# yozhijk/capsaicin

Measured on AMD Instinct MI355X. Metric: Mrays/sec (primary+secondary), cornell_box 1080p 64spp, higher is better.
Workload: dtype f32; 1 GPU; cornell_box.obj 1920x1080 64spp depth=8 (reference shading: Lambert + directional light + sky), tile-sharded over 1 GPU(s); triangles=32, bvh_depth=8, parallelism=tiles1, exchange=none

## Files before the change

### capsaicin_amd/capi.py

```python
import ctypes as C
import os
import subprocess

import numpy as np

_PKG = os.path.dirname(os.path.abspath(__file__))
_ROOT = os.path.dirname(_PKG)
LIB_PATH = os.path.join(_PKG, "libcapsaicin_hip.so")
if os.environ.get("CAP_LIB_VARIANT"):
    LIB_PATH = os.path.join(_PKG, "variants", "libcapsaicin_hip_%s.so" % os.environ["CAP_LIB_VARIANT"])

RENDER_AOV = 1
RENDER_EXT_MATERIALS = 2
RENDER_STAGE_TIMERS = 4
RENDER_GBUFFER_FEEDBACK = 8
RENDER_LOWRES_INDIRECT = 16

BUF_GBUFFER_GEO, BUF_DIRECT, BUF_ALBEDO, BUF_NORMAL_DEPTH, BUF_INDIRECT, BUF_COMBINED, BUF_ACCUM_SUM, BUF_ACCUM_MEAN, BUF_INDIRECT_LOWRES = range(9)


class CapError(RuntimeError):
    pass


# ... 267 lines not shown
    "cap_obj_set_threads": (None, [C.c_int]),
    "cap_geometry_view": (_i, [_vp, C.POINTER(GeometryView)]),
    "cap_geometry_texture_name": (C.c_char_p, [_vp, _u32]),
    "cap_geometry_warning": (C.c_char_p, [_vp]),
    "cap_geometry_materials": (_i, [_vp, _vp]),
    "cap_scene_upload_geometry": (_i, [_vp, _vp]),
    "cap_comm_unique_id": (_i, [_vp]),
    "cap_comm_init_rank": (_i, [_vp, _vp, _u32, _u32]),
    "cap_comm_gather_frame": (_i, [_vp]),
    "cap_comm_init_all": (_i, [_vp, _u32]),
    "cap_comm_gather_frame_all": (_i, [_vp, _u32]),
    "cap_comm_image": (_i, [_vp, C.POINTER(C.c_void_p)]),
    "cap_comm_readback": (_i, [_vp, _vp]),
    "cap_comm_info": (_i, [_vp, C.POINTER(_u32), C.POINTER(_u32), C.POINTER(_u32)]),
    "cap_comm_destroy": (_i, [_vp]),
    "cap_comm_abort": (_i, [_vp]),
    "cap_image_decode": (_i, [_vp, C.c_size_t, C.c_char_p, C.POINTER(C.c_void_p), C.POINTER(_u32), C.POINTER(_u32)]),
    "cap_image_free": (None, [_vp]),
    "cap_host_sah_build": (_i, [_vp, _u32, _vp, _vp, C.POINTER(_u32)]),
    "cap_host_wide_build": (_i, [_vp, _u32, _vp, _vp, _vp, _u32, _vp, _vp]),
}

_LIB = None


def build_native(force=False):
    args = ["make", "-C", os.path.join(_PKG, "csrc"), "-j8"]
    if force:
        args.append("-B")
    subprocess.check_call(args, stdout=subprocess.DEVNULL)
    return LIB_PATH


def lib():
    global _LIB
    if _LIB is None:
        if not os.path.exists(LIB_PATH):
            raise CapError("native library %s is missing: run `python -c 'import __graft_entry__ as g; g.build()'` "
                           "(there is no CPU fallback)" % LIB_PATH)
        try:
            import torch
        except Exception:
            pass
        L = C.CDLL(LIB_PATH)
        for name, (res, args) in SYMBOLS.items():
            fn = getattr(L, name)
            fn.restype, fn.argtypes = res, args
        _LIB = L
    return _LIB


def _check(rc, what):
    if rc != 0:
        raise CapError("%s failed (status %d): %s" % (what, rc, lib().cap_last_error().decode()))


def _p(a):
    return a.ctypes.data_as(C.c_void_p)


def device_count():
    return int(lib().cap_device_count())


def load_bluenoise(path=None):
    path = path or os.path.join(_ROOT, "assets", "bluenoise256.rgba")
    return np.fromfile(path, np.uint8).reshape(256, 256, 4)


_SCENE_CONFIG = None


def scene_config():
    global _SCENE_CONFIG
    if _SCENE_CONFIG is None:
        import json
        cfg = json.load(open(os.path.join(os.path.dirname(_PKG), "assets", "scene_config.json")))
        cfg["cornell_ggx"] = {k: v for k, v in cfg["cornell_ggx"].items() if not k.startswith("_")}
        _SCENE_CONFIG = cfg
    return _SCENE_CONFIG


def camera_from_config(c, width, height):
    cam = CameraData()
    f = np.float64(c["forward"])
    f /= np.linalg.norm(f)
    right = np.float64(c["right"]) if "right" in c else -np.cross(f, (0.0, 1.0, 0.0))
    right /= np.linalg.norm(right)
    up = np.float64(c["up"]) if "up" in c else np.cross(f, right)
    cam.position[:] = c["position"]
    cam.forward[:] = f
    cam.right[:] = right
    cam.up[:] = up
    cam.focal_length = c["focal_length"]
    cam.sensor_size[0] = c["sensor_x"]
    cam.sensor_size[1] = np.float32(c["sensor_x"]) * (np.float32(height) / np.float32(width))
    return cam


def cornell_camera(width, height):
    return camera_from_config(scene_config()["cornell_camera"], width, height)


class Geometry:

    def __init__(self, obj_path, mtl_dir=None):
        self.h = C.c_void_p()
        _check(lib().cap_obj_load(obj_path.encode(), (mtl_dir or "").encode(), C.byref(self.h)), "cap_obj_load")
        v = GeometryView()
        _check(lib().cap_geometry_view(self.h, C.byref(v)), "cap_geometry_view")
        self.view = v
        nv, ni, nm = v.vertex_count, v.index_count, v.mesh_count
        self.positions = np.ctypeslib.as_array(v.positions, (3 * nv,)).copy() if nv else np.zeros(0, np.float32)
        self.normals = np.ctypeslib.as_array(v.normals, (3 * nv,)).copy() if nv else np.zeros(0, np.float32)
        self.texcoords = np.ctypeslib.as_array(v.texcoords, (2 * nv,)).copy() if nv else np.zeros(0, np.float32)
        self.indices = np.ctypeslib.as_array(v.indices, (ni,)).copy() if ni else np.zeros(0, np.uint32)
        self.meshes = np.ctypeslib.as_array(v.meshes, (nm * 8,)).copy().reshape(-1, 8) if nm else np.zeros((0, 8), np.uint32)
        self.texture_names = [lib().cap_geometry_texture_name(self.h, i).decode() for i in range(v.texture_count)]
        self.material_count = v.material_count
        self.warning = lib().cap_geometry_warning(self.h).decode()

    def materials(self):
        m = np.zeros((self.meshes.shape[0], 12), np.float32)
        _check(lib().cap_geometry_materials(self.h, _p(m)), "cap_geometry_materials")
        return m

    def __del__(self):
        if getattr(self, "h", None):
            lib().cap_geometry_free(self.h)
            self.h = None


def host_sah_build(tri_lo, tri_hi):
    lo, hi = np.asarray(tri_lo, np.float32), np.asarray(tri_hi, np.float32)
    n = len(lo)
    boxes = np.zeros((n, 8), np.float32)
    boxes[:, 0:3], boxes[:, 4:7] = lo, hi
    nodes = np.zeros((max(n - 1, 1), 16), np.float32)
    order = np.zeros(n, np.uint32)
    depth = C.c_uint32()
    _check(lib().cap_host_sah_build(_p(boxes), n, _p(nodes), _p(order), C.byref(depth)), "cap_host_sah_build")
    return nodes[:max(n - 1, 0)], order, int(depth.value)


def image_decode(data, name=None):
    buf = np.frombuffer(bytes(data), np.uint8)
    px, w, h = C.c_void_p(), _u32(), _u32()
    _check(lib().cap_image_decode(_p(buf), buf.size, name.encode() if name else None, C.byref(px), C.byref(w), C.byref(h)), "cap_image_decode")
    out = np.ctypeslib.as_array(C.cast(px, C.POINTER(C.c_uint8)), (h.value, w.value, 4)).copy()
    lib().cap_image_free(px)
    return out


def host_wide_build(nodes, n, scene_lo, scene_hi):
    nodes = np.ascontiguousarray(nodes, np.float32)
    lo, hi = np.ascontiguousarray(scene_lo, np.float32), np.ascontiguousarray(scene_hi, np.float32)
    wide = np.zeros((max(n, 1), 20), np.uint32)
    src = np.zeros(max(n, 1), np.uint32)
    info = np.zeros(3, np.uint32)
    _check(lib().cap_host_wide_build(_p(nodes) if n > 1 else None, n, _p(lo), _p(hi), _p(wide), wide.shape[0], _p(src), _p(info)),
           "cap_host_wide_build")
    return wide[:int(info[0])], src[:n], int(info[1]), int(info[2])


def comm_unique_id():
    buf = (C.c_uint8 * 128)()
    _check(lib().cap_comm_unique_id(C.cast(buf, C.c_void_p)), "cap_comm_unique_id")
    return bytes(buf)


def comm_init_all(renderers):
    arr = (C.c_void_p * len(renderers))(*[r.ctx for r in renderers])
    _check(lib().cap_comm_init_all(C.cast(arr, C.c_void_p), len(renderers)), "cap_comm_init_all")


def comm_gather_frame_all(renderers):
    arr = (C.c_void_p * len(renderers))(*[r.ctx for r in renderers])
    _check(lib().cap_comm_gather_frame_all(C.cast(arr, C.c_void_p), len(renderers)), "cap_comm_gather_frame_all")


class Renderer:

    def __init__(self, device=0, stream=None):
        self.ctx = C.c_void_p()
        _check(lib().cap_ctx_create(device, C.c_void_p(stream) if stream else None, C.byref(self.ctx)), "cap_ctx_create")
        self.width = self.height = 0
        self.device = device
        self._tri_end = np.zeros(0, np.int64)
        self._vertex_count = 0

    def close(self):
        if getattr(self, "ctx", None):
            lib().cap_ctx_destroy(self.ctx)
            self.ctx = None

    __del__ = close

    def upload_scene(self, positions, normals, texcoords, indices, meshes):
        a = [np.ascontiguousarray(positions, np.float32).ravel(), np.ascontiguousarray(normals, np.float32).ravel(),
             np.ascontiguousarray(texcoords, np.float32).ravel(), np.ascontiguousarray(indices, np.uint32).ravel(),
             np.ascontiguousarray(meshes, np.uint32).reshape(-1, 8)]
        _check(lib().cap_scene_upload(self.ctx, _p(a[0]), _p(a[1]), _p(a[2]), _p(a[3]), _p(a[4]), a[0].size // 3, a[3].size,
                                      a[4].shape[0]), "cap_scene_upload")
        self._set_mesh_table(a[4])
        self._vertex_count = a[0].size // 3

    def upload_geometry(self, geo):
        _check(lib().cap_scene_upload_geometry(self.ctx, geo.h), "cap_scene_upload_geometry")
        self._set_mesh_table(geo.meshes)
        self._vertex_count = int(geo.view.vertex_count)

    def _set_mesh_table(self, meshes):
        self._tri_end = np.cumsum(np.asarray(meshes, np.uint32).reshape(-1, 8)[:, 2].astype(np.int64) // 3)

    def upload_texture(self, index, rgba8):
        if rgba8 is None:
            _check(lib().cap_texture_upload(self.ctx, index, None, 0, 0), "cap_texture_upload")
            return
        t = np.ascontiguousarray(rgba8, np.uint8)
        _check(lib().cap_texture_upload(self.ctx, index, _p(t), t.shape[1], t.shape[0]), "cap_texture_upload")

    def upload_bluenoise(self, rgba8):
        t = np.ascontiguousarray(rgba8, np.uint8)
        assert t.size == 256 * 256 * 4
        _check(lib().cap_bluenoise_upload(self.ctx, _p(t)), "cap_bluenoise_upload")

    def upload_materials(self, materials):
        m = np.ascontiguousarray(materials, np.float32).reshape(-1, 12)
        _check(lib().cap_materials_upload(self.ctx, _p(m), m.shape[0]), "cap_materials_upload")

    BVH_BUILD_AUTO, BVH_BUILD_LBVH, BVH_BUILD_SAH, BVH_BUILD_PLOC, BVH_BUILD_SAH_DEVICE = 0, 1, 2, 3, 4

    def set_bvh_build(self, mode):
        _check(lib().cap_set_bvh_build(self.ctx, mode), "cap_set_bvh_build")

    def build_bvh(self):
        _check(lib().cap_bvh_build(self.ctx), "cap_bvh_build")
        return self.bvh_info()

    def update_vertices(self, positions=None, normals=None, texcoords=None):
        ptrs, flags, keep = vertex_update_args(self._vertex_count, positions, normals, texcoords)
        if flags:
            import torch
            dev = torch.device("cuda", self.device)
            for a in keep:
                if a.device != dev:
                    raise CapError("update_vertices: tensors must be on %s, got %s" % (dev, a.device))
            torch.cuda.current_stream(dev).synchronize()
        _check(lib().cap_scene_update_vertices(self.ctx, ptrs[0], ptrs[1], ptrs[2], flags), "cap_scene_update_vertices")

    def refit_bvh(self):
        info = RefitInfo()
        _check(lib().cap_bvh_refit(self.ctx, C.byref(info)), "cap_bvh_refit")
        return info

    def bvh_info(self):
        bi = BvhInfo()
        _check(lib().cap_bvh_info(self.ctx, C.byref(bi)), "cap_bvh_info")
        return bi

    def bvh_readback(self):
        bi = self.bvh_info()
        nodes = np.zeros((bi.node_count, 16), np.float32)
        leaves = np.zeros(bi.triangle_count, np.uint32)
        _check(lib().cap_bvh_readback(self.ctx, _p(nodes), _p(leaves)), "cap_bvh_readback")
        return nodes, leaves

    def bvh_wide_readback(self):
        info = np.zeros(3, np.uint32)
        _check(lib().cap_bvh_wide_readback(self.ctx, None, None, _p(info)), "cap_bvh_wide_readback")
        nodes = np.zeros((int(info[0]), 20), np.uint32)
        src = np.zeros(max(1, self.bvh_info().triangle_count), np.uint32)
        _check(lib().cap_bvh_wide_readback(self.ctx, _p(nodes), _p(src), _p(info)), "cap_bvh_wide_readback")
        return nodes, src[:self.bvh_info().triangle_count], int(info[1]), int(info[2])

    def bvh_wide_info(self):
        info = np.zeros(3, np.uint32)
        _check(lib().cap_bvh_wide_readback(self.ctx, None, None, _p(info)), "cap_bvh_wide_readback")
        return int(info[0]), int(info[1]), int(info[2])

    def set_camera(self, cam):
        _check(lib().cap_camera_set(self.ctx, C.byref(cam)), "cap_camera_set")

    def set_prev_camera(self, cam):
        _check(lib().cap_prev_camera_set(self.ctx, C.byref(cam)), "cap_prev_camera_set")

    def set_resolution(self, width, height):
        _check(lib().cap_set_resolution(self.ctx, width, height), "cap_set_resolution")
        self.width, self.height = width, height

    def set_shard(self, index, count):
        _check(lib().cap_set_shard(self.ctx, index, count), "cap_set_shard")

    def set_traversal(self, mode):
        _check(lib().cap_set_traversal(self.ctx, mode), "cap_set_traversal")

    DEBUG_QUEUE_CAPACITY_DIV, DEBUG_WIDE_DEPTH_LIMIT, DEBUG_WIDE_IN_USE, DEBUG_FAIL_LANE1, DEBUG_LANES_USED = 1, 2, 3, 4, 5
    DEBUG_QUEUE_CANARY_FILL, DEBUG_QUEUE_CANARY_BEHIND, DEBUG_QUEUE_CANARY_USED, DEBUG_SELFTEST_DIV, DEBUG_NEE_PAIRS = 6, 7, 8, 9, 10
    DEBUG_SELFTEST_SHADE_UNARY, DEBUG_SELFTEST_SHADE_DIV2, DEBUG_SHADE_TAME = 11, 12, 13
    DEBUG_CAMERA_CULL = 14
    DEBUG_MARK_FORM = 15
    DEBUG_SAMPLE_TABLE = 16
    DEBUG_SELFTEST_SAMPLE_TABLE = 17

    def debug_set(self, key, value):
        _check(lib().cap_debug_set(self.ctx, key, value), "cap_debug_set")

    DEBUG_SWITCH_BASE = 64

    def debug_switch(self, name, value):
        i = lib().cap_debug_switch_index(name.encode())
        if i < 0:
            raise CapError("unknown switch %s" % name)
        self.debug_set(self.DEBUG_SWITCH_BASE + i, 0xFFFFFFFFFFFFFFFF if value is None else int(value))

    def debug_get(self, key):
        v = _u64()
        _check(lib().cap_debug_get(self.ctx, key, C.byref(v)), "cap_debug_get")
        return int(v.value)

    def set_batch_paths(self, n):
        _check(lib().cap_set_batch_paths(self.ctx, n), "cap_set_batch_paths")

    def render(self, frame_begin, n_frames, num_bounces, flags=0):
        _check(lib().cap_render(self.ctx, frame_begin, n_frames, num_bounces, flags), "cap_render")

    def accum_reset(self):
        _check(lib().cap_accum_reset(self.ctx), "cap_accum_reset")

    def accum_import(self, sum_rgba, frames):
        a = np.ascontiguousarray(sum_rgba, np.float32)
        assert a.shape == (self.height, self.width, 4)
        _check(lib().cap_accum_import(self.ctx, _p(a), int(frames)), "cap_accum_import")

    def sync(self):
        _check(lib().cap_sync(self.ctx), "cap_sync")

    def readback(self, kind):
        if kind == BUF_INDIRECT_LOWRES:
            out = np.zeros((self.height // 2, self.width // 2, 4), np.float32)
        else:
            out = np.zeros((self.height, self.width, 4), np.float32)
        _check(lib().cap_readback(self.ctx, kind, _p(out)), "cap_readback")
        return out

    def stats(self):
        s = Stats()
        _check(lib().cap_stats_get(self.ctx, C.byref(s)), "cap_stats_get")
        return s

    def stats_reset(self):
        _check(lib().cap_stats_reset(self.ctx), "cap_stats_reset")

    RAY_FLAG_ACCEPT_FIRST_HIT, RAY_FLAG_CULL_BACK_FACING, RAY_FLAG_CULL_FRONT_FACING = 0x04, 0x10, 0x20

    def set_instance_masks(self, masks):
        if masks is None:
            _check(lib().cap_scene_set_instance_masks(self.ctx, None, len(self._tri_end)), "cap_scene_set_instance_masks")
            return
        m = np.ascontiguousarray(masks, np.uint8).reshape(-1)
        _check(lib().cap_scene_set_instance_masks(self.ctx, _p(m), m.size), "cap_scene_set_instance_masks")

    def trace_options(self, cull=None, mask=None, first_hit=False):
        if cull not in (None, "back", "front"):
            raise CapError('cull must be None, "back" or "front", got %r' % (cull,))
        if cull is None and mask is None and not first_hit:
            return None
        flags = {None: 0, "back": self.RAY_FLAG_CULL_BACK_FACING, "front": self.RAY_FLAG_CULL_FRONT_FACING}[cull]
        if first_hit:
            flags |= self.RAY_FLAG_ACCEPT_FIRST_HIT
        return TraceOptions(flags, 0 if mask is None else int(mask))

    MULTI_MAX_K, MULTI_CONTINUE = 16, 1

    def _stage_records(self, records, width, what):
        import torch
        dev = torch.device("cuda", self.device)
        if isinstance(records, np.ndarray):
            records = torch.from_numpy(np.ascontiguousarray(records, np.float32).reshape(-1, width)).to(dev)
        if records.dtype != torch.float32 or records.dim() != 2 or records.shape[1] != width or not records.is_contiguous() or records.device != dev:
            raise CapError("%s must be a contiguous (N, %d) float32 tensor on %s, got %s %s on %s"
                           % (what, width, dev, records.dtype, tuple(records.shape), records.device))
        return dev, records, records.shape[0]

    def _out(self, out, shape, dtype, dev):
        host_out = None
        if isinstance(out, np.ndarray):
            host_out, out = out, None
        if out is None:
            import torch
            out = torch.empty(shape, dtype=dtype, device=dev)
        elif out.dtype != dtype or out.shape != shape or not out.is_contiguous() or out.device != dev:
            raise CapError("out must be a contiguous %s %s tensor on %s, got %s %s on %s" % (shape, dtype, dev, out.dtype, tuple(out.shape), out.device))
        return out, host_out

    def _resume_page(self, page, shape, dtype, dev, what):
        if page is None or isinstance(page, np.ndarray):
            import torch
            if page is None:
                return torch.empty(shape, dtype=dtype, device=dev), None
            if page.size == int(np.prod(shape)):
                return torch.from_numpy(np.ascontiguousarray(page, np.float32 if dtype == torch.float32 else np.int32).reshape(shape)).to(dev), page
        elif page.dtype == dtype and page.shape == shape and page.is_contiguous() and page.device == dev:
            return page, None
        raise CapError("%s must be the %s %s page of the previous call, a contiguous tensor on %s or a numpy array of its size, got %s %s"
                       % (what, shape, dtype, dev, page.dtype, tuple(page.shape)))

    def _page_size(self, k, counts, resuming):
        k = int(k)
        if not 0 <= k <= self.MULTI_MAX_K:
            raise CapError("k must be in 0 .. %d (page with resume=), got %d" % (self.MULTI_MAX_K, k))
        if k == 0 and (not counts or resuming):
            raise CapError("k = 0 counts only: pass counts=True and no resume")
        return k

    def _run(self, name, args, dev, sync, host, outputs, host_outputs):
        if sync:
            import torch
            torch.cuda.current_stream(dev).synchronize()
        _check(getattr(lib(), name)(self.ctx, *[a if a is None or type(a) in (int, C.c_float) else C.byref(a) if type(a) is TraceOptions
                                                else C.c_void_p(a.data_ptr()) for a in args]), name)
        if sync or host:
            self.sync()
        if not host:
            return outputs
        res = []
        for out, mine in zip(outputs, host_outputs):
            h = out.cpu().numpy()
            if mine is not None:
                mine[...] = h.reshape(mine.shape)
                h = mine
            res.append(h)
        return res

    def _single(self, name, records, width, what, out, cols, dtype, sync, tail, second=()):
        host = isinstance(records, np.ndarray)
        dev, records, n = self._stage_records(records, width, what)
        out, host_out = self._out(out, (n, cols) if cols else (n,), dtype, dev)
        extra = [out.new_empty((n,), dtype=t) for t in second]
        res = self._run(name, (records, n, out, *extra, *tail), dev, sync or host, host or host_out is not None,
                        [out] + extra, [host_out] + [None] * len(extra))
        return tuple(res) if second else res[0]

    def _multi(self, name, records, width, what, cols, instanced, k, counts, resume, sync, tail):
        import torch
        if not instanced:
            given, names = [resume], ("resume",)
        elif resume is None or (isinstance(resume, (tuple, list)) and len(resume) == 2):
            given, names = [None, None] if resume is None else list(resume), ("resume[0]", "resume[1]")
        else:
            raise CapError("resume must be the (records, instances) pair of pages of the previous call")
        host = isinstance(records, np.ndarray)
        dev, records, n = self._stage_records(records, width, what)
        k = self._page_size(k, counts, resume is not None)
        pages, host_pages = [], []
        for page, page_name, (shape, dtype) in zip(given, names, (((n, k, cols), torch.float32), ((n, k), torch.int32))):
            page, mine = self._resume_page(page, shape, dtype, dev, page_name)
            pages.append(page)
            host_pages.append(mine)
            host = host or mine is not None
        cnt = [torch.empty((n,), dtype=torch.int32, device=dev)] if counts else []
        res = self._run(name, (records, n, k, *(pages if k else [None] * len(pages)), cnt[0] if counts else None,
                               self.MULTI_CONTINUE if resume is not None else 0, *tail),
                        dev, sync or host, host, pages + cnt, host_pages + [None])
        return tuple(res) if instanced or counts else res[0]

    @staticmethod
    def _plain_or_ex(name, options, plain_tail):
        return (name, plain_tail) if options is None else (name + "_ex", (options,))

    def trace_rays(self, rays, out=None, sync=True, cull=None, mask=None, first_hit=False):
        import torch
        name, tail = self._plain_or_ex("cap_trace_rays", self.trace_options(cull, mask, first_hit), (0,))
        return self._single(name, rays, 8, "rays", out, 4, torch.float32, sync, tail)

    def trace_occlusion(self, rays, out=None, sync=True, cull=None, mask=None):
        import torch
        name, tail = self._plain_or_ex("cap_trace_occlusion", self.trace_options(cull, mask), (0,))
        return self._single(name, rays, 8, "rays", out, 0, torch.int32, sync, tail)

    def _closest_single(self, name, points, out, sync, mask, second=()):
        import torch
        return self._single(name, points, 4, "points", out, 8, torch.float32, sync, (self.trace_options(None, mask),), second)

    def closest_points(self, points, out=None, sync=True, mask=None):
        return self._closest_single("cap_closest_points", points, out, sync, mask)

    def build_pseudonormals(self):
        info = PseudonormalsInfo()
        _check(lib().cap_pseudonormals_build(self.ctx, C.byref(info)), "cap_pseudonormals_build")
        return info

    def drop_pseudonormals(self):
        _check(lib().cap_pseudonormals_drop(self.ctx), "cap_pseudonormals_drop")

    def pseudonormals(self):
        table = np.zeros((int(self._tri_end[-1]) if len(self._tri_end) else 0, 7, 3), np.float32)
        _check(lib().cap_pseudonormals_readback(self.ctx, _p(table)), "cap_pseudonormals_readback")
        return table

    def signed_distance(self, points, out=None, sync=True, mask=None, sign="pseudonormal", beta=2.0):
        import torch
        if sign == "pseudonormal":
            return self._closest_single("cap_signed_distance", points, out, sync, mask, (torch.float32,))
        if sign != "winding":
            raise CapError('sign must be "pseudonormal" or "winding", got %r' % (sign,))
        if mask is not None:
            raise CapError('sign="winding" takes no mask=: the winding number covers every triangle')
        host = isinstance(points, np.ndarray)
        dev, pts, n = self._stage_records(points, 4, "points")
        rec, host_out = self._out(out, (n, 8), torch.float32, dev)
        rec, signed = self._closest_single("cap_signed_distance", pts, rec, sync or host, None, (torch.float32,))
        w = self.winding_numbers(pts, beta=beta, sync=sync or host)
        signed = torch.where(w >= 0.5, -signed.abs(), signed.abs())
        if not (host or host_out is not None):
            return rec, signed
        h = rec.cpu().numpy()
        if host_out is not None:
            host_out[...] = h.reshape(host_out.shape)
            h = host_out
        return h, signed.cpu().numpy()

    def build_winding(self):
        info = WindingInfo()
        _check(lib().cap_winding_build(self.ctx, C.byref(info)), "cap_winding_build")
        return info

    def drop_winding(self):
        _check(lib().cap_winding_drop(self.ctx), "cap_winding_drop")

    def winding_table(self):
        table = np.zeros((max(self.bvh_info().triangle_count, 1) - 1, 2, 8), np.float32)
        _check(lib().cap_winding_readback(self.ctx, _p(table)), "cap_winding_readback")
        return table

    def winding_numbers(self, points, beta=2.0, out=None, visits=False, sync=True):
        import torch
        host = isinstance(points, np.ndarray)
        dev, points, n = self._stage_records(points, 4, "points")
        out, host_out = self._out(out, (n,), torch.float32, dev)
        vis = [torch.empty((n, 2), dtype=torch.int32, device=dev)] if visits else []
        res = self._run("cap_winding_numbers", (points, n, C.c_float(beta), out, vis[0] if visits else None), dev, sync or host,
                        host or host_out is not None, [out] + vis, [host_out, None])
        return tuple(res) if visits else res[0]

    def closest_instances(self, points, out=None, sync=True, mask=None):
        import torch
        return self._closest_single("cap_closest_instances", points, out, sync, mask, (torch.int32,))

    def signed_distance_instances(self, points, out=None, sync=True, mask=None):
        import torch
        return self._closest_single("cap_signed_distance_instances", points, out, sync, mask, (torch.int32, torch.float32))

    def closest_points_multi(self, points, k, counts=False, resume=None, sync=True, mask=None):
        return self._multi("cap_closest_points_multi", points, 4, "points", 8, False, k, counts, resume, sync, (self.trace_options(None, mask),))

    def closest_instances_multi(self, points, k, counts=False, resume=None, sync=True, mask=None):
        return self._multi("cap_closest_instances_multi", points, 4, "points", 8, True, k, counts, resume, sync, (self.trace_options(None, mask),))


    def set_objects(self, ranges):
        info = ObjectsInfo()
        r = np.zeros((0, 2), np.uint32) if ranges is None else np.ascontiguousarray(ranges, np.uint32).reshape(-1, 2)
        _check(lib().cap_objects_set(self.ctx, _p(r) if len(r) else None, len(r), C.byref(info)), "cap_objects_set")
        self._instances_n = 0
        return info

    def objects_info(self):
        n = C.c_uint32(0)
        _check(lib().cap_objects_info(self.ctx, None, 0, C.byref(n)), "cap_objects_info")
        out = np.zeros(n.value, OBJECT_INFO_DTYPE)
        if n.value:
            _check(lib().cap_objects_info(self.ctx, _p(out), n.value, None), "cap_objects_info")
        return out

    def set_instances(self, transforms, masks=None, sync=True, objects=None):
        info = InstancesInfo()
        if transforms is None:
            _check(lib().cap_instances_set(self.ctx, None, 0, 0, C.byref(info)), "cap_instances_set")
            self._instances_n = 0
            return info
        if isinstance(transforms, np.ndarray) or not hasattr(transforms, "device"):
            t = np.ascontiguousarray(transforms, np.float32)
            if t.ndim < 2 or t.size != t.shape[0] * 12:
                raise CapError("transforms must be (N, 3, 4) or (N, 12), got %s" % (t.shape,))
            d = np.zeros(t.shape[0], INSTANCE_DESC_DTYPE)
            d["transform"] = t.reshape(-1, 12)
            d["mask"] = 0xFF if masks is None else np.asarray(masks).astype(np.uint32).reshape(-1)
            if objects is None:
                _check(lib().cap_instances_set(self.ctx, _p(d), d.shape[0], 0, C.byref(info)), "cap_instances_set")
            else:
                o = np.ascontiguousarray(np.asarray(objects).astype(np.uint32).reshape(-1))
                if o.size != d.shape[0]:
                    raise CapError("objects must hold one index per instance (%d), got %d" % (d.shape[0], o.size))
                _check(lib().cap_instances_set_ex(self.ctx, _p(d), _p(o), d.shape[0], 0, C.byref(info)), "cap_instances_set_ex")
            self._instances_n = d.shape[0]
            return info
        import torch
        dev = torch.device("cuda", self.device)
        if transforms.dtype != torch.float32 or transforms.device != dev or transforms.numel() != transforms.shape[0] * 12:
            raise CapError("transforms must be an (N, 3, 4) or (N, 12) float32 tensor on %s" % (dev,))
        n = transforms.shape[0]
        d = torch.zeros((n, 16), dtype=torch.float32, device=dev)
        d[:, :12] = transforms.reshape(n, 12)
        m = torch.full((n,), 0xFF, dtype=torch.int32, device=dev) if masks is None else torch.as_tensor(masks, device=dev).to(torch.int32).reshape(n)
        d[:, 12] = m.view(torch.float32)
# ... 128 lines not shown
```

### capsaicin_amd/csrc/cap_context.h

```cpp
#pragma once

#include <array>
#include <string>
#include <utility>
#include <vector>

#include "../../include/capsaicin_hip.h"

#include "cap_kernels.h"

namespace cap
{
int fail(int code, const char* fmt, ...);

#define HIP_TRY(expr)                                                                                         \
    do                                                                                                        \
    {                                                                                                         \
        hipError_t e_ = (expr);                                                                               \
        if (e_ != hipSuccess) return fail(CAP_ERR_HIP, "%s failed: %s (%s:%d)", #expr, hipGetErrorString(e_), \
                                          __FILE__, __LINE__);                                                \
    } while (0)

template <typename T>
struct DevBuf
{
    T*     p = nullptr;
    size_t n = 0;
    DevBuf() = default;
    DevBuf(const DevBuf&) = delete;
    DevBuf& operator=(const DevBuf&) = delete;
    DevBuf(DevBuf&& o) noexcept : p(o.p), n(o.n) { o.p = nullptr, o.n = 0; }
    DevBuf& operator=(DevBuf&& o) noexcept
    {
        if (this != &o)
        {
            release();
            p = o.p, n = o.n, o.p = nullptr, o.n = 0;
        }
        return *this;
    }
    ~DevBuf() { release(); }
    void release()
    {
        if (p) (void)hipFree(p);
        p = nullptr, n = 0;
    }
    hipError_t ensure(size_t count)
    {
        if (count <= n && p) return hipSuccess;
        release();
        if (count == 0) count = 1;
        hipError_t e = hipMalloc((void**)&p, count * sizeof(T));
        if (e == hipSuccess) n = count;
        return e;
    }
};

enum StageId
{
    ST_PRIMARY,
    ST_CLOSEST,
    ST_ANY,
    ST_SHADE,
    ST_RESOLVE,
    ST_POST,
    ST_COUNT,
    ST_DIRECT,
    ST_POST_PASS0,
    ST_NONE = -1
};

struct TimedSpan
{
    hipEvent_t a, b;
    int        stage;
    int        also = ST_NONE;
};
}

using namespace cap;

struct CapContext
{
    int         device = 0;
    hipStream_t stream = nullptr;
    bool        own_stream = false;
    int         cu_count = 256;

    DevBuf<float>    positions, normals, texcoords;
    DevBuf<uint32_t> indices;
    DevBuf<uint4>    tri_ids;
    DevBuf<uint4>    mesh_offsets;
    DevBuf<uint32_t> mesh_texture;
    uint32_t         vertex_count = 0, index_count = 0, mesh_count = 0, tri_count = 0;
    bool             scene_ready = false;

    std::vector<DevBuf<uint8_t>> texture_data;
    std::vector<TextureDev>      texture_host;
    DevBuf<TextureDev>           textures;
    bool                         textures_dirty = true;
    DevBuf<float2>               bluenoise;
    bool                         bluenoise_ready = false;
    std::vector<CapMaterial>     materials_host;
    DevBuf<CapMaterial>          materials;
    std::vector<float>           positions_host;
    std::vector<uint32_t>        indices_host;
    std::vector<CapMeshDesc>     meshes_host;
    DevBuf<uint32_t>             light_tris;
    DevBuf<float>                light_cdf;
    DevBuf<float2>               bluenoise_ba;
    uint32_t                     light_count = 0;
    float                        light_area  = 0.0f;
    bool                         materials_ready = false;

    DevBuf<float4>   shade_tris, tris_sorted, nodes, tri_raw, tri_box;
    DevBuf<float4>   nodes8, tris8;
    DevBuf<uint32_t> wide_src;
    DevBuf<uint32_t> wide_task, wide_alloc, wide_cnt;
    uint32_t         wide8_depth = 0, wide8_top = 0, wide8_nodes = 0;
    float            wide8_ms = 0.f;
    DevBuf<uint32_t> query_work, query_defer;
    DevBuf<uint8_t>  tri_mask;
    bool             tri_mask_on = false;
    DevBuf<float4>   inst_desc, inst_rec, inst_box, inst_tlas;
    DevBuf<uint32_t> inst_keys[2], inst_vals[2], inst_hist, inst_scan, inst_misc, inst_level_off;
    uint32_t         inst_count = 0, inst_top = 0, inst_nodes = 0;
    DevBuf<float2>   inst_near;
    DevBuf<uint32_t> inst_obj;
    bool             inst_obj_on = false;
    InstObject       scene_object_host{};
    DevBuf<InstObject> scene_object;
    std::vector<CapObjectInfo> obj_info;
    std::vector<uint32_t>      obj_node_base, obj_rec_base;
    uint32_t                   obj_count = 0, obj_max_depth = 0;
    DevBuf<float4>             forest_nodes, forest_tris;
    DevBuf<InstObject>         obj_table;
    DevBuf<float4>             obj_tri_raw, obj_tri_box;
    DevBuf<uint32_t>           obj_leaf_tri, obj_misc;
    DevBuf<float4>   fan_pairs, fan_singles;
    uint32_t         fan_pair_count = 0, fan_single_count = 0;
    DevBuf<float4>   fan_pairs_nee;
    uint32_t         fan_pair_nee_count = 0;
    std::vector<float>    fan_pairs_host;
    std::vector<uint32_t> light_tris_host;
    DevBuf<uint32_t> leaf_tri, keys0, keys1, vals0, vals1, hist, parent, flags, bvh_misc;
    DevBuf<float4>   ploc_boxes;
    DevBuf<uint32_t> ploc_ints;
    DevBuf<uint32_t> sahdev_words;
    CapBvhInfo       bvh_info{};
    bool             shade_tame = false;
    bool             bvh_ready = false;
    DevBuf<float>        pn_table;
    bool                 pn_ready = false;
    CapPseudonormalsInfo pn_info{};
    DevBuf<float4>       wn_table;
    bool                 wn_ready = false;
    CapWindingInfo       wn_info{};
    bool                  bvh_stale = false;
    bool                  positions_host_stale = false;
    bool                  visits_built_known = false;
    double                refit_visits_built = 0.0;
    std::vector<uint32_t> wide_levels;
    DevBuf<float>         wide_boxes;
    DevBuf<double>        refit_sums;

    CapCameraData camera{}, prev_camera{};
    bool          camera_ready = false, prev_camera_ready = false;
    ScreenDev     screen{};
    uint64_t      max_batch_paths = 0;
    SwitchTable   sw{};
    uint32_t      debug_capacity_div = 1;
    uint32_t      debug_wide_depth_limit = 0;
    bool          debug_fail_lane = false;
    uint64_t      lane1_failed_paths = 0;
    uint32_t      lane1_failed_bounces = 0, lane1_retry_tick = 0;
    uint32_t      lanes_last_render = 0;
    uint32_t      last_class_capacity = 0;
    uint32_t      tri_ids_dense = 0;
    uint32_t      last_mark_form = 0;
    uint32_t      last_sample_table = 0;
    struct LastTerms
    {
        const FrameConst* frames = nullptr;
        uint32_t          n_slots = 0, num_bounces = 0, lane = 0;
    } last_terms;
    uint32_t      last_cull_camera_pairs = 0;
    uint32_t      traversal_mode  = CAP_TRAVERSAL_AUTO;
    uint32_t      bvh_build_mode  = CAP_BVH_BUILD_AUTO;

    DevBuf<float4>     aov_geo, aov_nd, accum, image_tmp;
    DevBuf<uint64_t>   shaded_counter;
    struct Lane
    {
        hipStream_t      stream = nullptr;
        DevBuf<float4>   hits, q_org[2], q_dir[2], q_thr[2], s_org, s_dir, s_con, pl_color, pl_direct, pl_albedo;
        DevBuf<float4>   terms;
        DevBuf<uint32_t> counters;
        DevBuf<uint32_t> stack_spill;
    } lane[2];
    hipStream_t stream2 = nullptr;
    hipEvent_t  lane_ev[2] = {nullptr, nullptr}, fork_ev = nullptr, join_ev = nullptr;
    static constexpr int kFrameRing = 4;
    DevBuf<FrameConst> frames_ring[kFrameRing];
    FrameConst*        frames_pinned[kFrameRing] = {nullptr, nullptr, nullptr, nullptr};
    size_t             frames_pinned_n[kFrameRing] = {0, 0, 0, 0};
    hipEvent_t         frames_event[kFrameRing] = {nullptr, nullptr, nullptr, nullptr};
    uint32_t           frames_next = 0;
    uint32_t           last_slots = 0;
    bool               aov_valid = false;
    bool               aov_lowres = false;
    uint32_t           aov_frame  = 0;
    uint64_t           frames_accumulated = 0;

    DevBuf<float4> post_in[4];
    DevBuf<float4> post_ihist[2], post_mhist[2], post_chist[2], post_prev_nd, post_itemp, post_temp[2], post_normals;
    uint32_t       post_w = 0, post_h = 0;
    int            post_last_dst = -1;

    void*           comm = nullptr;
    uint32_t        comm_rank = 0, comm_size = 0;
    bool            comm_local = false;
    DevBuf<float>   comm_send, comm_gathered, comm_image;
    hipEvent_t      comm_event = nullptr;

    CapStats               stats{};
    std::vector<TimedSpan> spans;
    std::vector<std::array<hipEvent_t, 6>> post_marks;
    std::vector<hipEvent_t> event_pool;
    std::vector<uint32_t*> pinned_pool;
    std::vector<std::pair<uint32_t*, uint32_t>> pending;
    uint64_t*              pinned_shaded = nullptr;
};

namespace cap
{
struct AovPlanes
{
    const float4 *color, *direct, *albedo;
};

int        sync_and_collect(CapContext* c);
hipEvent_t get_event(CapContext* c);
CameraDev  camera_dev(const CapCameraData& cd);
BvhDev     bvh_dev(const CapContext* c, const CapContext::Lane& lane);
AovPlanes  aov_planes(const CapContext* c);
int        trace_launch(const CapContext* c, const char* fmt, ...);
void       launch_texture_footprints(hipStream_t stream, const uint32_t* src, uint4* dst, uint32_t width, uint32_t height);
bool pair_ids_dense(const float* pairs, uint32_t pair_count, uint32_t single_count, uint32_t tri_count);
int  upload_fan_records(CapContext* c);
int  update_nee_pairs(CapContext* c);
int  ensure_positions_host(CapContext* c);
int  upload_light_table(CapContext* c);
int query_state(CapContext* c, const char* what);
}
```

### capsaicin_amd/csrc/cap_kernels.h

```cpp
#pragma once

#include "cap_device.h"

#include <cstdio>
#include <vector>

namespace cap
{
enum CapSwitch : uint32_t
{
    SW_NO_WIDE8 = 0,
    SW_LANE1_PRIORITY,
    SW_PLOC_RADIUS,
    SW_SAHDEV_LEAF,
    SW_WIDE_HOST_COLLAPSE,
    SW_TRACE_LAUNCHES,
    SW_NO_TWO_LANES,
    SW_LANE_SPLIT_MIN,
    SW_BLOCKS_PER_CU,
    SW_NO_CAMERA_CULL,
    SW_NO_ALBEDO_IN_W,
    SW_NO_INLINE_NEE,
    SW_NO_INLINE_PROBE,
    SW_NO_WAVE_RING,
    SW_ANY_REFILL,
    SW_PRIMARY_WIDE,
    SW_NO_PACKET,
    SW_NO_ANY_PROBE,
    SW_ANY_PROBE,
    SW_ANY_BLOCKS,
    SW_NO_PRIMARY_FUSE,
    SW_W8_REFILL,
    SW_W8_GRID,
    SW_AUTO_SAH_TRIANGLES,
    SW_NO_NEE_PAIR_CULL,
    SW_RAYGEN_KERNEL,
    SW_NO_PLANE_CODE,
    SW_SAMPLE_TABLE,
    SW_COUNT
};
struct SwitchTable
{
    int64_t v[SW_COUNT];
    bool    on(CapSwitch k) const { return v[k] > 0; }
    int64_t get(CapSwitch k, int64_t dflt) const { return v[k] >= 0 ? v[k] : dflt; }
};

struct LaunchCfg
{
    hipStream_t stream;
    uint32_t    grid_blocks;
    uint32_t    stack_entries;
    uint32_t    cu_count = 0;
    uint32_t    any_no_probe = 0;
    const SwitchTable* sw = nullptr;
    bool    sw_on(CapSwitch k) const { return sw && sw->on(k); }
    int64_t sw_get(CapSwitch k, int64_t dflt) const { return sw ? sw->get(k, dflt) : dflt; }
};

template <auto K>
uint32_t resident_grid(const LaunchCfg& cfg, uint32_t want)
{
    static int per_cu = -1;
    if (per_cu < 0)
    {
        int n = 0;
        per_cu = (hipOccupancyMaxActiveBlocksPerMultiprocessor(&n, K, (int)kBlock, 0) == hipSuccess && n > 0) ? n : 0;
        if (cfg.sw_on(SW_TRACE_LAUNCHES)) fprintf(stderr, "[cap] resident workgroups per CU: %d\n", per_cu);
    }
    if (!cfg.cu_count || !per_cu) return want;
    const uint32_t cap = cfg.cu_count * (uint32_t)per_cu;
    return want < cap ? want : cap;
}
inline uint32_t queue_grid(const LaunchCfg& cfg, uint32_t max_count)
{
    uint32_t g = (max_count + kBlock - 1) / kBlock;
    if (g > cfg.grid_blocks) g = cfg.grid_blocks;
    return g ? g : 1;
}

void launch_trace_primary(const LaunchCfg& cfg, const BvhDev& bvh, const CameraDev& cam, const ScreenDev& screen,
                          const FrameConst* frames, uint32_t n_slots, float4* hits, uint32_t* work);
void launch_raygen_identity(const LaunchCfg& cfg, const CameraDev& cam, const ScreenDev& screen, const FrameConst* frames, uint32_t n_slots,
                            const RayQueue& q);
void launch_trace_closest(const LaunchCfg& cfg, const BvhDev& bvh, const RayQueue& q, uint32_t max_count, float4* hits);
void launch_trace_closest8(const LaunchCfg& cfg, const BvhDev& bvh, const RayQueue& q, uint32_t max_count, float4* hits, uint32_t* work);
void launch_trace_closest8_camera(const LaunchCfg& cfg, const BvhDev& bvh, const RayQueue& q, uint32_t max_count, float4* hits, uint32_t* work,
                                  const CameraDev& cam, const ScreenDev& screen, const FrameConst* frames, uint32_t n_slots);
void launch_trace_any(const LaunchCfg& cfg, const BvhDev& bvh, const ShadowQueue& q, uint32_t max_count, float4* target,
                      uint32_t pixels_padded, uint32_t n_slots, uint64_t* guard, uint32_t* work, bool mostly_unoccluded,
                      const FrameConst* frames, float4* code_plane = nullptr);

void launch_trace_any8_refill(const LaunchCfg& cfg, const BvhDev& bvh, const ShadowQueue& q, uint32_t max_count, float4* target, uint32_t pixels_padded,
                              uint32_t n_slots, uint64_t* guard, uint32_t* work, const FrameConst* frames);

struct QueryArgs
{
    const float4* rays;
    uint32_t      n;
    void*         out;
    uint32_t*     work;
    uint32_t*     defer;
    float         safe;
};
constexpr float kQuerySafeScale = 4.0f;
bool query8_stack_matches();
struct RayFilter;
void launch_query8(const LaunchCfg& cfg, const BvhDev& bvh, const QueryArgs& q, bool any, const RayFilter* f = nullptr, bool first_hit = false);
void launch_query_binary(const LaunchCfg& cfg, const BvhDev& bvh, const QueryArgs& q, bool any, bool deferred);
struct MultiArgs
{
    QueryArgs q;
    uint32_t  k;
    uint32_t* counts;
    uint32_t  resume;
};
constexpr uint32_t kMultiMaxK = 16;
uint32_t multi_bucket(uint32_t k);
void     launch_query8_multi(const LaunchCfg& cfg, const BvhDev& bvh, const MultiArgs& m, const RayFilter* f = nullptr);
void     launch_query_binary_multi(const LaunchCfg& cfg, const BvhDev& bvh, const MultiArgs& m, bool deferred, const RayFilter* f = nullptr);

struct RayFilter
{
    uint32_t       cull_and, cull_xor;
    uint32_t       mask;
    const uint8_t* tri_mask;
};
void launch_query_binary_filtered(const LaunchCfg& cfg, const BvhDev& bvh, const QueryArgs& q, const RayFilter& f, bool any, bool first_hit, bool deferred);

struct ClosestArgs
{
    const float4* points;
    uint32_t      n;
    float4*       out;
    float         slack;
};
constexpr float kClosestSlackScale = 1.0f / 262144.0f;
void launch_closest_points(const LaunchCfg& cfg, const BvhDev& bvh, const ClosestArgs& a, const RayFilter* f, uint32_t depth);
struct SignedArgs
{
    const float* normals;
    float*       signed_out;
};
void launch_signed_distance(const LaunchCfg& cfg, const BvhDev& bvh, const ClosestArgs& a, const SignedArgs& s, const RayFilter* f, uint32_t depth);
struct ClosestMultiArgs
{
    ClosestArgs a;
    uint32_t    k;
    uint32_t*   counts;
    uint32_t    resume;
};
void launch_closest_points_multi(const LaunchCfg& cfg, const BvhDev& bvh, const ClosestMultiArgs& m, const RayFilter* f, uint32_t depth);
struct TlasDev;
struct ClosestInstArgs
{
    ClosestArgs     a;
    uint32_t*       inst_out;
    const float4*   descs;
    const float2*   near;
    const uint32_t* xw_max;
};
void launch_closest_instances(const LaunchCfg& cfg, const BvhDev& bvh, const ClosestInstArgs& a, const TlasDev& tl, const RayFilter& f, uint32_t depth);
void launch_signed_distance_instances(const LaunchCfg& cfg, const BvhDev& bvh, const ClosestInstArgs& a, const SignedArgs& s, const TlasDev& tl,
                                      const RayFilter& f, uint32_t depth);
struct ClosestInstMultiArgs
{
    ClosestInstArgs ia;
    uint32_t        k;
    uint32_t*       counts;
    uint32_t        resume;
};
void launch_closest_instances_multi(const LaunchCfg& cfg, const BvhDev& bvh, const ClosestInstMultiArgs& m, const TlasDev& tl, const RayFilter& f,
                                    uint32_t depth);

struct InstObject
{
    double   blo[3], bhi[3];
    int32_t  root;
    uint32_t reserved;
};
struct InstanceBuildArgs
{
    const float*      descs;
    uint32_t          n;
    const InstObject* objects;
    uint32_t          n_objects;
    const uint32_t*   object_index;
    float4*      rec;
    float4*      box;
    float4*      tlas;
    float2*      near;
    uint32_t*    keys[2];
    uint32_t*    vals[2];
    uint32_t*    hist;
    uint32_t*    scan;
    uint32_t*    misc;
};
constexpr uint32_t kTlasMaxLevels = 25;
uint32_t tlas_layout(uint32_t n, uint32_t level_off[kTlasMaxLevels], uint32_t* total);
void     launch_instances_build(hipStream_t stream, const InstanceBuildArgs& a);
struct TlasDev
{
    const float4*   rec;
    const float4*   tlas;
    const uint32_t* level_off;
    uint32_t        top;
};
void launch_query_instances(const LaunchCfg& cfg, const BvhDev& bvh, const QueryArgs& q, const TlasDev& tl, const RayFilter& f, int mode, uint32_t* inst_out,
                            uint32_t depth);
void launch_query_instances_multi(const LaunchCfg& cfg, const BvhDev& bvh, const MultiArgs& m, const TlasDev& tl, const RayFilter& f, uint32_t* inst_out,
                                  uint32_t depth);
struct ForestRelocArgs
{
    float4*  nodes;
    float4*  tris;
    uint32_t n_tris, node_base, rec_base, first_triangle;
};
void launch_forest_relocate(hipStream_t stream, const ForestRelocArgs& a);

struct ShadeArgs
{
    SceneDev          scene;
    CameraDev         cam;
    ScreenDev         screen;
    const FrameConst* frames;
    union
    {
        const float4* hits;
        const float4* sample_terms;
    };
    RayQueue          in;
    RayQueue          out;
    ShadowQueue       shadow;
    Planes            planes;
    uint32_t          n_slots;
    uint32_t          bounce;
    uint32_t          num_bounces;
    uint32_t          max_count;
    uint32_t          aov_slot;
    uint64_t*         shaded_counter;
    uint32_t*         work;
    FeedbackDev       fb;
    uint32_t          albedo_in_w;
    uint32_t          inline_nee;
    uint32_t          inline_probe;
    uint32_t          wave_ring;
    uint32_t          cull_camera_pairs;
    uint32_t          code_in_color;
};
constexpr float kCodePadding = 0.f, kCodeSky = 1.f, kCodeKd = 2.f, kCodeBlack = 3.f;
constexpr float kCodeLit = 4.f;
constexpr float kCameraCullPad = 2.0f;
void launch_shade(const LaunchCfg& cfg, const ShadeArgs& args, bool ext, bool feedback = false);
bool launch_primary_shade(const LaunchCfg& cfg, const BvhDev& bvh, const ShadeArgs& args, float4* hits, bool ext);
uint32_t launch_trace_shade(const LaunchCfg& cfg, const BvhDev& bvh, const ShadeArgs& args, bool ext, bool feedback = false);
bool trace_shade_has_code_form(const BvhDev& bvh, const SceneDev& scene);
bool trace_shade_has_table_form(const BvhDev& bvh, const SceneDev& scene);
void launch_sample_terms(hipStream_t stream, const float2* bluenoise, const FrameConst* frames, uint32_t n_slots, uint32_t num_bounces, float4* table);
void launch_sample_terms_selftest(hipStream_t stream, const float2* bluenoise, const FrameConst* frames, uint32_t n_slots, uint32_t num_bounces,
                                  const float4* table, unsigned long long* out_device);

void launch_resolve(const LaunchCfg& cfg, const Planes& planes, uint32_t n_slots, uint32_t pixels_padded, float4* accum,
                    bool albedo_in_w = false, float kd_untextured = 0.0f, bool code_in_color = false);
void launch_untile(const LaunchCfg& cfg, const ScreenDev& screen, const float4* src, const float4* albedo, const float4* direct,
                   int plane_kind, float4* image);
void launch_tile(const LaunchCfg& cfg, const ScreenDev& screen, const float4* image, float4* dst);
void launch_untile4(const LaunchCfg& cfg, const ScreenDev& screen, const float4* s0, const float4* s1, const float4* s2, const float4* s3,
                    float4* d0, float4* d1, float4* d2, float4* d3);
void launch_tiles_mean(const LaunchCfg& cfg, const float4* accum, uint32_t pixels_padded, float4* dst);
void launch_assemble(const LaunchCfg& cfg, const ScreenDev& screen, const float4* gathered, uint32_t shard_count, float4* image,
                     size_t shard_stride = 0);
void launch_geo_aov(const LaunchCfg& cfg, const SceneDev& scene, const float4* hits_slot, uint32_t pixels_padded, float4* aov_geo);

struct BvhBuildArgs
{
    const float*    positions;
    const float*    normals;
    const float*    texcoords;
    const uint32_t* indices;
    const uint4*    tri_ids;
    const uint4*    mesh_offsets;
    uint32_t        tri_count;
    float4*         shade_tris;
    float4*         tris_sorted;
    float4*         nodes;
    uint32_t*       leaf_tri;
    float4*         tri_raw;
    float4*         tri_box;
    uint32_t*       keys[2];
    uint32_t*       vals[2];
    uint32_t*       hist;
    uint32_t*       parent;
    uint32_t*       flags;
    uint32_t*       bounds;
    uint32_t*       max_depth;
};
size_t bvh_radix_blocks(uint32_t n);
void   launch_bvh_build(hipStream_t stream, const BvhBuildArgs& a);
int    launch_bvh_sort(hipStream_t stream, const BvhBuildArgs& a);
size_t bvh_radix_scan_words(uint32_t n);
int    launch_radix_sort_pairs(hipStream_t stream, uint32_t* const keys[2], uint32_t* const vals[2], uint32_t n, uint32_t* hist, uint32_t* scan);
size_t bvh_scan_scratch_words(uint32_t total);
void   launch_exclusive_scan_u32(hipStream_t stream, uint32_t* v, uint32_t total, uint32_t* scratch);
struct PlocScratch
{
    float4*   boxes;
    uint32_t* ints;
};
int    launch_bvh_build_ploc(hipStream_t stream, const BvhBuildArgs& a, const PlocScratch& s, uint32_t radius);
size_t bvh_sah_device_scratch_words(uint32_t n);
int    launch_bvh_build_sah_device(hipStream_t stream, const BvhBuildArgs& a, const PlocScratch& s, uint32_t* scratch, uint32_t radius, uint32_t leaf);
void launch_bvh_setup(hipStream_t stream, const BvhBuildArgs& a);
void launch_bvh_finish_host(hipStream_t stream, const BvhBuildArgs& a);

void     launch_gather_wide(hipStream_t stream, const uint32_t* tri_src, const float4* tris_sorted, uint32_t n, float4* tris8);
struct WideCollapseArgs
{
    const float4*   bnodes;
    const uint32_t* count;
    uint32_t        n_tris, capacity;
    double          pad;
    uint32_t *      task, *alloc, *nodes8, *tri_src;
    uint32_t*       cnt;
    uint32_t        begin, end;
};
int      launch_wide_collapse(hipStream_t stream, WideCollapseArgs a, uint32_t* node_count, uint32_t* depth, uint32_t* top_nodes,
                          std::vector<uint32_t>* level_begin = nullptr);
struct PseudonormalArgs
{
    const float*    positions;
    const uint32_t* indices;
    const uint4*    tri_ids;
    const uint4*    mesh_offsets;
    uint32_t        tri_count;
    float*          table;
    uint32_t *      kx, *ky, *kz;
    uint32_t*       keys[2];
    uint32_t*       vals[2];
    uint32_t*       weld;
    uint32_t*       flag;
    uint32_t*       hist;
    uint32_t*       scan;
    double*         nf;
    double*         ang;
    uint32_t*       stats;
};
size_t pseudonormal_scan_words(uint32_t corners);
void   launch_pseudonormals_build(hipStream_t stream, const PseudonormalArgs& a);

struct WindingBuildArgs
{
    const float*    positions;
    const uint32_t* indices;
    const uint4*    tri_ids;
    const uint4*    mesh_offsets;
    uint32_t        tri_count;
    const float4*   nodes;
    const uint32_t* leaf_tri;
    float4*         table;
    double*         tri_sums;
    double*         sums;
    uint32_t*       parent;
    uint32_t*       flags;
    uint32_t*       stats;
    double*         root;
};
void launch_winding_build(hipStream_t stream, const WindingBuildArgs& a);
struct WindingArgs
{
    const float4* points;
    uint32_t      n;
    const float4* table;
    float         beta;
    float*        out;
    uint32_t*     visits;
};
void launch_winding_numbers(const LaunchCfg& cfg, const BvhDev& bvh, const WindingArgs& a, uint32_t depth);

void   launch_bvh_refit_climb(hipStream_t stream, const BvhBuildArgs& a);
void   launch_refit_binary(hipStream_t stream, const BvhBuildArgs& a);
size_t tree_visits_scratch();
void   launch_tree_visits(hipStream_t stream, const float4* nodes, uint32_t n_tris, double* scratch, double* out);
struct WideRefitArgs
{
    uint32_t*     nodes8;
    const float4* tris8;
    const float4* tri_box;
    float*        boxes;
    double        pad;
    uint32_t      one_triangle;
    uint32_t      begin, end;
};
void launch_refit_wide(hipStream_t stream, WideRefitArgs a, const std::vector<uint32_t>& level_begin);
uint32_t wide8_stack_pairs();

struct PostSettingsDev
{
    int   gather, denoise, eaw5;
    float eaw_normal_sigma, eaw_depth_sigma, eaw_luma_sigma;
    float gather_normal_sigma, gather_depth_sigma, gather_luma_sigma;
    float temporal_upscale_feedback, taa_feedback;
    int   lowres_indirect;
    int   use_variance;
    int   fast_weights;
    int   output;
};
struct PostChainArgs
{
    PostSettingsDev settings;
    uint32_t        width, height, frame_count;
    CameraDev       camera, prev_camera;
    const float4 *indirect, *direct, *albedo, *normal_depth;
    uint32_t      tiled;
    const float4 *tiled_indirect, *tiled_normal_depth;
    float4*       indirect_rowmajor;
    ScreenDev     screen;
    float4 *indirect_history[2], *moments_history[2], *combined_history[2], *prev_normal_depth;
    float4 *indirect_temp, *temp[2], *normals;
    void (*mark)(void* user, int pass);
    void* mark_user;
};
void launch_post_chain(hipStream_t stream, const PostChainArgs& a);
void launch_div_selftest(hipStream_t stream, unsigned long long* out_device);
void launch_shade_forms_selftest(hipStream_t stream, unsigned long long* out_device, uint32_t which);
void launch_decimate2x(hipStream_t stream, const float4* full, uint32_t width, uint32_t height, uint32_t ox, uint32_t oy, float4* out);
}
```

### capsaicin_amd/csrc/context.hip

```cpp
#include <algorithm>
#include <cmath>
#include <cstdarg>
#include <cstdio>
#include <cstdlib>
#include <cstring>
#include <memory>

#include "cap_context.h"
#include "cap_near.h"
#include "cap_wide.h"
#include "query_ranges.h"

namespace
{
thread_local std::string g_error;

constexpr double kPrimaryWideTrianglesPerPixel = 2.0;
constexpr uint64_t kAnyRefillTreeBytes = ~0ull;

constexpr size_t kGuardWords = 8;
}

namespace cap
{
int fail(int code, const char* fmt, ...)
{
    char    buf[512];
    va_list ap;
    va_start(ap, fmt);
    vsnprintf(buf, sizeof(buf), fmt, ap);
    va_end(ap);
    g_error = buf;
    return code;
}

int sync_and_collect(CapContext* c)
{
    HIP_TRY(hipStreamSynchronize(c->stream));
    for (auto& sp : c->spans)
    {
        float ms = 0.f;
        if (hipEventElapsedTime(&ms, sp.a, sp.b) == hipSuccess)
        {
            for (int stage : {sp.stage, sp.also})
                switch (stage)
                {
                case ST_PRIMARY: c->stats.ms_primary += ms; break;
                case ST_CLOSEST: c->stats.ms_trace_closest += ms; break;
                case ST_ANY: c->stats.ms_trace_any += ms; break;
                case ST_SHADE: c->stats.ms_shade += ms; break;
                case ST_RESOLVE: c->stats.ms_resolve += ms; break;
                case ST_POST: c->stats.ms_post += ms; break;
                case ST_COUNT: c->stats.ms_total += ms; break;
                case ST_DIRECT: c->stats.ms_direct += ms; break;
                default:
                    if (stage >= ST_POST_PASS0 && stage < ST_POST_PASS0 + 5) c->stats.ms_post_pass[stage - ST_POST_PASS0] += ms;
                }
        }
        c->event_pool.push_back(sp.a);
        c->event_pool.push_back(sp.b);
    }
    c->spans.clear();
    for (auto& m : c->post_marks)
    {
        for (int pass = 0; pass < 5; ++pass)
        {
            float ms = 0.f;
            if (hipEventElapsedTime(&ms, m[pass], m[pass + 1]) == hipSuccess) c->stats.ms_post_pass[pass] += ms, c->stats.ms_post += ms;
        }
        for (hipEvent_t e : m) c->event_pool.push_back(e);
    }
    c->post_marks.clear();
    for (auto& pc : c->pending)
    {
        const uint32_t D = pc.second & 0xffffu;
        const bool     queued = (pc.second >> 16) == 0u;
        const size_t per = (size_t)kQueueClasses * kCounterStride;
        for (uint32_t b = 0; b <= D; ++b)
            for (uint32_t k = 0; k < kQueueClasses; ++k)
            {
                c->stats.rays_extension += pc.first[b * per + k * kCounterStride];
                c->stats.rays_shadow += pc.first[b * per + k * kCounterStride + 1];
                if (queued) c->stats.shadow_entries += pc.first[b * per + k * kCounterStride + 1];
                if (b == 0)
                {
                    c->stats.rays_extension_bounce0 += pc.first[k * kCounterStride];
                    c->stats.rays_shadow_bounce0 += pc.first[k * kCounterStride + 1];
                    if (queued) c->stats.shadow_entries_bounce0 += pc.first[k * kCounterStride + 1];
                }
                c->stats.rays_shadow += pc.first[b * per + k * kCounterStride + 2];
                if (b == 0) c->stats.rays_shadow_bounce0 += pc.first[k * kCounterStride + 2];
                c->stats.shaded_vertices += pc.first[b * per + k * kCounterStride + 3];
            }
        c->pinned_pool.push_back(pc.first);
    }
    c->pending.clear();
    if (c->pinned_shaded && c->shaded_counter.p)
    {
        HIP_TRY(hipMemcpy(c->pinned_shaded, c->shaded_counter.p, kGuardWords * sizeof(uint64_t), hipMemcpyDeviceToHost));
        c->stats.guard_shade     = c->pinned_shaded[1];
        c->stats.guard_trace_any = c->pinned_shaded[2];
        c->stats.guard_last      = c->pinned_shaded[3];
        c->stats.guard_append    = c->pinned_shaded[4];
    }
    return CAP_OK;
}

hipEvent_t get_event(CapContext* c)
{
    if (!c->event_pool.empty())
    {
        hipEvent_t e = c->event_pool.back();
        c->event_pool.pop_back();
        return e;
    }
    hipEvent_t e = nullptr;
    (void)hipEventCreate(&e);
    return e;
}

CameraDev camera_dev(const CapCameraData& cd)
{
    CameraDev d{};
    for (int k = 0; k < 3; ++k) d.position[k] = cd.position[k], d.right[k] = cd.right[k], d.forward[k] = cd.forward[k], d.up[k] = cd.up[k];
    d.focal_length = cd.focal_length;
    d.sensor_x     = cd.sensor_size[0];
    d.sensor_y     = cd.sensor_size[1];
    return d;
}

BvhDev bvh_dev(const CapContext* c, const CapContext::Lane& lane)
{
    BvhDev b{};
    b.nodes     = c->nodes.p;
    b.tris      = c->tris_sorted.p;
    b.tris_by_id = c->tri_raw.p;
    b.stack_spill   = lane.stack_spill.p;
    b.spill_threads = (uint32_t)(lane.stack_spill.n / kSpillEntries);
    const bool no_wide8 = c->sw.on(SW_NO_WIDE8);
    b.nodes8 = c->nodes8.p, b.tris8 = c->tris8.p;
    b.wide8_ok  = !no_wide8 && lane.stack_spill.p && c->wide8_nodes != 0 && c->wide8_depth <= wide8_stack_pairs() + 1u &&
                 c->wide8_depth <= kWideLdsEntries / 2u + kSpillEntries / 2u + 1u &&
                 (c->debug_wide_depth_limit == 0u || c->wide8_depth <= c->debug_wide_depth_limit);
    b.wide8_top = c->wide8_top;
    b.fan_pairs = c->fan_pairs.p, b.fan_singles = c->fan_singles.p;
    b.fan_pair_count = c->fan_pair_count, b.fan_single_count = c->fan_single_count;
    b.tri_ids_dense = c->tri_ids_dense;
    b.fan_pairs_nee = c->fan_pairs_nee.p ? c->fan_pairs_nee.p : c->fan_pairs.p;
    b.fan_pair_nee_count = c->fan_pairs_nee.p ? c->fan_pair_nee_count : c->fan_pair_count;
    b.tri_count = c->tri_count;
    b.root      = c->tri_count >= 2 ? 0 : ~0;
    return b;
}

AovPlanes aov_planes(const CapContext* c)
{
    const size_t off = (size_t)(c->last_slots ? c->last_slots - 1 : 0) * c->screen.pixels_padded;
    return AovPlanes{c->lane[0].pl_color.p + off, c->lane[0].pl_direct.p + off, c->lane[0].pl_albedo.p + off};
}

int trace_launch(const CapContext* c, const char* fmt, ...)
{
    if (!c->sw.on(SW_TRACE_LAUNCHES)) return CAP_OK;
    va_list ap;
    va_start(ap, fmt);
    fputs("[cap] ", stderr);
    vfprintf(stderr, fmt, ap);
    va_end(ap);
    fputs(" ... ", stderr);
    fflush(stderr);
    hipError_t e = hipStreamSynchronize(c->stream);
    fprintf(stderr, "%s\n", hipGetErrorString(e));
    fflush(stderr);
    return e == hipSuccess ? CAP_OK : CAP_ERR_HIP;
}
}

namespace
{
struct StageTimer
{
    CapContext* c;
    TimedSpan   sp;
    bool        on;
    StageTimer(CapContext* ctx, int stage, bool enabled = true, int also = ST_NONE) : c(ctx), on(enabled)
    {
        if (!on) return;
        sp.stage = stage;
        sp.also  = also;
        sp.a     = get_event(c);
        sp.b     = get_event(c);
        (void)hipEventRecord(sp.a, c->stream);
    }
    ~StageTimer()
    {
        if (!on) return;
        (void)hipEventRecord(sp.b, c->stream);
        c->spans.push_back(sp);
    }
};

void update_screen(CapContext* c, uint32_t w, uint32_t h, uint32_t shard_index, uint32_t shard_count)
{
    ScreenDev& s  = c->screen;
    s.width       = w;
    s.height      = h;
    s.tiles_x     = (w + kTileDim - 1) / kTileDim;
    s.tiles_y     = (h + kTileDim - 1) / kTileDim;
    s.tile_count  = s.tiles_x * s.tiles_y;
    s.shard_index = shard_index;
    s.shard_count = shard_count ? shard_count : 1;
    const uint32_t max_local = (s.tile_count + s.shard_count - 1) / s.shard_count;
    s.local_tiles   = s.tile_count > s.shard_index ? (s.tile_count - s.shard_index + s.shard_count - 1) / s.shard_count : 0;
    s.pixels_padded = max_local * kTilePixels;
    tile_div_setup(s.tiles_x, s.tiles_x_mul, s.tiles_x_shift);
    c->frames_accumulated = 0;
    c->aov_valid = false;
}

FrameConst frame_const(uint32_t frame_count, bool lowres_indirect)
{
    FrameConst f{};
    halton23(frame_count, f.jitter_x, f.jitter_y);
    f.frame_count = frame_count;
    f.lowres_sel = lowres_indirect ? (4u | (((frame_count % 4u) / 2u) << 1) | ((frame_count % 4u) % 2u)) : 0u;
    const float t = 2.0f * 3.14f * (float)(frame_count % 4096) / 4096.0f;
    float       st, ct;
    sincos_c(t, st, ct);
    const v3 dir = normalize3(mk3(40.0f * st, 100.0f, 40.0f * ct));
    f.light_dir[0] = dir.x, f.light_dir[1] = dir.y, f.light_dir[2] = dir.z;
    f.light_intensity[0] = 1.0f * (2.0f * 14.0f + 0.0f);
    f.light_intensity[1] = 1.0f * (2.0f * 12.0f + 0.0f);
    f.light_intensity[2] = 1.0f * (2.0f * 10.0f + (2.0f + 2.0f * ct));
    return f;
}

SceneDev scene_dev(const CapContext* c)
{
    SceneDev s{};
    s.shade_tris    = c->shade_tris.p;
    s.tri_ids       = c->tri_ids.p;
    s.mesh_texture  = c->mesh_texture.p;
    s.textures      = c->textures.p;
    s.texture_count = (uint32_t)c->texture_host.size();
    s.bluenoise     = c->bluenoise.p;
    s.kd_untextured = pow22_c(0.75f);
    s.shade_tame    = c->shade_tame ? 1u : 0u;
    s.bluenoise_ba  = c->bluenoise_ba.p;
    s.materials     = reinterpret_cast<const MaterialDev*>(c->materials.p);
    s.material_count = c->materials_ready ? c->mesh_count : 0u;
    s.light_tris    = c->light_tris.p;
    s.light_cdf     = c->light_cdf.p;
    s.light_count   = c->light_count;
    s.light_area    = c->light_area;
    return s;
}

struct LaneSizes
{
    size_t planes, queues, rings, counters, terms;
};

LaneSizes lane_sizes(const CapContext* c, uint32_t slots, uint32_t bounces, bool sample_table)
{
    LaneSizes z;
    z.planes = (size_t)slots * c->screen.pixels_padded;
    z.queues = z.planes + (size_t)kQueueClasses * 64;
    z.rings = std::max(z.queues, (size_t)std::max(c->cu_count, 1) * 8 * (kBlock / 64) * 128);
    z.counters = (3 * (size_t)(bounces + 1) + 1) * kQueueClasses * kCounterStride;
    z.terms = sample_table ? (size_t)slots * bounces * 4096 : 0;
    return z;
}

bool lane_grows(const CapContext::Lane& L, const LaneSizes& z) { return L.pl_color.n < z.planes || L.counters.n < z.counters || L.terms.n < z.terms; }

int ensure_lane(CapContext* c, CapContext::Lane& L, uint32_t slots, uint32_t bounces, bool sample_table)
{
    const LaneSizes z = lane_sizes(c, slots, bounces, sample_table);
    for (DevBuf<float4>* b : {&L.hits, &L.q_org[0], &L.q_org[1], &L.q_dir[0], &L.q_dir[1], &L.q_thr[0], &L.q_thr[1], &L.s_dir})
        HIP_TRY(b->ensure(z.queues));
    for (DevBuf<float4>* b : {&L.s_org, &L.s_con}) HIP_TRY(b->ensure(z.rings));
    for (DevBuf<float4>* b : {&L.pl_color, &L.pl_direct, &L.pl_albedo}) HIP_TRY(b->ensure(z.planes));
    HIP_TRY(L.counters.ensure(z.counters));
    if (z.terms) HIP_TRY(L.terms.ensure(z.terms));
    if (c->lane[0].stack_spill.n) HIP_TRY(L.stack_spill.ensure(c->lane[0].stack_spill.n));
    return CAP_OK;
}

int ensure_frame_buffers(CapContext* c)
{
    HIP_TRY(c->aov_geo.ensure(c->screen.pixels_padded));
    HIP_TRY(c->aov_nd.ensure(c->screen.pixels_padded));
    if (!c->shaded_counter.p)
    {
        HIP_TRY(c->shaded_counter.ensure(kGuardWords));
        HIP_TRY(hipMemsetAsync(c->shaded_counter.p, 0, kGuardWords * sizeof(uint64_t), c->stream));
    }
    if (!c->accum.p || c->accum.n < c->screen.pixels_padded)
    {
        HIP_TRY(c->accum.ensure(c->screen.pixels_padded));
        HIP_TRY(hipMemsetAsync(c->accum.p, 0, sizeof(float4) * c->screen.pixels_padded, c->stream));
        c->frames_accumulated = 0;
    }
    return CAP_OK;
}

int ensure_lane_streams(CapContext* c)
{
    if (!c->stream2)
    {
        if (c->sw.v[SW_LANE1_PRIORITY] >= 0)
            HIP_TRY(hipStreamCreateWithPriority(&c->stream2, hipStreamNonBlocking, (int)c->sw.v[SW_LANE1_PRIORITY]));
        else
            HIP_TRY(hipStreamCreateWithFlags(&c->stream2, hipStreamNonBlocking));
    }
    c->lane[1].stream = c->stream2;
    for (hipEvent_t* e : {&c->lane_ev[0], &c->lane_ev[1], &c->fork_ev, &c->join_ev})
        if (!*e) HIP_TRY(hipEventCreateWithFlags(e, hipEventDisableTiming));
    return CAP_OK;
}

struct BatchPolicy
{
    uint32_t slots;
    bool     two_lanes;
    bool     lane1_failed_before;
};

BatchPolicy batch_policy(const CapContext* c, uint32_t n_frames, uint32_t num_bounces, uint32_t flags, bool tree_path)
{
    const uint32_t Ppad = c->screen.pixels_padded;
    uint64_t       budget = c->max_batch_paths ? c->max_batch_paths : (uint64_t)64 << 20;
    if (!c->max_batch_paths && (uint64_t)n_frames * Ppad > budget)
    {
        const uint64_t big       = (uint64_t)128 << 20;
        const uint64_t big_slots = std::max<uint64_t>(1, std::min<uint64_t>(big / std::max(1u, Ppad), kMaxFrameSlots));
        bool           room      = c->lane[0].pl_color.n >= big_slots * Ppad && (!tree_path || c->lane[1].pl_color.n >= big_slots * Ppad);
        if (!room)
        {
            size_t free_b = 0, total_b = 0;
            room = hipMemGetInfo(&free_b, &total_b) == hipSuccess && free_b > 3u * big_slots * Ppad * 256u;
        }
        if (room) budget = big;
    }
    uint32_t       slots  = (uint32_t)std::max<uint64_t>(1, std::min<uint64_t>(budget / std::max(1u, Ppad), kMaxFrameSlots));
    slots                 = std::min(slots, n_frames);
    const bool no_two_lanes = c->sw.on(SW_NO_TWO_LANES);
    bool two_lanes = !no_two_lanes && tree_path && c->bvh_info.stack_entries != 0 && !(flags & CAP_RENDER_GBUFFER_FEEDBACK) &&
                     !(flags & CAP_RENDER_LOWRES_INDIRECT) && n_frames >= 2;
    if (two_lanes && slots >= n_frames)
    {
        const uint64_t split_min = (uint64_t)c->sw.get(SW_LANE_SPLIT_MIN, (int64_t)4 << 20);
        if ((uint64_t)n_frames * Ppad >= split_min)
            slots = (n_frames + 1) / 2;
        else
            two_lanes = false;
    }
    if ((flags & CAP_RENDER_STAGE_TIMERS) || c->sw.on(SW_TRACE_LAUNCHES)) two_lanes = false;
    const bool failed_before =
        two_lanes && c->lane1_failed_paths && (uint64_t)slots * Ppad >= c->lane1_failed_paths && num_bounces >= c->lane1_failed_bounces;
    return BatchPolicy{slots, two_lanes, failed_before};
}
}

__global__ __launch_bounds__(256) void k_texture_footprints(const uint32_t* src, uint4* dst, uint32_t width, uint32_t height)
{
    const size_t i = (size_t)blockIdx.x * 256 + threadIdx.x;
    if (i >= (size_t)width * height) return;
    const uint32_t y = (uint32_t)(i / width), x = (uint32_t)(i - (size_t)y * width);
    const uint32_t x1 = x + 1 == width ? 0 : x + 1, y1 = y + 1 == height ? 0 : y + 1;
    dst[i] = make_uint4(src[(size_t)y * width + x], src[(size_t)y * width + x1], src[(size_t)y1 * width + x], src[(size_t)y1 * width + x1]);
}

void cap::launch_texture_footprints(hipStream_t stream, const uint32_t* src, uint4* dst, uint32_t width, uint32_t height)
{
    const size_t texels = (size_t)width * height;
    hipLaunchKernelGGL(k_texture_footprints, dim3((unsigned)((texels + 255) / 256)), dim3(256), 0, stream, src, dst, width, height);
}

extern "C" {

const char* cap_last_error(void) { return g_error.c_str(); }
void cap_set_error_(const char* msg) { g_error = msg ? msg : ""; }

int cap_device_count(void)
{
    int n = 0;
    if (hipGetDeviceCount(&n) != hipSuccess) return 0;
    return n;
}

static const char* const kSwitchNames[SW_COUNT] = {
    "CAP_NO_WIDE8", "CAP_LANE1_PRIORITY", "CAP_PLOC_RADIUS", "CAP_SAHDEV_LEAF", "CAP_WIDE_HOST_COLLAPSE", "CAP_TRACE_LAUNCHES", "CAP_NO_TWO_LANES",
    "CAP_LANE_SPLIT_MIN", "CAP_BLOCKS_PER_CU", "CAP_NO_CAMERA_CULL", "CAP_NO_ALBEDO_IN_W", "CAP_NO_INLINE_NEE", "CAP_NO_INLINE_PROBE", "CAP_NO_WAVE_RING",
    "CAP_ANY_REFILL", "CAP_PRIMARY_WIDE", "CAP_NO_PACKET", "CAP_NO_ANY_PROBE", "CAP_ANY_PROBE", "CAP_ANY_BLOCKS", "CAP_NO_PRIMARY_FUSE", "CAP_W8_REFILL",
    "CAP_W8_GRID", "CAP_AUTO_SAH_TRIANGLES", "CAP_NO_NEE_PAIR_CULL", "CAP_RAYGEN_KERNEL", "CAP_NO_PLANE_CODE", "CAP_SAMPLE_TABLE"};

static void switches_from_environment(SwitchTable& t)
{
    for (uint32_t k = 0; k < SW_COUNT; ++k)
    {
        const char* e = getenv(kSwitchNames[k]);
        t.v[k]        = -1;
        if (!e) continue;
        char*           end = nullptr;
        const long long v   = strtoll(e, &end, 10);
        t.v[k]              = (end != e && v >= 0) ? v : 1;
    }
    if (getenv("CAP_BVH_BINARY") && t.v[SW_NO_WIDE8] < 0) t.v[SW_NO_WIDE8] = 1;
}

int cap_debug_switch_index(const char* name)
{
    for (uint32_t k = 0; name && k < SW_COUNT; ++k)
        if (strcmp(name, kSwitchNames[k]) == 0) return (int)k;
    return -1;
}

extern "C" int cap_debug_tile_divmod(uint32_t tiles_x, const uint32_t* n, uint64_t count, uint32_t* quotient, uint32_t* remainder)
{
    if (!tiles_x || !n || !quotient || !remainder) return CAP_ERR_INVALID_ARG;
    uint32_t mul, shift;
    tile_div_setup(tiles_x, mul, shift);
    for (uint64_t k = 0; k < count; ++k)
    {
        quotient[k]  = tile_div(n[k], mul, shift);
        remainder[k] = n[k] - quotient[k] * tiles_x;
    }
    return CAP_OK;
}

int cap_debug_pair_ids_dense(const float* pair_records, uint32_t pair_count, uint32_t single_count, uint32_t tri_count)
{
    if (!pair_records && pair_count) return 0;
    return pair_ids_dense(pair_records, pair_count, single_count, tri_count) ? 1 : 0;
}

int cap_debug_query_ranges(uint64_t n, uint32_t count, const uint64_t* base, const uint64_t* stride, const uint32_t* align)
{
    static const char* const names[4] = {"range 0", "range 1", "range 2", "range 3"};
    if (count > 4 || (count && (!base || !stride || !align))) return fail(CAP_ERR_INVALID_ARG, "cap_debug_query_ranges: at most 4 ranges, no NULL array");
    QueryRange r[4];
    for (uint32_t i = 0; i < count; ++i)
    {
        if (!align[i] || (align[i] & (align[i] - 1u))) return fail(CAP_ERR_INVALID_ARG, "cap_debug_query_ranges: align[%u] is not a power of two", i);
        r[i] = QueryRange{names[i], (uintptr_t)base[i], stride[i], align[i], stride[i] != 0};
    }
    char msg[256];
    return query_ranges_ok("cap_debug_query_ranges", n, r, count, msg, sizeof(msg)) ? CAP_OK : fail(CAP_ERR_INVALID_ARG, "%s", msg);
}

int cap_debug_closest_instance_bound(const float* transform, const float* box_lo, const float* box_hi, const float* point, float best_dist2,
                                     float* world_to_object, float* g, float* xw, float* slack, uint32_t* skip)
{
    if (!transform || !box_lo || !box_hi || !point) return fail(CAP_ERR_INVALID_ARG, "cap_debug_closest_instance_bound: NULL input");
    double m[12], w[12], wd[12], A[12], nA, kappa, blo[3], bhi[3];
    float  wf[12];
    bool   live = true;
    for (int k = 0; k < 12; ++k) m[k] = (double)transform[k], live = live && finite_d(m[k]);
    for (int k = 0; k < 3; ++k) blo[k] = (double)box_lo[k], bhi[k] = (double)box_hi[k];
    live = instance_inverse(m, live, w, wf, wd, A, nA, kappa, (float)CAP_INSTANCE_MAX_CONDITION);
    const float gi = live ? near_sigma_min_bound(w) : 0.0f, xi = live ? near_world_extent(m, blo, bhi) : 0.0f;
    const float pmax = fmaxf(fabsf(point[0]), fmaxf(fabsf(point[1]), fabsf(point[2])));
    const float sl   = near_slack(pmax, xi);
    float       ox, oy, oz;
    near_to_object(wf, point[0], point[1], point[2], ox, oy, oz);
    const float bd2 = box_dist2(ox, oy, oz, box_lo[0], box_lo[1], box_lo[2], box_hi[0], box_hi[1], box_hi[2]);
    if (world_to_object)
        for (int k = 0; k < 12; ++k) world_to_object[k] = wf[k];
    if (g) *g = gi;
    if (xw) *xw = xi;
    if (slack) *slack = sl;
    if (skip) *skip = live && near_skip(bd2, near_bound2_object(sqrtf(best_dist2), sl, gi)) ? 1u : 0u;
    return CAP_OK;
}

int cap_ctx_create(int device_id, void* hip_stream, CapContext** out_ctx)
{
    if (!out_ctx) return fail(CAP_ERR_INVALID_ARG, "cap_ctx_create: out_ctx is NULL");
    *out_ctx = nullptr;
    int n    = 0;
    HIP_TRY(hipGetDeviceCount(&n));
    if (device_id < 0 || device_id >= n) return fail(CAP_ERR_HIP, "cap_ctx_create: device %d not present (%d HIP devices)", device_id, n);
    HIP_TRY(hipSetDevice(device_id));
    CapContext* c = new CapContext;
    c->device     = device_id;
    switches_from_environment(c->sw);
    hipDeviceProp_t prop;
    if (hipGetDeviceProperties(&prop, device_id) == hipSuccess) c->cu_count = prop.multiProcessorCount;
    if (hip_stream)
        c->stream = (hipStream_t)hip_stream;
    else
    {
        hipError_t e = hipStreamCreateWithFlags(&c->stream, hipStreamNonBlocking);
        if (e != hipSuccess)
        {
            delete c;
            return fail(CAP_ERR_HIP, "hipStreamCreate failed: %s", hipGetErrorString(e));
        }
        c->own_stream = true;
    }
    c->lane[0].stream = c->stream;
    (void)hipHostMalloc((void**)&c->pinned_shaded, kGuardWords * sizeof(uint64_t), hipHostMallocDefault);
    update_screen(c, 0, 0, 0, 1);
    *out_ctx = c;
    return CAP_OK;
}

void cap_ctx_destroy(CapContext* c)
{
    if (!c) return;
    (void)hipSetDevice(c->device);
    (void)hipStreamSynchronize(c->stream);
    for (auto& sp : c->spans)
    {
        (void)hipEventDestroy(sp.a);
        (void)hipEventDestroy(sp.b);
    }
    for (auto e : c->event_pool) (void)hipEventDestroy(e);
    for (auto& pc : c->pending) (void)hipHostFree(pc.first);
    for (auto p : c->pinned_pool) (void)hipHostFree(p);
    if (c->pinned_shaded) (void)hipHostFree(c->pinned_shaded);
    (void)cap_comm_destroy(c);
    for (int k = 0; k < CapContext::kFrameRing; ++k)
    {
        if (c->frames_pinned[k]) (void)hipHostFree(c->frames_pinned[k]);
        if (c->frames_event[k]) (void)hipEventDestroy(c->frames_event[k]);
    }
    if (c->stream2) (void)hipStreamSynchronize(c->stream2), (void)hipStreamDestroy(c->stream2);
    for (hipEvent_t e : {c->lane_ev[0], c->lane_ev[1], c->fork_ev, c->join_ev})
        if (e) (void)hipEventDestroy(e);
    if (c->own_stream) (void)hipStreamDestroy(c->stream);
    delete c;
}

int cap_camera_set(CapContext* c, const CapCameraData* camera)
{
    if (!c || !camera) return fail(CAP_ERR_INVALID_ARG, "cap_camera_set: NULL argument");
    c->camera       = *camera;
    c->camera_ready = true;
    return CAP_OK;
}

int cap_prev_camera_set(CapContext* c, const CapCameraData* camera)
{
    if (!c || !camera) return fail(CAP_ERR_INVALID_ARG, "cap_prev_camera_set: NULL argument");
    c->prev_camera       = *camera;
    c->prev_camera_ready = true;
    return CAP_OK;
}

int cap_set_resolution(CapContext* c, uint32_t width, uint32_t height)
{
    if (!c) return fail(CAP_ERR_INVALID_ARG, "cap_set_resolution: ctx is NULL");
    if (!width || !height || width > 32768 || height > 32768) return fail(CAP_ERR_INVALID_ARG, "cap_set_resolution: bad extent %ux%u", width, height);
    HIP_TRY(hipSetDevice(c->device));
    HIP_TRY(hipStreamSynchronize(c->stream));
    update_screen(c, width, height, c->screen.shard_index, c->screen.shard_count);
    if ((uint64_t)c->screen.pixels_padded > kPidMask) return fail(CAP_ERR_UNSUPPORTED, "too many pixels per shard");
    c->accum.release();
    c->lane1_failed_paths = 0;
    c->post_w = c->post_h = 0;
    c->post_last_dst = -1;
    return CAP_OK;
}

int cap_set_shard(CapContext* c, uint32_t shard_index, uint32_t shard_count)
{
    if (!c) return fail(CAP_ERR_INVALID_ARG, "cap_set_shard: ctx is NULL");
    if (!shard_count || shard_index >= shard_count) return fail(CAP_ERR_INVALID_ARG, "cap_set_shard: bad shard %u of %u", shard_index, shard_count);
    HIP_TRY(hipSetDevice(c->device));
    HIP_TRY(hipStreamSynchronize(c->stream));
    update_screen(c, c->screen.width, c->screen.height, shard_index, shard_count);
    c->accum.release();
    c->lane1_failed_paths = 0;
    return CAP_OK;
}

int cap_set_batch_paths(CapContext* c, uint64_t max_paths)
{
    if (!c) return fail(CAP_ERR_INVALID_ARG, "cap_set_batch_paths: ctx is NULL");
    c->max_batch_paths = max_paths;
    c->lane1_failed_paths = 0;
    return CAP_OK;
}

constexpr uint32_t kCanaryWord = 0x7fc0da7au;
__global__ __launch_bounds__(256) void k_canary_count(const uint4* p, size_t begin, size_t end, unsigned long long* out)
{
    unsigned long long n = 0;
    for (size_t i = begin + blockIdx.x * (size_t)256 + threadIdx.x; i < end; i += (size_t)gridDim.x * 256)
    {
        const uint4 v = p[i];
        n += (v.x != kCanaryWord || v.y != kCanaryWord || v.z != kCanaryWord || v.w != kCanaryWord) ? 1u : 0u;
    }
    for (int off = 32; off > 0; off >>= 1) n += __shfl_down(n, off);
    if ((threadIdx.x & 63u) == 0 && n) atomicAdd(out, n);
}
static int canary_count(CapContext* c, bool behind, uint64_t* value)
{
    CapContext::Lane& L = c->lane[0];
    if (!L.q_org[0].p || !c->last_class_capacity) return fail(CAP_ERR_STATE, "cap_debug_get: no render yet");
    HIP_TRY(hipSetDevice(c->device));
    DevBuf<unsigned long long> dbuf;
    HIP_TRY(dbuf.ensure(1));
    unsigned long long* d = dbuf.p;
    HIP_TRY(hipMemsetAsync(d, 0, sizeof(*d), c->stream));
    const size_t used = std::min((size_t)kQueueClasses * c->last_class_capacity, L.q_org[0].n);
    for (int k = 0; k < 2; ++k)
        for (DevBuf<float4>* b : {&L.q_org[k], &L.q_dir[k], &L.q_thr[k]})
        {
            const size_t lo = behind ? used : 0, hi = behind ? b->n : used;
            if (hi > lo) hipLaunchKernelGGL(k_canary_count, dim3(512), dim3(256), 0, c->stream, reinterpret_cast<const uint4*>(b->p), lo, hi, d);
        }
    HIP_TRY(hipGetLastError());
    unsigned long long h = 0;
    HIP_TRY(hipMemcpyAsync(&h, d, sizeof(h), hipMemcpyDeviceToHost, c->stream));
    HIP_TRY(hipStreamSynchronize(c->stream));
    *value = h;
    return CAP_OK;
}

int cap_debug_set(CapContext* c, uint32_t key, uint64_t value)
{
    if (!c) return fail(CAP_ERR_INVALID_ARG, "cap_debug_set: ctx is NULL");
    switch (key)
    {
    case CAP_DEBUG_QUEUE_CAPACITY_DIV:
        if (value < 1 || value > 1024) return fail(CAP_ERR_INVALID_ARG, "cap_debug_set: capacity divisor %llu not in 1..1024", (unsigned long long)value);
        c->debug_capacity_div = (uint32_t)value;
        return CAP_OK;
    case CAP_DEBUG_WIDE_DEPTH_LIMIT:
        c->debug_wide_depth_limit = (uint32_t)value;
        return CAP_OK;
    case CAP_DEBUG_QUEUE_CANARY_FILL:
        if (!c->lane[0].q_org[0].p) return fail(CAP_ERR_STATE, "cap_debug_set: the queues are allocated by the first cap_render");
        HIP_TRY(hipSetDevice(c->device));
        for (int k = 0; k < 2; ++k)
            for (DevBuf<float4>* b : {&c->lane[0].q_org[k], &c->lane[0].q_dir[k], &c->lane[0].q_thr[k]})
                HIP_TRY(hipMemsetD32Async((hipDeviceptr_t)b->p, (int)kCanaryWord, b->n * 4, c->stream));
        return CAP_OK;
    case CAP_DEBUG_FAIL_LANE1:
        c->debug_fail_lane = value != 0;
        if (!value) c->lane1_failed_paths = 0;
        return CAP_OK;
    default:
        if (key >= CAP_DEBUG_SWITCH_BASE && key < CAP_DEBUG_SWITCH_BASE + SW_COUNT)
        {
            c->sw.v[key - CAP_DEBUG_SWITCH_BASE] = value == ~0ull ? -1 : (int64_t)value;
            return CAP_OK;
        }
        return fail(CAP_ERR_INVALID_ARG, "cap_debug_set: unknown key %u", key);
    }
}

int cap_debug_get(CapContext* c, uint32_t key, uint64_t* value)
{
    if (!c || !value) return fail(CAP_ERR_INVALID_ARG, "cap_debug_get: NULL argument");
    switch (key)
    {
    case CAP_DEBUG_QUEUE_CAPACITY_DIV: *value = c->debug_capacity_div; return CAP_OK;
    case CAP_DEBUG_WIDE_DEPTH_LIMIT: *value = c->debug_wide_depth_limit; return CAP_OK;
    case CAP_DEBUG_FAIL_LANE1: *value = c->debug_fail_lane ? 1u : 0u; return CAP_OK;
    case CAP_DEBUG_LANES_USED: *value = c->lanes_last_render; return CAP_OK;
    case CAP_DEBUG_SELFTEST_DIV:
    {
        HIP_TRY(hipSetDevice(c->device));
        DevBuf<unsigned long long> d;
        unsigned long long         h[3] = {0, 0, 0};
        HIP_TRY(d.ensure(3));
        HIP_TRY(hipMemsetAsync(d.p, 0, sizeof(h), c->stream));
        launch_div_selftest(c->stream, d.p);
        HIP_TRY(hipGetLastError());
        HIP_TRY(hipMemcpyAsync(h, d.p, sizeof(h), hipMemcpyDeviceToHost, c->stream));
        HIP_TRY(hipStreamSynchronize(c->stream));
        const unsigned long long expected = (0x7f7fffffull - 0x00800000ull + 1ull) + (1ull << 30);
        if (h[2] != expected) return fail(CAP_ERR_HIP, "cap_debug_get: the division self-test compared %llu of %llu cases", h[2], expected);
        *value = h[0] + h[1];
        return CAP_OK;
    }
    case CAP_DEBUG_SELFTEST_SHADE_UNARY:
    case CAP_DEBUG_SELFTEST_SHADE_DIV2:
    {
        HIP_TRY(hipSetDevice(c->device));
        DevBuf<unsigned long long> d;
        unsigned long long         h[2] = {0, 0};
        HIP_TRY(d.ensure(2));
        HIP_TRY(hipMemsetAsync(d.p, 0, sizeof(h), c->stream));
        launch_shade_forms_selftest(c->stream, d.p, key == CAP_DEBUG_SELFTEST_SHADE_DIV2 ? 1u : 0u);
        HIP_TRY(hipGetLastError());
        HIP_TRY(hipMemcpyAsync(h, d.p, sizeof(h), hipMemcpyDeviceToHost, c->stream));
        HIP_TRY(hipStreamSynchronize(c->stream));
        const unsigned long long floats_sqrt = 0x7f7fffffull - ((127ull - 96ull) << 23) + 1ull;
        const unsigned long long least = key == CAP_DEBUG_SELFTEST_SHADE_DIV2 ? (1ull << 30) : 2ull * floats_sqrt + 3ull + (5ull << 23) + 1ull + 0x40000001ull + (8ull << 23);
        if (h[1] < least) return fail(CAP_ERR_HIP, "cap_debug_get: the shading self-test compared %llu of at least %llu cases", h[1], least);
        *value = h[0];
        return CAP_OK;
    }
    case CAP_DEBUG_SHADE_TAME:
        if (!c->bvh_ready || c->bvh_stale) return fail(CAP_ERR_STATE, "cap_debug_get: BVH not built or stale");
        *value = c->shade_tame ? 1u : 0u;
        return CAP_OK;
    case CAP_DEBUG_CAMERA_CULL: *value = c->last_cull_camera_pairs; return CAP_OK;
    case CAP_DEBUG_MARK_FORM:
        if (!c->bvh_ready) return fail(CAP_ERR_STATE, "cap_debug_get: BVH not built");
        *value = ((uint64_t)c->last_mark_form << 8) | c->tri_ids_dense;
        return CAP_OK;
    case CAP_DEBUG_SAMPLE_TABLE: *value = c->last_sample_table; return CAP_OK;
    case CAP_DEBUG_SELFTEST_SAMPLE_TABLE:
    {
        const CapContext::LastTerms& lt = c->last_terms;
        if (!c->last_sample_table || !lt.frames) return fail(CAP_ERR_STATE, "cap_debug_get: the last cap_render built no sample table");
        HIP_TRY(hipSetDevice(c->device));
        if (sync_and_collect(c) != CAP_OK) return CAP_ERR_HIP;
        DevBuf<unsigned long long> d;
        unsigned long long         h[2] = {0, 0};
        HIP_TRY(d.ensure(2));
        HIP_TRY(hipMemsetAsync(d.p, 0, sizeof(h), c->stream));
        launch_sample_terms_selftest(c->stream, c->bluenoise.p, lt.frames, lt.n_slots, lt.num_bounces, c->lane[lt.lane].terms.p, d.p);
        HIP_TRY(hipGetLastError());
        HIP_TRY(hipMemcpyAsync(h, d.p, sizeof(h), hipMemcpyDeviceToHost, c->stream));
        HIP_TRY(hipStreamSynchronize(c->stream));
        const unsigned long long expected = (unsigned long long)lt.n_slots * lt.num_bounces * 4096ull;
        if (h[1] != expected) return fail(CAP_ERR_HIP, "cap_debug_get: the sample table self-test compared %llu of %llu entries", h[1], expected);
        *value = (h[0] << 32) | (expected >> 12);
        return CAP_OK;
    }
    case CAP_DEBUG_NEE_PAIRS:
        if (!c->bvh_ready) return fail(CAP_ERR_STATE, "cap_debug_get: BVH not built");
        *value = ((uint64_t)(c->fan_pairs_nee.p ? c->fan_pair_nee_count : c->fan_pair_count) << 32) | c->fan_pair_count;
        return CAP_OK;
    case CAP_DEBUG_QUEUE_CANARY_BEHIND: return canary_count(c, true, value);
    case CAP_DEBUG_QUEUE_CANARY_USED: return canary_count(c, false, value);
    case CAP_DEBUG_WIDE_IN_USE:
        if (!c->bvh_ready) return fail(CAP_ERR_STATE, "cap_debug_get: BVH not built");
        *value = bvh_dev(c, c->lane[0]).wide8_ok;
        return CAP_OK;
    default:
        if (key >= CAP_DEBUG_SWITCH_BASE && key < CAP_DEBUG_SWITCH_BASE + SW_COUNT)
        {
            *value = (uint64_t)c->sw.v[key - CAP_DEBUG_SWITCH_BASE];
            return CAP_OK;
        }
        return fail(CAP_ERR_INVALID_ARG, "cap_debug_get: unknown key %u", key);
    }
}

int cap_set_bvh_build(CapContext* c, uint32_t mode)
{
    if (!c) return fail(CAP_ERR_INVALID_ARG, "cap_set_bvh_build: ctx is NULL");
    if (mode > CAP_BVH_BUILD_SAH_DEVICE) return fail(CAP_ERR_INVALID_ARG, "cap_set_bvh_build: unknown mode %u", mode);
    c->bvh_build_mode = mode;
    return CAP_OK;
}

int cap_set_traversal(CapContext* c, uint32_t mode)
{
    if (!c) return fail(CAP_ERR_INVALID_ARG, "cap_set_traversal: ctx is NULL");
    if (mode > CAP_TRAVERSAL_EXHAUSTIVE) return fail(CAP_ERR_INVALID_ARG, "cap_set_traversal: unknown mode %u", mode);
    c->traversal_mode = mode;
    return CAP_OK;
}

int cap_accum_reset(CapContext* c)
{
    if (!c) return fail(CAP_ERR_INVALID_ARG, "cap_accum_reset: ctx is NULL");
    HIP_TRY(hipSetDevice(c->device));
    if (c->accum.p) HIP_TRY(hipMemsetAsync(c->accum.p, 0, sizeof(float4) * c->accum.n, c->stream));
    c->frames_accumulated = 0;
    return CAP_OK;
}

int cap_accum_import(CapContext* c, const float* sum_rgba, uint64_t frames)
{
    if (!c || !sum_rgba) return fail(CAP_ERR_INVALID_ARG, "cap_accum_import: NULL argument");
    if (!c->screen.width) return fail(CAP_ERR_STATE, "cap_accum_import: resolution not set");
    HIP_TRY(hipSetDevice(c->device));
    if (sync_and_collect(c) != CAP_OK) return CAP_ERR_HIP;
    const size_t npix = (size_t)c->screen.width * c->screen.height;
    HIP_TRY(c->image_tmp.ensure(npix));
    HIP_TRY(c->accum.ensure(c->screen.pixels_padded));
    HIP_TRY(hipMemcpyAsync(c->image_tmp.p, sum_rgba, sizeof(float4) * npix, hipMemcpyHostToDevice, c->stream));
    LaunchCfg cfg{c->stream, (uint32_t)c->cu_count * 8u, 32};
    launch_tile(cfg, c->screen, c->image_tmp.p, c->accum.p);
    HIP_TRY(hipGetLastError());
    HIP_TRY(hipStreamSynchronize(c->stream));
    c->frames_accumulated = frames;
    return CAP_OK;
}

int cap_sync(CapContext* c)
{
    if (!c) return fail(CAP_ERR_INVALID_ARG, "cap_sync: ctx is NULL");
    HIP_TRY(hipSetDevice(c->device));
    return sync_and_collect(c);
}

int cap_render(CapContext* c, uint32_t frame_begin, uint32_t n_frames, uint32_t num_bounces, uint32_t flags)
{
    if (!c) return fail(CAP_ERR_INVALID_ARG, "cap_render: ctx is NULL");
    if (!c->bvh_ready) return fail(CAP_ERR_STATE, "cap_render: call cap_bvh_build first");
    if (c->bvh_stale) return fail(CAP_ERR_STATE, "cap_render: vertices changed; call cap_bvh_refit or cap_bvh_build");
    if (!c->camera_ready || !c->bluenoise_ready || !c->screen.width) return fail(CAP_ERR_STATE, "cap_render: camera, blue noise and resolution must be set");
    const bool ext = (flags & CAP_RENDER_EXT_MATERIALS) != 0;
    if (ext && !c->materials_ready) return fail(CAP_ERR_STATE, "cap_render: CAP_RENDER_EXT_MATERIALS needs cap_materials_upload (one material per mesh)");
    static_assert(sizeof(MaterialDev) == sizeof(CapMaterial), "material layouts must match");
    if (num_bounces > 255) return fail(CAP_ERR_INVALID_ARG, "cap_render: num_bounces %u exceeds 255", num_bounces);
    if (!n_frames) return CAP_OK;
    HIP_TRY(hipSetDevice(c->device));
    c->last_mark_form   = 0;
    c->last_sample_table = 0;
    c->last_terms        = CapContext::LastTerms{};
    const bool feedback = (flags & CAP_RENDER_GBUFFER_FEEDBACK) != 0;
    if (feedback)
    {
        if (ext) return fail(CAP_ERR_UNSUPPORTED, "cap_render: CAP_RENDER_GBUFFER_FEEDBACK is defined for the reference shading model only");
        if (n_frames != 1) return fail(CAP_ERR_INVALID_ARG, "cap_render: CAP_RENDER_GBUFFER_FEEDBACK renders one frame per call (n_frames is %u)", n_frames);
        if (!c->prev_camera_ready) return fail(CAP_ERR_STATE, "cap_render: CAP_RENDER_GBUFFER_FEEDBACK needs cap_prev_camera_set");
        if (c->post_w != c->screen.width || c->post_h != c->screen.height)
            if (int e = cap_post_reset(c)) return e;
    }

    const bool lowres = (flags & CAP_RENDER_LOWRES_INDIRECT) != 0;
    if (lowres)
    {
        if (ext) return fail(CAP_ERR_UNSUPPORTED, "cap_render: CAP_RENDER_LOWRES_INDIRECT is defined for the reference shading model only");
        if (n_frames != 1) return fail(CAP_ERR_INVALID_ARG, "cap_render: CAP_RENDER_LOWRES_INDIRECT renders one frame per call (n_frames is %u)", n_frames);
        if ((c->screen.width | c->screen.height) & 1u) return fail(CAP_ERR_INVALID_ARG, "cap_render: CAP_RENDER_LOWRES_INDIRECT needs even width and height (%ux%u)", c->screen.width, c->screen.height);
    }

    if (c->traversal_mode == CAP_TRAVERSAL_EXHAUSTIVE && c->tri_count > 4096)
        return fail(CAP_ERR_UNSUPPORTED, "cap_render: exhaustive traversal refused for %u triangles", c->tri_count);
    const bool     tree_path     = c->traversal_mode == CAP_TRAVERSAL_EXHAUSTIVE ? false
                                                                                 : !(c->traversal_mode == CAP_TRAVERSAL_AUTO && c->tri_count <= kExhaustiveMax);
    const uint32_t stack_entries = tree_path ? c->bvh_info.stack_entries : 0u;
    const bool     fused         = stack_entries == 0;

    const uint32_t    Ppad      = c->screen.pixels_padded;
    const BatchPolicy policy    = batch_policy(c, n_frames, num_bounces, flags, tree_path);
    const uint32_t    slots     = policy.slots;
    bool              two_lanes = policy.two_lanes;
    if (c->spans.size() > 2048 || c->pending.size() > 64 || c->post_marks.size() > 256)
        if (sync_and_collect(c) != CAP_OK) return CAP_ERR_HIP;
    const bool sample_table = fused && !ext && !feedback && num_bounces >= 1 && c->sw.get(SW_SAMPLE_TABLE, 1) != 0 &&
                              trace_shade_has_table_form(bvh_dev(c, c->lane[0]), scene_dev(c));
    c->last_sample_table = sample_table ? 1u : 0u;
    const LaneSizes need = lane_sizes(c, slots, num_bounces, sample_table);
    if (lane_grows(c->lane[0], need) || !c->accum.p || c->accum.n < Ppad) HIP_TRY(hipStreamSynchronize(c->stream));
    if (ensure_lane(c, c->lane[0], slots, num_bounces, sample_table) != CAP_OK || ensure_frame_buffers(c) != CAP_OK) return CAP_ERR_HIP;
    if (policy.lane1_failed_before)
    {
        size_t free_b = 0, total_b = 0;
        const bool room = hipMemGetInfo(&free_b, &total_b) == hipSuccess && free_b > (size_t)slots * Ppad * 256u;
        if (!room && (++c->lane1_retry_tick % 32u) != 0u)
        {
            two_lanes = false;
            ++c->stats.lane1_dropped;
        }
    }
    if (two_lanes)
    {
        if (lane_grows(c->lane[1], need))
        {
            HIP_TRY(hipStreamSynchronize(c->stream));
            if (c->stream2) HIP_TRY(hipStreamSynchronize(c->stream2));
        }
        if (c->debug_fail_lane || ensure_lane(c, c->lane[1], slots, num_bounces, sample_table) != CAP_OK || ensure_lane_streams(c) != CAP_OK)
        {
            (void)hipGetLastError();
            c->lane[1] = CapContext::Lane{};
            c->lane1_failed_paths = (uint64_t)slots * Ppad, c->lane1_failed_bounces = num_bounces;
            ++c->stats.lane1_dropped;
            two_lanes = false;
        }
    }
    c->lanes_last_render = two_lanes ? 2u : 1u;
    const uint32_t ring = c->frames_next;
    c->frames_next      = (c->frames_next + 1) % CapContext::kFrameRing;
    if (!c->frames_event[ring]) HIP_TRY(hipEventCreateWithFlags(&c->frames_event[ring], hipEventDisableTiming));
    HIP_TRY(hipEventSynchronize(c->frames_event[ring]));
    if (c->frames_ring[ring].n < n_frames)
    {
        HIP_TRY(c->frames_ring[ring].ensure(n_frames));
    }
    if (c->frames_pinned_n[ring] < n_frames)
    {
        if (c->frames_pinned[ring]) HIP_TRY(hipHostFree(c->frames_pinned[ring]));
        c->frames_pinned[ring] = nullptr;
        HIP_TRY(hipHostMalloc((void**)&c->frames_pinned[ring], sizeof(FrameConst) * n_frames, hipHostMallocDefault));
        c->frames_pinned_n[ring] = n_frames;
    }
    for (uint32_t f = 0; f < n_frames; ++f) c->frames_pinned[ring][f] = frame_const(frame_begin + f, lowres);
    HIP_TRY(hipMemcpyAsync(c->frames_ring[ring].p, c->frames_pinned[ring], sizeof(FrameConst) * n_frames, hipMemcpyHostToDevice, c->stream));
    const bool st = (flags & CAP_RENDER_STAGE_TIMERS) != 0;
    if (c->textures_dirty)
    {
        HIP_TRY(hipStreamSynchronize(c->stream));
        HIP_TRY(c->textures.ensure(std::max<size_t>(1, c->texture_host.size())));
        if (!c->texture_host.empty())
            HIP_TRY(hipMemcpy(c->textures.p, c->texture_host.data(), sizeof(TextureDev) * c->texture_host.size(), hipMemcpyHostToDevice));
        c->textures_dirty = false;
    }

    uint32_t blocks_per_cu = fused ? 6u : (stack_entries <= 32 ? 5u : 2u);
    if (c->sw.v[SW_BLOCKS_PER_CU] >= 0) blocks_per_cu = (uint32_t)std::max<int64_t>(1, c->sw.v[SW_BLOCKS_PER_CU]);
    const SceneDev  scene = scene_dev(c);
    const CameraDev cam   = camera_dev(c->camera);
    const uint32_t  D     = num_bounces;
    std::unique_ptr<StageTimer> total(new StageTimer(c, ST_COUNT));

    const uint32_t n_batches = (n_frames + slots - 1) / slots;
    struct LaneJoin
    {
        CapContext* c;
        bool        armed = false;
        ~LaneJoin()
        {
            if (!armed) return;
            if (hipEventRecord(c->join_ev, c->stream2) != hipSuccess || hipStreamWaitEvent(c->stream, c->join_ev, 0) != hipSuccess)
                (void)hipStreamSynchronize(c->stream2);
        }
    } lane_join{c};
    if (two_lanes)
    {
        HIP_TRY(hipEventRecord(c->fork_ev, c->stream));
        HIP_TRY(hipStreamWaitEvent(c->stream2, c->fork_ev, 0));
        lane_join.armed = true;
    }
    hipEvent_t last_resolve = nullptr;
    uint32_t   batch        = 0;

    for (uint32_t done = 0; done < n_frames; done += slots, ++batch)
    {
        const uint32_t    lane = two_lanes ? ((n_batches - 1u - batch) & 1u) : 0u;
        CapContext::Lane& L    = c->lane[lane];
        const BvhDev      bvh  = bvh_dev(c, L);
        LaunchCfg         cfg{L.stream, (uint32_t)c->cu_count * blocks_per_cu, stack_entries, (uint32_t)c->cu_count};
        cfg.sw = &c->sw;
        const uint32_t ns = std::min(slots, n_frames - done);
        const FrameConst* frames = c->frames_ring[ring].p + done;
        const size_t   per_queue     = (size_t)kQueueClasses * kCounterStride;
        const size_t   counter_words = (size_t)(D + 1) * per_queue;
        HIP_TRY(hipMemsetAsync(L.counters.p, 0, sizeof(uint32_t) * 3 * counter_words, L.stream));
        uint32_t*      ext_count = L.counters.p;
        uint32_t*      sh_count  = L.counters.p + 1;
        uint32_t*      work_shade = L.counters.p + counter_words;
        uint32_t*      work_any   = L.counters.p + 2 * counter_words;
        const uint32_t total_chunks   = ns * (Ppad >> 6);
        uint32_t       class_capacity = ((total_chunks + kQueueClasses - 1) / kQueueClasses) * 64u;
        if (c->debug_capacity_div > 1) class_capacity = std::max(64u, (class_capacity / c->debug_capacity_div) & ~63u);
        c->last_class_capacity = class_capacity;
        const bool     last_batch = done + ns >= n_frames;
        const uint32_t aov_slot   = ((flags & CAP_RENDER_AOV) && last_batch) ? ns - 1 : ~0u;
        const uint32_t max_count  = ns * Ppad;

        ShadeArgs sa{};
        sa.scene = scene, sa.cam = cam, sa.screen = c->screen, sa.frames = frames;
        if (!fused) sa.hits = L.hits.p;
        sa.planes = Planes{L.pl_color.p, L.pl_direct.p, L.pl_albedo.p, c->aov_geo.p, c->aov_nd.p};
        sa.n_slots = ns, sa.num_bounces = D, sa.max_count = max_count, sa.aov_slot = aov_slot, sa.shaded_counter = c->shaded_counter.p;
        {
            const bool no_cull = c->sw.on(SW_NO_CAMERA_CULL);
            auto dotf = [](const float* x, const float* y) { return x[0] * y[0] + x[1] * y[1] + x[2] * y[2]; };
            const CapCameraData& cd = c->camera;
            const float skew = std::max({std::fabs(dotf(cd.right, cd.up)), std::fabs(dotf(cd.right, cd.forward)), std::fabs(dotf(cd.up, cd.forward)),
                                         std::fabs(dotf(cd.right, cd.right) - 1.f), std::fabs(dotf(cd.up, cd.up) - 1.f),
                                         std::fabs(dotf(cd.forward, cd.forward) - 1.f)});
            const double f = cd.focal_length, sx = cd.sensor_size[0], sy = cd.sensor_size[1];
            const double shift_x = (double)skew * c->screen.width * (f / sx + 1.0 + sy / (2.0 * sx) + (sx + sy) / (4.0 * f));
            const double shift_y = (double)skew * c->screen.height * (f / sy + 1.0 + sx / (2.0 * sy) + (sx + sy) / (4.0 * f));
            const bool   ortho   = skew < 1e-4f && shift_x <= 0.125 * (double)kCameraCullPad && shift_y <= 0.125 * (double)kCameraCullPad;
            sa.cull_camera_pairs = (ortho && !no_cull) ? 1u : 0u;
            c->last_cull_camera_pairs = sa.cull_camera_pairs;
        }
        const bool no_albedo_w = c->sw.on(SW_NO_ALBEDO_IN_W);
        sa.albedo_in_w = (!no_albedo_w && !feedback && !lowres && !(flags & CAP_RENDER_AOV) && (ext || scene.texture_count == 0)) ? 1u : 0u;
        const bool no_plane_code = c->sw.on(SW_NO_PLANE_CODE);
        sa.code_in_color = (sa.albedo_in_w && fused && !ext && !no_plane_code && trace_shade_has_code_form(bvh, scene)) ? 1u : 0u;
        if (feedback)
            sa.fb = FeedbackDev{camera_dev(c->prev_camera), c->post_prev_nd.p, c->post_chist[(frame_begin + 1) % 2].p};
        const bool no_inline_nee = c->sw.on(SW_NO_INLINE_NEE);
        sa.inline_nee = (ext && fused && !no_inline_nee) ? 1u : 0u;
        const bool no_inline_probe = c->sw.on(SW_NO_INLINE_PROBE);
        sa.inline_probe = (!ext && !feedback && fused && !no_inline_probe && c->tri_count <= kExhaustiveMax && bvh.fan_pair_count >= 1 &&
                           bvh.fan_pair_count <= kExhaustiveMax / 2)
                              ? 1u
                              : 0u;
        const bool no_wave_ring = c->sw.on(SW_NO_WAVE_RING);
        sa.wave_ring = (sa.inline_probe && !no_wave_ring && (size_t)cfg.grid_blocks * (kBlock / 64) * 128 <= std::min(L.s_org.n, L.s_con.n)) ? 1u : 0u;
        LaunchCfg cfg_any    = cfg;
        cfg_any.any_no_probe = sa.inline_probe;
        bool primary_shaded = false;
        bool any_refill = false;
        if (!fused && !ext && bvh.wide8_ok && c->tri_count > kExhaustiveMax)
        {
            const int force = (int)c->sw.v[SW_ANY_REFILL];
            const uint64_t tree_bytes = (uint64_t)c->wide8_nodes * kWideNodeStride * 4u + (uint64_t)c->tri_count * 64u;
            any_refill = force >= 0 ? force != 0 : tree_bytes >= kAnyRefillTreeBytes;
        }
        bool primary_wide = false;
        if (!fused && bvh.wide8_ok && c->tri_count > kExhaustiveMax)
        {
            const int force = (int)c->sw.v[SW_PRIMARY_WIDE];
            bool inside = true;
            for (int k = 0; k < 3; ++k)
                inside = inside && c->camera.position[k] >= c->bvh_info.bounds_lo[k] && c->camera.position[k] <= c->bvh_info.bounds_hi[k];
            const double per_pixel = (double)c->tri_count / std::max(1.0, (double)c->screen.width * c->screen.height);
            primary_wide = inside && (force >= 0 ? force != 0 : per_pixel >= kPrimaryWideTrianglesPerPixel);
        }
        if (sample_table)
        {
            launch_sample_terms(L.stream, scene.bluenoise, frames, ns, D, L.terms.p);
            c->last_terms = CapContext::LastTerms{frames, ns, D, lane};
            if (trace_launch(c, "sample_terms batch %u", batch)) return fail(CAP_ERR_HIP, "sample_terms failed");
        }
        for (uint32_t b = 0; b <= D; ++b)
        {
            const int pi = (int)(b & 1u), po = pi ^ 1;
            sa.bounce    = b;
            if (fused) sa.sample_terms = sample_table ? L.terms.p + (size_t)(b < D ? b : 0u) * ns * 4096 : nullptr;
            sa.in        = RayQueue{L.q_org[pi].p, L.q_dir[pi].p, L.q_thr[pi].p, b ? ext_count + (b - 1) * per_queue : nullptr, class_capacity,
                                    pi ? L.s_dir.p : L.s_org.p};
            sa.out       = RayQueue{L.q_org[po].p, L.q_dir[po].p, L.q_thr[po].p, ext_count + b * per_queue, class_capacity,
                                    po ? L.s_dir.p : L.s_org.p};
            sa.shadow    = ShadowQueue{L.s_org.p, L.s_dir.p, L.s_con.p, sh_count + b * per_queue, class_capacity};
            sa.work      = work_shade + b * per_queue;
            if (fused)
            {
                StageTimer t(c, b == 0 ? ST_PRIMARY : ST_CLOSEST, st);
                const uint32_t form = launch_trace_shade(cfg, bvh, sa, ext, feedback);
                if (b) ++c->stats.launches_trace_closest, c->last_mark_form = form;
                if (trace_launch(c, "trace_shade bounce %u batch %u", b, batch)) return fail(CAP_ERR_HIP, "trace_shade failed");
            }
            else
            {
                if (b == 0)
                {
                    {
                        StageTimer t(c, ST_PRIMARY, st);
                        if (primary_wide)
                        {
                            const uint32_t id_cap = (((max_count + kQueueClasses - 1) / kQueueClasses) + 63u) & ~63u;
                            const RayQueue idq{L.q_org[0].p, L.q_dir[0].p, nullptr, L.counters.p + 3 * counter_words, id_cap, nullptr};
                            if (c->sw.on(SW_RAYGEN_KERNEL) || bvh.tri_count == 0)
                            {
                                launch_raygen_identity(cfg, cam, c->screen, frames, ns, idq);
                                launch_trace_closest8(cfg, bvh, idq, max_count, L.hits.p, sa.work);
                            }
                            else
                                launch_trace_closest8_camera(cfg, bvh, idq, max_count, L.hits.p, sa.work, cam, c->screen, frames, ns);
                        }
                        else
                        {
                            primary_shaded = launch_primary_shade(cfg, bvh, sa, L.hits.p, ext);
                            if (!primary_shaded) launch_trace_primary(cfg, bvh, cam, c->screen, frames, ns, L.hits.p, sa.work);
                        }
                    }
                    if (aov_slot != ~0u) launch_geo_aov(cfg, scene, L.hits.p + (size_t)aov_slot * Ppad, Ppad, c->aov_geo.p);
                }
                if (b != 0 || !primary_shaded)
                {
                    StageTimer t(c, ST_SHADE, st, b == 0 ? ST_DIRECT : ST_NONE);
                    launch_shade(cfg, sa, ext, feedback);
                    ++c->stats.launches_shade;
                }
            }
            if (!sa.inline_nee && !(fused && sa.wave_ring && b != 0))
            {
                StageTimer t(c, ST_ANY, st, b == 0 ? ST_DIRECT : ST_NONE);
                if (any_refill)
                    launch_trace_any8_refill(cfg_any, bvh, sa.shadow, max_count, b == 0 ? L.pl_direct.p : L.pl_color.p, Ppad, ns, c->shaded_counter.p,
                                             work_any + b * per_queue, frames);
                else
                    launch_trace_any(cfg_any, bvh, sa.shadow, max_count, b == 0 ? L.pl_direct.p : L.pl_color.p, Ppad, ns, c->shaded_counter.p,
                                     work_any + b * per_queue,  ext, frames,
                                     (b == 0 && sa.code_in_color) ? L.pl_color.p : nullptr);
                ++c->stats.launches_trace_any;
                if (trace_launch(c, "trace_any bounce %u batch %u", b, batch)) return fail(CAP_ERR_HIP, "trace_any failed");
            }
            if (!fused && b < D)
            {
                StageTimer t(c, ST_CLOSEST, st);
                if (bvh.wide8_ok)
                    launch_trace_closest8(cfg, bvh, sa.out, max_count, L.hits.p, work_shade + (b + 1) * per_queue);
                else
                    launch_trace_closest(cfg, bvh, sa.out, max_count, L.hits.p);
                ++c->stats.launches_trace_closest;
            }
        }
        if (!lowres)
        {
            StageTimer t(c, ST_RESOLVE, st);
            if (two_lanes && last_resolve) HIP_TRY(hipStreamWaitEvent(L.stream, last_resolve, 0));
            launch_resolve(cfg, sa.planes, ns, Ppad, c->accum.p, sa.albedo_in_w != 0u, scene.kd_untextured, sa.code_in_color != 0u);
            if (two_lanes)
            {
                HIP_TRY(hipEventRecord(c->lane_ev[lane], L.stream));
                last_resolve = c->lane_ev[lane];
            }
        }
        uint32_t* pinned = nullptr;
        if (!c->pinned_pool.empty())
        {
            pinned = c->pinned_pool.back();
            c->pinned_pool.pop_back();
        }
        else
            HIP_TRY(hipHostMalloc((void**)&pinned, sizeof(uint32_t) * 2 * 256 * kQueueClasses * kCounterStride, hipHostMallocDefault));
        HIP_TRY(hipMemcpyAsync(pinned, L.counters.p, sizeof(uint32_t) * counter_words, hipMemcpyDeviceToHost, L.stream));
        c->pending.push_back({pinned, D | (sa.inline_nee ? 1u << 16 : 0u)});
        HIP_TRY(hipGetLastError());

        uint64_t valid = 0;
        for (uint32_t lt = 0; lt < c->screen.local_tiles; ++lt)
        {
            const uint32_t gt = lt * c->screen.shard_count + c->screen.shard_index;
            const uint32_t ty = gt / c->screen.tiles_x, tx = gt % c->screen.tiles_x;
            const uint32_t w = std::min(kTileDim, c->screen.width - tx * kTileDim), h = std::min(kTileDim, c->screen.height - ty * kTileDim);
            valid += (uint64_t)w * h;
        }
        c->stats.rays_primary += valid * ns;
        c->stats.frames += ns;
        if (!lowres) c->frames_accumulated += ns;
        c->last_slots = ns;
        c->aov_valid  = aov_slot != ~0u;
        c->aov_lowres = lowres;
        c->aov_frame  = frame_begin + done + ns - 1;
        if (c->spans.size() > 4096)
        {
            total.reset();
            if (two_lanes) HIP_TRY(hipStreamSynchronize(c->stream2));
            if (sync_and_collect(c) != CAP_OK) return CAP_ERR_HIP;
            total.reset(new StageTimer(c, ST_COUNT));
        }
    }
    if (two_lanes)
    {
        HIP_TRY(hipEventRecord(c->join_ev, c->stream2));
        HIP_TRY(hipStreamWaitEvent(c->stream, c->join_ev, 0));
        lane_join.armed = false;
    }
    total.reset();
    HIP_TRY(hipEventRecord(c->frames_event[ring], c->stream));
    return CAP_OK;
}

int cap_readback(CapContext* c, CapBufferKind kind, float* dst)
{
    if (!c || !dst) return fail(CAP_ERR_INVALID_ARG, "cap_readback: NULL argument");
    if (!c->screen.width) return fail(CAP_ERR_STATE, "cap_readback: resolution not set");
    HIP_TRY(hipSetDevice(c->device));
    if (sync_and_collect(c) != CAP_OK) return CAP_ERR_HIP;
    const size_t npix = (size_t)c->screen.width * c->screen.height;
    HIP_TRY(c->image_tmp.ensure(npix));
    HIP_TRY(hipMemsetAsync(c->image_tmp.p, 0, sizeof(float4) * npix, c->stream));
    LaunchCfg cfg{c->stream, (uint32_t)c->cu_count * 8u, 32};
    const bool is_aov = kind <= CAP_BUF_COMBINED || kind == CAP_BUF_INDIRECT_LOWRES;
    if (is_aov && !c->aov_valid) return fail(CAP_ERR_STATE, "cap_readback: no frame rendered with CAP_RENDER_AOV");
    if (!is_aov && !c->accum.p) return fail(CAP_ERR_STATE, "cap_readback: nothing rendered");
    const AovPlanes aov = aov_planes(c);
    switch (kind)
    {
    case CAP_BUF_GBUFFER_GEO: launch_untile(cfg, c->screen, c->aov_geo.p, nullptr, nullptr, 0, c->image_tmp.p); break;
    case CAP_BUF_NORMAL_DEPTH: launch_untile(cfg, c->screen, c->aov_nd.p, nullptr, nullptr, 0, c->image_tmp.p); break;
    case CAP_BUF_DIRECT: launch_untile(cfg, c->screen, aov.direct, nullptr, nullptr, 0, c->image_tmp.p); break;
    case CAP_BUF_ALBEDO: launch_untile(cfg, c->screen, aov.albedo, nullptr, nullptr, 0, c->image_tmp.p); break;
    case CAP_BUF_INDIRECT: launch_untile(cfg, c->screen, aov.color, nullptr, nullptr, 0, c->image_tmp.p); break;
    case CAP_BUF_COMBINED:
        launch_untile(cfg, c->screen, aov.color, aov.albedo, aov.direct, 1, c->image_tmp.p);
        break;
    case CAP_BUF_ACCUM_SUM: launch_untile(cfg, c->screen, c->accum.p, nullptr, nullptr, 0, c->image_tmp.p); break;
    case CAP_BUF_ACCUM_MEAN: launch_untile(cfg, c->screen, c->accum.p, nullptr, nullptr, 2, c->image_tmp.p); break;
    case CAP_BUF_INDIRECT_LOWRES:
    {
        if (!c->aov_lowres) return fail(CAP_ERR_STATE, "cap_readback: the last CAP_RENDER_AOV frame was not rendered with CAP_RENDER_LOWRES_INDIRECT");
        launch_untile(cfg, c->screen, aov.color, nullptr, nullptr, 0, c->image_tmp.p);
        HIP_TRY(c->post_itemp.ensure(npix));
        launch_decimate2x(c->stream, c->image_tmp.p, c->screen.width, c->screen.height, (c->aov_frame % 4u) / 2u, (c->aov_frame % 4u) % 2u,
                          c->post_itemp.p);
        HIP_TRY(hipGetLastError());
        HIP_TRY(hipMemcpyAsync(dst, c->post_itemp.p, sizeof(float4) * (npix / 4), hipMemcpyDeviceToHost, c->stream));
        HIP_TRY(hipStreamSynchronize(c->stream));
        return CAP_OK;
    }
    default: return fail(CAP_ERR_INVALID_ARG, "cap_readback: unknown buffer kind %d", (int)kind);
    }
    HIP_TRY(hipGetLastError());
    HIP_TRY(hipMemcpyAsync(dst, c->image_tmp.p, sizeof(float4) * npix, hipMemcpyDeviceToHost, c->stream));
    HIP_TRY(hipStreamSynchronize(c->stream));
    return CAP_OK;
}

int cap_stats_get(CapContext* c, CapStats* out)
{
    if (!c || !out) return fail(CAP_ERR_INVALID_ARG, "cap_stats_get: NULL argument");
    HIP_TRY(hipSetDevice(c->device));
    if (sync_and_collect(c) != CAP_OK) return CAP_ERR_HIP;
    *out = c->stats;
    return CAP_OK;
}

int cap_stats_reset(CapContext* c)
{
    if (!c) return fail(CAP_ERR_INVALID_ARG, "cap_stats_reset: ctx is NULL");
    HIP_TRY(hipSetDevice(c->device));
    if (sync_and_collect(c) != CAP_OK) return CAP_ERR_HIP;
    c->stats = CapStats{};
    if (c->shaded_counter.p) HIP_TRY(hipMemsetAsync(c->shaded_counter.p, 0, kGuardWords * sizeof(uint64_t), c->stream));
    return CAP_OK;
}

int cap_tile_buffer_floats(CapContext* c, size_t* out_floats)
{
    if (!c || !out_floats) return fail(CAP_ERR_INVALID_ARG, "cap_tile_buffer_floats: NULL argument");
    if (!c->screen.width) return fail(CAP_ERR_STATE, "cap_tile_buffer_floats: resolution not set");
    *out_floats = (size_t)c->screen.pixels_padded * 4;
    return CAP_OK;
}

int cap_resolve_tiles(CapContext* c, float* device_dst)
{
    if (!c || !device_dst) return fail(CAP_ERR_INVALID_ARG, "cap_resolve_tiles: NULL argument");
    if (!c->accum.p) return fail(CAP_ERR_STATE, "cap_resolve_tiles: nothing rendered");
    HIP_TRY(hipSetDevice(c->device));
    LaunchCfg cfg{c->stream, (uint32_t)c->cu_count * 8u, 32};
    launch_tiles_mean(cfg, c->accum.p, c->screen.pixels_padded, reinterpret_cast<float4*>(device_dst));
    HIP_TRY(hipGetLastError());
    return CAP_OK;
}

int cap_assemble_tiles(CapContext* c, const float* device_src, uint32_t shard_count, float* device_image)
{
    if (!c || !device_src || !device_image) return fail(CAP_ERR_INVALID_ARG, "cap_assemble_tiles: NULL argument");
    if (shard_count != c->screen.shard_count) return fail(CAP_ERR_INVALID_ARG, "cap_assemble_tiles: shard_count %u != context's %u", shard_count, c->screen.shard_count);
    HIP_TRY(hipSetDevice(c->device));
    LaunchCfg cfg{c->stream, (uint32_t)c->cu_count * 8u, 32};
    launch_assemble(cfg, c->screen, reinterpret_cast<const float4*>(device_src), shard_count, reinterpret_cast<float4*>(device_image));
    HIP_TRY(hipGetLastError());
    return CAP_OK;
}
}
```

### capsaicin_amd/csrc/small_scene.hip

```cpp
#include "cap_shade.h"

#include <cassert>

namespace cap
{
#ifndef CAP_TS_FIRST
#define CAP_TS_FIRST 5
#endif
#ifndef CAP_TS_EXT
#define CAP_TS_EXT 6
#endif
#ifndef CAP_TS_NEXT
#define CAP_TS_NEXT 6
#endif
#ifdef CAP_STAMPS
__device__ unsigned long long g_wave_times[2 * 16384];
#endif
template <bool FIRST_, bool EXT_, bool FB_, bool LDS_, bool TAME_, bool CODE_ = false, bool TAB_ = false>
struct TraceShadeCfg
{
    static_assert(!TAME_ || (!EXT_ && !FB_ && LDS_), "TAME: reference model, scene in LDS");
    static_assert(!CODE_ || (FIRST_ && TAME_), "CODE: bounce 0 of the reference model, scene in LDS, tame records");
    static_assert(!TAB_ || (TAME_ && kChunkLean), "TAB: the lean kernels (reference model, scene in LDS, tame records)");
    static constexpr bool FIRST = FIRST_, EXT = EXT_, FB = FB_, LDS = LDS_, TAME = TAME_, CODE = CODE_, TAB = TAB_;
    static constexpr bool CARRY = !EXT && !TAB, SKY_RMW = false;
    static constexpr bool PROBE = !EXT && !FB && LDS;
    static constexpr bool LEAN = PROBE && TAME && kChunkLean;
    static constexpr bool ORG  = FIRST && LDS;
    static constexpr bool XT   = EXT && LDS;
    static constexpr int  kBlocksPerCu = FB ? 4 : (EXT ? (FIRST ? 5 : CAP_TS_EXT) : (FIRST ? CAP_TS_FIRST : CAP_TS_NEXT));
};

__device__ __forceinline__ void stage_scene_records(const BvhDev& bvh, const ShadeArgs& a, float4* lds_shade, float4* lds_rec)
{
    const uint32_t n = bvh.tri_count <= kExhaustiveMax ? bvh.tri_count : kExhaustiveMax;
    for (uint32_t k = threadIdx.x; k < kShadeRec * n; k += kBlock) lds_shade[k] = a.scene.shade_tris[k];
    for (uint32_t k = threadIdx.x; k < 4 * n; k += kBlock) lds_rec[k] = bvh.tris_by_id[k];
}
__device__ __forceinline__ void stage_ext_tables(const ShadeArgs& a, float* lds_mat, float* lds_lcdf, float4* lds_lrec)
{
    const float* ms = reinterpret_cast<const float*>(a.scene.materials);
    for (uint32_t k = threadIdx.x; k < 12u * a.scene.material_count; k += kBlock) lds_mat[k] = ms[k];
    for (uint32_t k = threadIdx.x; k < a.scene.light_count; k += kBlock)
    {
        lds_lcdf[k] = a.scene.light_cdf[k];
        const float4* lt = a.scene.shade_tris + kShadeRec * (size_t)a.scene.light_tris[k];
        const float4  l0 = lt[0], l1 = lt[1], l2 = lt[2];
        const v3      q0 = mk3(l0.x, l0.y, l0.z), q1 = mk3(l1.x, l1.y, l1.z), q2 = mk3(l2.x, l2.y, l2.z);
        const v3      nl = normalize3(cross3(q1 - q0, q2 - q0));
        const MaterialDev lm = a.scene.materials[f2u(lt[6].x)];
        lds_lrec[4 * k]     = make_float4(q0.x, q0.y, q0.z, lm.ke[0]);
        lds_lrec[4 * k + 1] = make_float4(q1.x, q1.y, q1.z, lm.ke[1]);
        lds_lrec[4 * k + 2] = make_float4(q2.x, q2.y, q2.z, lm.ke[2]);
        lds_lrec[4 * k + 3] = make_float4(nl.x, nl.y, nl.z, 0.f);
    }
}
__device__ __forceinline__ void stage_camera_pairs(const BvhDev& bvh, const ShadeArgs& a, float4* lds_org, float4* lds_bounds)
{
    const v3     o  = mk3(a.cam.position[0], a.cam.position[1], a.cam.position[2]);
    const float* fp = reinterpret_cast<const float*>(bvh.fan_pairs);
    for (uint32_t k = threadIdx.x; k < bvh.fan_pair_count && 2 * k + 1 < kExhaustiveMax; k += kBlock)
    {
        const float* rec  = fp + 20 * (size_t)k;
        const v3     tvec = o - mk3(rec[0], rec[1], rec[2]);
        lds_org[2 * k]     = make_float4(tvec.x, tvec.y, tvec.z, dot3(tvec, mk3(rec[12], rec[13], rec[14])));
        lds_org[2 * k + 1] = make_float4(dot3(tvec, mk3(rec[15], rec[16], rec[17])), 0.f, 0.f, 0.f);
        const v3 R = mk3(a.cam.right[0], a.cam.right[1], a.cam.right[2]), U = mk3(a.cam.up[0], a.cam.up[1], a.cam.up[2]),
                 F = mk3(a.cam.forward[0], a.cam.forward[1], a.cam.forward[2]);
        float x0 = 3.0e38f, y0 = 3.0e38f, x1 = -3.0e38f, y1 = -3.0e38f;
        bool  behind = false;
        for (int e = 0; e < 4; ++e)
        {
            const v3    d = e == 0 ? tvec * -1.0f : (mk3(rec[3 * e], rec[3 * e + 1], rec[3 * e + 2]) - tvec);
            const float z = dot3(d, F);
            behind |= !(z > 1e-4f);
            const float px = ((a.cam.focal_length * dot3(d, R) / z) / a.cam.sensor_x + 0.5f) * (float)a.screen.width;
            const float py = ((a.cam.focal_length * dot3(d, U) / z) / a.cam.sensor_y + 0.5f) * (float)a.screen.height;
            x0 = fminf(x0, px), x1 = fmaxf(x1, px), y0 = fminf(y0, py), y1 = fmaxf(y1, py);
        }
        const bool usable = a.cull_camera_pairs != 0u && !behind && x0 == x0 && y0 == y0 && x1 == x1 && y1 == y1;
        lds_bounds[k] = usable ? make_float4(x0 - kCameraCullPad, y0 - kCameraCullPad, x1 + kCameraCullPad, y1 + kCameraCullPad) : make_float4(-3.0e38f, -3.0e38f, 3.0e38f, 3.0e38f);
    }
}
__device__ __forceinline__ void stage_probe_rows(const BvhDev& bvh, const ShadeArgs& a, float* lds_pscore, uint32_t& probe_k, float4* lds_probe)
{
    const uint32_t np = bvh.fan_pair_count;
    const float*   fp = reinterpret_cast<const float*>(bvh.fan_pairs);
    if (threadIdx.x < np)
    {
        const float* rec = fp + 20 * (size_t)threadIdx.x;
        const v3     L   = mk3(a.frames[0].light_dir[0], a.frames[0].light_dir[1], a.frames[0].light_dir[2]);
        const v3     v0  = mk3(rec[0], rec[1], rec[2]);
        float        sc  = dot3(v0, L);
        for (int e = 0; e < 3; ++e) sc += dot3(v0 + mk3(rec[3 + 3 * e], rec[4 + 3 * e], rec[5 + 3 * e]), L);
        lds_pscore[threadIdx.x] = sc;
    }
    __syncthreads();
    if (threadIdx.x < np)
    {
        const float sc   = lds_pscore[threadIdx.x];
        uint32_t    rank = 0;
        for (uint32_t j = 0; j < np; ++j)
        {
            const float o = lds_pscore[j];
            rank += (o > sc || (o == sc && j < threadIdx.x)) ? 1u : 0u;
        }
        if (rank == 0) probe_k = threadIdx.x;
    }
    __syncthreads();
    const float* rec = fp + 20 * (size_t)probe_k;
    for (uint32_t sl = threadIdx.x; sl < a.n_slots && sl < kMaxFrameSlots; sl += kBlock)
    {
        const v3 d = mk3(a.frames[sl].light_dir[0], a.frames[sl].light_dir[1], a.frames[sl].light_dir[2]);
        lds_probe[2 * sl]     = tri_pre(d, mk3(rec[12], rec[13], rec[14]), kRayEps, kRayFar);
        lds_probe[2 * sl + 1] = tri_pre(d, mk3(rec[15], rec[16], rec[17]), kRayEps, kRayFar);
    }
}

template <bool FIRST, bool EXT, bool FB = false, bool LDS = false, bool TAME = false, bool CODE = false>
__global__ __launch_bounds__(kBlock, (TraceShadeCfg<FIRST, EXT, FB, LDS, TAME, CODE>::kBlocksPerCu)) void k_trace_shade(BvhDev bvh, ShadeArgs a)
{
    using C            = TraceShadeCfg<FIRST, EXT, FB, LDS, TAME, CODE>;
    constexpr bool TAB = false;
#include "small_scene_body.h"
}
template <bool FIRST, bool CODE>
__global__ __launch_bounds__(kBlock, (TraceShadeCfg<FIRST, false, false, true, true, CODE, kChunkLean>::kBlocksPerCu)) void k_trace_shade_tab(BvhDev bvh, ShadeArgs a)
{
    using C            = TraceShadeCfg<FIRST, false, false, true, true, CODE, kChunkLean>;
    constexpr bool EXT = false, FB = false, LDS = true, TAB = kChunkLean;
#include "small_scene_body.h"
}

#ifdef CAP_STAMPS
extern "C" int cap_debug_stamps(unsigned long long* out, int reset)
{
    if (reset == 2) return (int)hipMemcpyFromSymbol(out, HIP_SYMBOL(g_wave_times), 2 * 16384 * sizeof(unsigned long long));
    hipError_t e = hipMemcpyFromSymbol(out, HIP_SYMBOL(g_stamps), 8 * sizeof(unsigned long long));
    if (e == hipSuccess && reset)
    {
        unsigned long long z[16] = {};
        e = hipMemcpyToSymbol(HIP_SYMBOL(g_stamps), z, sizeof(z));
    }
    return (int)e;
}
#endif

__device__ __forceinline__ uint32_t selftest_hash32(uint32_t x)
{
    x ^= x >> 16, x *= 0x7feb352du, x ^= x >> 15, x *= 0x846ca68bu, x ^= x >> 16;
    return x;
}
__global__ __launch_bounds__(kBlock) void k_shade_forms_selftest(unsigned long long* out, uint32_t which)
{
    const uint32_t     tid = blockIdx.x * kBlock + threadIdx.x, total = gridDim.x * kBlock;
    unsigned long long bad = 0, n = 0;
    auto               differ = [](float x, float y) { return f2u(x) != f2u(y) ? 1u : 0u; };
    if (which == 0)
    {
        for (uint64_t b = ((127ull - 96ull) << 23) + tid; b <= 0x7f7fffffull; b += total)
        {
            const float x = u2f((uint32_t)b), s = sqrtf(x);
            bad += differ(sqrt_pos(x), s) + differ(sqrt_unscaled(x), s), n += 2;
        }
        if (tid < 3)
        {
            const float x = tid == 0 ? 0.0f : (tid == 1 ? -0.0f : __builtin_inff());
            bad += differ(sqrt_unscaled(x), sqrtf(x)), ++n;
        }
        for (uint64_t b = (uint64_t)f2u(kNormLo) + tid; b <= f2u(kNormHi); b += total)
        {
            const float x = u2f((uint32_t)b);
            bad += differ(div_unscaled(1.0f, sqrt_pos(x)), 1.0f / sqrtf(x)), ++n;
        }
        for (uint64_t b = tid; b <= f2u(2.0f); b += total)
        {
            const float x = u2f((uint32_t)b), pdf = x / kPi, fast = div_unscaled(x, kPi);
            if (b == 0 || b >= ((127ull - 80ull) << 23))
                bad += differ(fast, pdf);
            else
                bad += (fast < 1e-5f && fast > -1e-5f) ? 0u : 1u;
            ++n;
            if (!(pdf < 1e-5f)) bad += differ(div_unscaled(kInvPi * fmaxf(x, 0.0f), pdf), (kInvPi * fmaxf(x, 0.0f)) / pdf), ++n;
        }
    }
    else
    {
        for (uint64_t i = tid; i < (1ull << 31); i += total)
        {
            const uint32_t h0 = selftest_hash32((uint32_t)i), h1 = selftest_hash32((uint32_t)i ^ 0x9e3779b9u), h2 = selftest_hash32(h0 + h1);
            const uint32_t e1 = 82u + h2 % 90u, d = (h2 >> 8) % 96u, e0 = e1 > d ? e1 - d : 1u;
            float          p = u2f((e1 << 23) | (h0 & 0x007fffffu) | ((h2 << 3) & 0x80000000u));
            float          q = u2f((e0 << 23) | (h1 & 0x007fffffu) | ((h2 << 2) & 0x80000000u));
            if ((h2 >> 24 & 7u) == 0u) q = (h2 & 0x08000000u) ? 0.0f : -0.0f;
            const bool  sw = (h2 >> 27 & 1u) != 0u;
            const float a = sw ? q : p, b = sw ? p : q, g = fmaf(a, a, b * b);
            if (!ortho_in_range(a, b, g)) continue;
            const float k = sqrtf(g), kf = sqrt_pos(g);
            float       qa, qb;
            div2_unscaled(a, b, kf, qa, qb);
            bad += differ(kf, k) + differ(qa, a / k) + differ(qb, b / k), ++n;
        }
    }
    if (bad) atomicAdd(&out[0], bad);
    atomicAdd(&out[1], n);
}

void launch_shade_forms_selftest(hipStream_t stream, unsigned long long* out_device, uint32_t which)
{
    hipLaunchKernelGGL(k_shade_forms_selftest, dim3(4096), dim3(kBlock), 0, stream, out_device, which);
}

__global__ __launch_bounds__(kBlock) void k_sample_terms(const float2* bluenoise, const FrameConst* frames, uint32_t n_slots, uint32_t num_bounces, float4* table)
{
    const uint32_t tid = blockIdx.x * kBlock + threadIdx.x, row = tid >> 12, at = tid & 4095u;
    if (row >= n_slots * num_bounces) return;
    const uint32_t b = row / n_slots, sl = row - b * n_slots;
    const uint32_t count = frames[sl].frame_count * 25u + b;
    float          r1, r2;
    bluenoise_at(bluenoise, bluenoise_base(at & 63u, at >> 6), bluenoise_offset(count), bluenoise_shift(count), r1, r2);
    const HemiTerms h = hemisphere_terms(r1, r2);
    table[tid]        = make_float4(h.ca, h.cb, h.cos_theta, 0.0f);
}

void launch_sample_terms(hipStream_t stream, const float2* bluenoise, const FrameConst* frames, uint32_t n_slots, uint32_t num_bounces, float4* table)
{
    const uint32_t rows = n_slots * num_bounces;
    if (!rows) return;
    hipLaunchKernelGGL(k_sample_terms, dim3(rows * (4096u / kBlock)), dim3(kBlock), 0, stream, bluenoise, frames, n_slots, num_bounces, table);
}

__global__ __launch_bounds__(kBlock) void k_sample_terms_selftest(const float2* bluenoise, const FrameConst* frames, uint32_t n_slots, uint32_t num_bounces,
                                                                  const float4* table, unsigned long long* out)
{
    const uint32_t tid = blockIdx.x * kBlock + threadIdx.x, row = tid >> 12, at = tid & 4095u;
    if (row >= n_slots * num_bounces) return;
    const uint32_t b = row / n_slots, sl = row - b * n_slots;
    float          r1, r2;
    bluenoise4x4(bluenoise, at & 63u, at >> 6, frames[sl].frame_count * 25u + b, r1, r2);
    const HemiTerms h = hemisphere_terms(r1, r2);
    const float4    q = table[tid];
    const bool      bad = f2u(q.x) != f2u(h.ca) || f2u(q.y) != f2u(h.cb) || f2u(q.z) != f2u(h.cos_theta) || f2u(q.w) != 0u;
    const unsigned long long mb = __ballot(bad), mn = __ballot(true);
    if ((threadIdx.x & 63u) == 0u)
    {
        if (mb) atomicAdd(&out[0], (unsigned long long)__popcll(mb));
        atomicAdd(&out[1], (unsigned long long)__popcll(mn));
    }
}

void launch_sample_terms_selftest(hipStream_t stream, const float2* bluenoise, const FrameConst* frames, uint32_t n_slots, uint32_t num_bounces,
                                  const float4* table, unsigned long long* out_device)
{
    const uint32_t rows = n_slots * num_bounces;
    if (!rows) return;
    hipLaunchKernelGGL(k_sample_terms_selftest, dim3(rows * (4096u / kBlock)), dim3(kBlock), 0, stream, bluenoise, frames, n_slots, num_bounces, table, out_device);
}

enum : uint32_t { TS_FIRST = 1, TS_EXT = 2, TS_FB = 4, TS_LDS = 8, TS_TAME = 16, TS_CODE = 32, TS_TAB = 64 };
struct TraceShadeKernel
{
    uint32_t is;
    void (*kernel)(BvhDev, ShadeArgs);
};
template <uint32_t IS>
constexpr TraceShadeKernel trace_shade_kernel()
{
    if constexpr ((IS & TS_TAB) != 0)
    {
        static_assert((IS & ~(TS_FIRST | TS_CODE)) == (TS_LDS | TS_TAME | TS_TAB), "TAB: the lean kernels");
        return {IS, k_trace_shade_tab<(IS & TS_FIRST) != 0, (IS & TS_CODE) != 0>};
    }
    else
        return {IS, k_trace_shade<(IS & TS_FIRST) != 0, (IS & TS_EXT) != 0, (IS & TS_FB) != 0, (IS & TS_LDS) != 0, (IS & TS_TAME) != 0, (IS & TS_CODE) != 0>};
}
constexpr TraceShadeKernel kTraceShadeKernels[16] = {
    trace_shade_kernel<TS_FIRST | TS_LDS | TS_TAME | TS_CODE>(),
    trace_shade_kernel<TS_FIRST | TS_EXT | TS_LDS>(), trace_shade_kernel<TS_FIRST | TS_EXT>(),
    trace_shade_kernel<TS_FIRST | TS_LDS | TS_TAME>(), trace_shade_kernel<TS_FIRST | TS_LDS>(), trace_shade_kernel<TS_FIRST>(),
    trace_shade_kernel<TS_EXT | TS_LDS>(), trace_shade_kernel<TS_EXT>(),
    trace_shade_kernel<TS_FB | TS_LDS>(), trace_shade_kernel<TS_FB>(),
    trace_shade_kernel<TS_LDS | TS_TAME>(), trace_shade_kernel<TS_LDS>(), trace_shade_kernel<0>(),
    trace_shade_kernel<TS_FIRST | TS_LDS | TS_TAME | TS_CODE | TS_TAB>(), trace_shade_kernel<TS_FIRST | TS_LDS | TS_TAME | TS_TAB>(), trace_shade_kernel<TS_LDS | TS_TAME | TS_TAB>(),
};

static bool tame_kernels(const BvhDev& bvh, const SceneDev& scene)
{
#if defined(CAP_SHADE_IEEE)
    return false;
#else
    return bvh.tri_count <= kExhaustiveMax && scene.shade_tame != 0;
#endif
}
bool trace_shade_has_code_form(const BvhDev& bvh, const SceneDev& scene) { return tame_kernels(bvh, scene); }
bool trace_shade_has_table_form(const BvhDev& bvh, const SceneDev& scene) { return kChunkLean && tame_kernels(bvh, scene); }

uint32_t launch_trace_shade(const LaunchCfg& cfg, const BvhDev& bvh, const ShadeArgs& args, bool ext, bool feedback)
{
    const bool first = args.bounce == 0;
    const bool fb    = feedback && !ext && !first;
    const bool lds   = bvh.tri_count <= kExhaustiveMax;
    const bool tame  = !ext && !fb && tame_kernels(bvh, args.scene);
    const bool code  = first && args.code_in_color != 0u;
    assert(!code || tame);
    const bool tab = args.sample_terms != nullptr;
    assert(!tab || (tame && kChunkLean));
    const uint32_t is = (first ? TS_FIRST : 0u) | (ext ? TS_EXT : 0u) | (fb ? TS_FB : 0u) | (lds ? TS_LDS : 0u) | (tame ? TS_TAME : 0u) | (code ? TS_CODE : 0u) | (tab ? TS_TAB : 0u);
    const uint32_t gx = queue_grid(cfg, first ? args.screen.pixels_padded * args.n_slots : args.max_count);
    const TraceShadeKernel* k = kTraceShadeKernels;
    while (k->is != is && k + 1 < kTraceShadeKernels + 16) ++k;
    assert(k->is == is);
    hipLaunchKernelGGL(k->kernel, dim3(gx), dim3(kBlock), 0, cfg.stream, bvh, args);
#if defined(CAP_CLOSEST_V1)
    return 0u;
#else
    if (!lds || first) return 0u;
    return (kMarkCarry && bvh.tri_ids_dense) ? (bvh.tri_count > 32u ? 3u : 2u) : 1u;
#endif
}
}
```

### capsaicin_amd/csrc/small_scene_body.h

```cpp
    const uint32_t Ppad     = a.screen.pixels_padded;
    const uint32_t cps      = Ppad >> 6;
    const uint32_t chunks   = FIRST ? cps * a.n_slots : (a.in.class_capacity >> 6) * kQueueClasses;
    uint32_t       n_shaded = 0, n_probed = 0;
    __shared__ FrameConst lds_frames[kMaxFrameSlots];
    __shared__ float4     lds_shade[LDS ? kShadeRec * kExhaustiveMax : 1];
    __shared__ float4     lds_rec[LDS ? 4 * kExhaustiveMax : 1];
    __shared__ float4     lds_probe[C::PROBE ? 2 * kMaxFrameSlots : 1];
    __shared__ float      lds_pscore[C::PROBE ? kExhaustiveMax / 2 : 1];
    __shared__ SlotSample lds_first[(C::LEAN && FIRST && !TAB) ? kMaxFrameSlots : 1];
    __shared__ uint32_t   lds_probe_k;
    __shared__ float4     lds_ring[(C::PROBE && !FIRST) ? (kBlock / 64) * kWaveRing : 1];
    __shared__ float4     lds_org[C::ORG ? kExhaustiveMax : 1];
    __shared__ float4     lds_bounds[C::ORG ? kExhaustiveMax / 2 : 1];
    __shared__ float      lds_mat[C::XT ? 12 * kExhaustiveMax : 1];
    __shared__ float      lds_lcdf[C::XT ? kExtLightsMax : 1];
    __shared__ float4     lds_lrec[C::XT ? 4 * kExtLightsMax : 1];
    const bool            ext_tabs = C::XT && a.scene.material_count <= kExhaustiveMax && a.scene.light_count <= kExtLightsMax;
    if (LDS)
    {
        stage_scene_records(bvh, a, lds_shade, lds_rec);
        if (C::XT && ext_tabs) stage_ext_tables(a, lds_mat, lds_lcdf, lds_lrec);
        if (C::ORG) stage_camera_pairs(bvh, a, lds_org, lds_bounds);
    }
    if (C::PROBE && a.inline_probe) stage_probe_rows(bvh, a, lds_pscore, lds_probe_k, lds_probe);
    if constexpr (C::LEAN)
        stage_frames_samples<FIRST, TAB>(a, lds_frames, lds_first);
    else
        stage_frames(a, lds_frames);
    ProbeArgs probe;
    if (C::PROBE && a.inline_probe) probe.rows = lds_probe, probe.pairs = bvh.fan_pairs, probe.k = lds_probe_k;
    uint32_t ring_head = 0, ring_n = 0;
    if (C::PROBE && !FIRST && a.inline_probe && a.wave_ring)
    {
        probe.ring_org = lds_ring + (threadIdx.x >> 6) * kWaveRing;
        probe.ring_con = a.shadow.contrib_pid + (size_t)wave_global_id() * kWaveRing;
    }
    auto trace_ring = [&](uint32_t count) {
        wave_handoff();
        const uint32_t lane_ = threadIdx.x & 63u;
        const bool     on    = lane_ < count;
        const uint32_t pos   = (ring_head + lane_) & (kWaveRing - 1u);
        float4         o     = make_float4(0.f, 0.f, 0.f, 0.f);
        if (on) o = probe.ring_org[pos];
        const uint32_t spid = f2u(o.w);
        const bool     good = on && (spid >> kPidShift) < a.n_slots && (spid & kPidMask) < Ppad;
        const FrameConst& fc = lds_frames[good ? (spid >> kPidShift) : 0u];
        const Ray  sr = make_ray(mk3(o.x, o.y, o.z), mk3(fc.light_dir[0], fc.light_dir[1], fc.light_dir[2]), kRayEps, good ? kRayFar : kRayEps);
        float4* const target = a.bounce == 0 ? a.planes.direct : a.planes.color;
        const size_t  idx    = good ? (size_t)(spid >> kPidShift) * Ppad + (spid & kPidMask) : 0;
        float4        c = make_float4(0.f, 0.f, 0.f, 0.f), cur = c;
        if (good) c = probe.ring_con[pos], cur = target[idx];
        const bool occluded = exhaustive_any<false>(bvh, sr);
        if (good && !occluded) target[idx] = make_float4(cur.x + c.x, cur.y + c.y, cur.z + c.z, cur.w);
        ring_head = (ring_head + count) & (kWaveRing - 1u);
        ring_n -= count;
    };
    const float4* shade_tab = LDS ? lds_shade : a.scene.shade_tris;
    const float4* rec_tab   = LDS ? lds_rec : bvh.tris_by_id;
    ExtTables     xtabs;
    if (C::XT && ext_tabs) xtabs.materials = reinterpret_cast<const MaterialDev*>(lds_mat), xtabs.light_cdf = lds_lcdf, xtabs.light_rec = lds_lrec;
    Stamps st;
    st.start();
    const uint32_t my_class = wave_global_id() % kQueueClasses;
    const uint32_t lane     = threadIdx.x & 63u;
    uint32_t       n_class  = 0;
    if (!FIRST)
    {
        n_class = a.in.count[my_class * kCounterStride];
        n_class = n_class < a.in.class_capacity ? n_class : a.in.class_capacity;
    }
    uint32_t grab = grab_issue(a.work, my_class);
    while (true)
    {
        const uint32_t j = grab_value(grab);
        uint32_t       i, pid = 0, slot = 0;
        const uint32_t klass = my_class;
        bool           active;
        v3             thr = mk3(1.0f, 1.0f, 1.0f);
        Ray            r   = make_ray(mk3(0.f, 0.f, 0.f), mk3(0.f, 0.f, 1.f), 0.0f, 0.0f);
        float          carried_r1 = 0.f, carried_r2 = 0.f;
        if (FIRST)
        {
            const uint32_t chunk = class_chunk(j, my_class);
            if (chunk >= chunks) break;
            grab   = grab_issue(a.work, my_class);
            slot   = chunk / cps;
            i      = (chunk - slot * cps) * 64 + lane;
            active = true;
            pid    = (slot << kPidShift) | i;
            uint32_t x, y;
            if (local_pixel_to_xy(a.screen, i, x, y))
                r = make_ray(mk3(a.cam.position[0], a.cam.position[1], a.cam.position[2]),
                             primary_dir(a.cam, a.screen, lds_frames[slot], x, y), 0.0f, kPrimaryFar);
        }
        else
        {
            if (j * 64u >= n_class) break;
            active = j * 64u + lane < n_class;
            if constexpr (C::LEAN)
            {
                const uint32_t local = j * 64u + lane;
                i                    = my_class * a.in.class_capacity + (local < n_class ? local : n_class - 1u);
                const float4 o = a.in.org_tmin[i], d = a.in.dir_tmax[i], tp = a.in.thr_pid[i];
                grab = grab_issue(a.work, my_class);
                r    = make_ray(mk3(o.x, o.y, o.z), mk3(d.x, d.y, d.z), kRayEps, kRayFar);
                thr  = mk3(tp.x, tp.y, tp.z), pid = f2u(tp.w);
                if (!TAB) carried_r1 = o.w, carried_r2 = d.w;
            }
            else
            {
                i      = my_class * a.in.class_capacity + j * 64u + lane;
                float4 o = make_float4(0.f, 0.f, 0.f, 0.f), d = make_float4(0.f, 0.f, 1.f, 0.f), tp = make_float4(1.f, 1.f, 1.f, 0.f);
                if (active) o = a.in.org_tmin[i], d = a.in.dir_tmax[i], tp = a.in.thr_pid[i];
                grab = grab_issue(a.work, my_class);
                if (active)
                {
                    r   = make_ray(mk3(o.x, o.y, o.z), mk3(d.x, d.y, d.z), kRayEps, kRayFar);
                    thr = mk3(tp.x, tp.y, tp.z), pid = f2u(tp.w);
                    carried_r1 = o.w, carried_r2 = d.w;
                }
            }
        }
        float    t, u, v;
        uint32_t gid;
        STAMP(st, 0, true);
        uint32_t pair_mask = ~0u;
        if (C::ORG)
        {
            uint32_t tx = 0, ty = 0;
            (void)local_pixel_to_xy(a.screen, i & ~63u, tx, ty);
            const float4 b    = lds_bounds[lane < kExhaustiveMax / 2 ? lane : 0u];
            const bool   over = lane < bvh.fan_pair_count && b.x < (float)(tx + 8u) && b.z >= (float)tx && b.y < (float)(ty + 8u) && b.w >= (float)ty;
            pair_mask         = (uint32_t)__ballot(over);
        }
        __builtin_amdgcn_s_setprio(0);
#if !defined(CAP_CLOSEST_V1)
        if constexpr (LDS && !C::ORG)
        {
            if (bvh.tri_count > 32u)
                exhaustive_closest_marked<true>(bvh, rec_tab, r, active, t, u, v, gid);
            else
                exhaustive_closest_marked<false>(bvh, rec_tab, r, active, t, u, v, gid);
        }
        else
#endif
            exhaustive_closest<C::ORG, !LDS>(bvh, rec_tab, r, t, u, v, gid, lds_org, pair_mask);
        __builtin_amdgcn_s_setprio(3);
        STAMP(st, 1, true);
        const ShadePre pre = shade_prefetch<C>(a, lds_frames, active, pid, carried_r1, carried_r2, lds_first);
        if (FIRST && slot == a.aov_slot)
        {
            float4 g = make_float4(0.f, 0.f, u2f(kInvalidId), u2f(kInvalidId));
            if (gid != kInvalidId)
            {
                const uint4 id = a.scene.tri_ids[gid];
                g              = make_float4(u, v, u2f(id.x), u2f(id.y));
            }
            a.planes.aov_geo[i] = g;
        }
        if constexpr (EXT)
        {
            if (a.inline_nee)
            {
                v3 acc = mk3(0.f, 0.f, 0.f);
                if (!FIRST && active)
                {
                    const float4 q = a.in.acc[i];
                    acc            = mk3(q.x, q.y, q.z);
                }
                shade_vertex_ext<FIRST, true>(a, shade_tab, pre, klass, pid, make_float4(u, v, u2f(gid), t), thr, r.d, n_shaded, &bvh, acc, xtabs);
            }
            else
                shade_vertex_ext<FIRST>(a, shade_tab, pre, klass, pid, make_float4(u, v, u2f(gid), t), thr, r.d, n_shaded, nullptr, mk3(0.f, 0.f, 0.f), xtabs);
        }
        else
        {
            shade_vertex<C>(a, shade_tab, pre, klass, pid, make_float4(u, v, u2f(gid), t), thr, n_shaded, st, probe, &n_probed, ring_head, &ring_n);
            if (C::PROBE && ring_n >= 64u) trace_ring(64u);
        }
        STAMP(st, 4, false);
    }
    if (!FIRST && !EXT && !FB) st.flush();
#ifdef CAP_STAMPS
    if (!FIRST && !EXT && !FB && (threadIdx.x & 63u) == 0 && wave_global_id() < 16384)
    {
        g_wave_times[2 * wave_global_id() + 0] = st.t_begin;
        g_wave_times[2 * wave_global_id() + 1] = __builtin_amdgcn_s_memrealtime();
    }
#endif
    if (C::PROBE && ring_n != 0u) trace_ring(ring_n);
    flush_stats(a.out.count + (size_t)my_class * kCounterStride, n_shaded, n_probed);
```

### include/capsaicin_hip.h

```cpp
#ifndef CAPSAICIN_HIP_H
#define CAPSAICIN_HIP_H

#include <stddef.h>
#include <stdint.h>

#ifdef __cplusplus
extern "C" {
#endif

typedef struct CapContext CapContext;

typedef enum CapStatus
{
    CAP_OK                = 0,
    CAP_ERR_INVALID_ARG   = 1,
    CAP_ERR_HIP           = 2,
    CAP_ERR_STATE         = 3,
    CAP_ERR_UNSUPPORTED   = 4,
    CAP_ERR_IO            = 5
} CapStatus;

typedef struct CapCameraData
{
    float position[3];
    float focal_length;
    float right[3];
    float znear;
    float forward[3];
    float focus_distance;
    float up[3];
    float aperture;
    float sensor_size[2];
} CapCameraData;

typedef struct CapMeshDesc
{
    uint32_t vertex_count;
    uint32_t first_vertex_offset;
    uint32_t index_count;
    uint32_t first_index_offset;
    uint32_t index;
    uint32_t texture_index;
    uint32_t padding[2];
} CapMeshDesc;

typedef struct CapMaterial
{
    float kd[3];
    float roughness;
    float ks[3];
    float pad0;
    float ke[3];
    float pad1;
} CapMaterial;

enum
{
    CAP_RENDER_AOV           = 1u << 0,
    CAP_RENDER_EXT_MATERIALS = 1u << 1,
    CAP_RENDER_STAGE_TIMERS  = 1u << 2,
    CAP_RENDER_GBUFFER_FEEDBACK = 1u << 3,
    CAP_RENDER_LOWRES_INDIRECT = 1u << 4
};

typedef enum CapBufferKind
{
    CAP_BUF_GBUFFER_GEO  = 0,
    CAP_BUF_DIRECT       = 1,
    CAP_BUF_ALBEDO       = 2,
    CAP_BUF_NORMAL_DEPTH = 3,
    CAP_BUF_INDIRECT     = 4,
    CAP_BUF_COMBINED     = 5,
    CAP_BUF_ACCUM_SUM    = 6,
    CAP_BUF_ACCUM_MEAN   = 7,
    CAP_BUF_INDIRECT_LOWRES = 8
} CapBufferKind;

typedef struct CapStats
{
    uint64_t rays_primary;
    uint64_t rays_extension;
    uint64_t rays_shadow;
    uint64_t shaded_vertices;
    uint64_t frames;
    double   ms_total;
    double   ms_primary;
    double   ms_trace_closest;
    double   ms_trace_any;
    double   ms_shade;
    double   ms_resolve;
    uint64_t launches_trace_closest;
    uint64_t launches_trace_any;
    uint64_t launches_shade;
    uint64_t rays_extension_bounce0;
    uint64_t rays_shadow_bounce0;
    uint64_t guard_shade;
    uint64_t guard_trace_any;
    uint64_t guard_last;
    double   ms_post;
    uint64_t post_frames;
    double   ms_direct;
    double   ms_post_pass[5];
    uint64_t shadow_entries;
    uint64_t shadow_entries_bounce0;
    uint64_t guard_append;
    uint64_t lane1_dropped;
} CapStats;

typedef struct CapBvhInfo
{
    uint32_t triangle_count;
    uint32_t node_count;
    uint32_t max_depth;
    uint32_t stack_entries;
    float    bounds_lo[3];
    float    bounds_hi[3];
    double   build_ms;
} CapBvhInfo;

const char* cap_last_error(void);
int cap_device_count(void);

int  cap_ctx_create(int device_id, void* hip_stream, CapContext** out_ctx);
void cap_ctx_destroy(CapContext* ctx);

int cap_scene_upload(CapContext* ctx, const float* positions, const float* normals, const float* texcoords,
                     const uint32_t* indices, const CapMeshDesc* meshes, uint32_t vertex_count, uint32_t index_count,
                     uint32_t mesh_count);
int cap_texture_upload(CapContext* ctx, uint32_t index, const uint8_t* rgba8, uint32_t width, uint32_t height);
int cap_bluenoise_upload(CapContext* ctx, const uint8_t* rgba8_256x256);
int cap_materials_upload(CapContext* ctx, const CapMaterial* materials, uint32_t mesh_count);

int cap_bvh_build(CapContext* ctx);
typedef enum CapBvhBuild
{
    CAP_BVH_BUILD_AUTO = 0,
    CAP_BVH_BUILD_LBVH = 1,
    CAP_BVH_BUILD_SAH  = 2,
    CAP_BVH_BUILD_PLOC = 3,
    CAP_BVH_BUILD_SAH_DEVICE = 4
} CapBvhBuild;
int cap_set_bvh_build(CapContext* ctx, uint32_t mode);
int cap_bvh_info(CapContext* ctx, CapBvhInfo* out);
int cap_bvh_readback(CapContext* ctx, float* nodes, uint32_t* leaf_triangles);
int cap_bvh_wide_readback(CapContext* ctx, uint32_t* nodes, uint32_t* tri_src, uint32_t* info);

enum
{
    CAP_VERTICES_DEVICE = 1u << 0
};
int cap_scene_update_vertices(CapContext* ctx, const float* positions, const float* normals, const float* texcoords, uint32_t flags);
typedef struct CapRefitInfo
{
    double ms;
    double expected_node_visits;
    double expected_node_visits_built;
} CapRefitInfo;
int cap_bvh_refit(CapContext* ctx, CapRefitInfo* out);

int cap_camera_set(CapContext* ctx, const CapCameraData* camera);
int cap_prev_camera_set(CapContext* ctx, const CapCameraData* camera);
int cap_set_resolution(CapContext* ctx, uint32_t width, uint32_t height);
int cap_set_shard(CapContext* ctx, uint32_t shard_index, uint32_t shard_count);
int cap_set_batch_paths(CapContext* ctx, uint64_t max_paths);
enum
{
    CAP_DEBUG_QUEUE_CAPACITY_DIV = 1,
    CAP_DEBUG_WIDE_DEPTH_LIMIT   = 2,
    CAP_DEBUG_WIDE_IN_USE        = 3,
    CAP_DEBUG_FAIL_LANE1         = 4,
    CAP_DEBUG_LANES_USED         = 5,
    CAP_DEBUG_QUEUE_CANARY_FILL   = 6,
    CAP_DEBUG_QUEUE_CANARY_BEHIND = 7,
    CAP_DEBUG_QUEUE_CANARY_USED   = 8,
    CAP_DEBUG_SELFTEST_DIV        = 9,
    CAP_DEBUG_NEE_PAIRS           = 10,
    CAP_DEBUG_SELFTEST_SHADE_UNARY = 11,
    CAP_DEBUG_SELFTEST_SHADE_DIV2  = 12,
    CAP_DEBUG_SHADE_TAME           = 13,
    CAP_DEBUG_CAMERA_CULL          = 14,
    CAP_DEBUG_MARK_FORM            = 15,
    CAP_DEBUG_SAMPLE_TABLE          = 16,
    CAP_DEBUG_SELFTEST_SAMPLE_TABLE = 17,
    CAP_DEBUG_SWITCH_BASE         = 64
};
int cap_debug_set(CapContext* ctx, uint32_t key, uint64_t value);
int cap_debug_get(CapContext* ctx, uint32_t key, uint64_t* value);
int cap_debug_switch_index(const char* name);
int cap_debug_pair_ids_dense(const float* pair_records, uint32_t pair_count, uint32_t single_count, uint32_t tri_count);
int cap_debug_query_ranges(uint64_t n, uint32_t count, const uint64_t* base, const uint64_t* stride, const uint32_t* align);
int cap_debug_closest_instance_bound(const float* transform, const float* box_lo, const float* box_hi, const float* point, float best_dist2,
                                     float* world_to_object, float* g, float* xw, float* slack, uint32_t* skip);
typedef enum CapTraversal
{
    CAP_TRAVERSAL_AUTO       = 0,
    CAP_TRAVERSAL_STACK      = 1,
    CAP_TRAVERSAL_EXHAUSTIVE = 2
} CapTraversal;
int cap_set_traversal(CapContext* ctx, uint32_t mode);

int cap_render(CapContext* ctx, uint32_t frame_begin, uint32_t n_frames, uint32_t num_bounces, uint32_t flags);
int cap_accum_reset(CapContext* ctx);
int cap_accum_import(CapContext* ctx, const float* sum_rgba, uint64_t frames);
int cap_sync(CapContext* ctx);

int cap_readback(CapContext* ctx, CapBufferKind kind, float* dst);

int cap_stats_get(CapContext* ctx, CapStats* out);
int cap_stats_reset(CapContext* ctx);

typedef struct CapRayDesc
{
    float origin[3];
    float tmin;
    float direction[3];
    float tmax;
} CapRayDesc;
typedef struct CapHit
{
    float    t;
    float    u;
    float    v;
    uint32_t triangle;
} CapHit;
int cap_trace_rays(CapContext* ctx, const CapRayDesc* device_rays, uint64_t n, CapHit* device_hits, uint32_t flags);
int cap_trace_occlusion(CapContext* ctx, const CapRayDesc* device_rays, uint64_t n, uint32_t* device_occluded, uint32_t flags);

#define CAP_MULTI_MAX_K 16
enum
{
    CAP_MULTI_CONTINUE = 1u << 0
};
int cap_trace_rays_multi(CapContext* ctx, const CapRayDesc* device_rays, uint64_t n, uint32_t k, CapHit* device_hits, uint32_t* device_counts,
                         uint32_t flags);

enum
{
    CAP_RAY_FLAG_ACCEPT_FIRST_HIT  = 0x04,
    CAP_RAY_FLAG_CULL_BACK_FACING  = 0x10,
    CAP_RAY_FLAG_CULL_FRONT_FACING = 0x20
};
typedef struct CapTraceOptions
{
    uint32_t ray_flags;
    uint32_t instance_mask;
    uint32_t reserved[2];
} CapTraceOptions;
int cap_scene_set_instance_masks(CapContext* ctx, const uint8_t* masks, uint32_t mesh_count);
int cap_trace_rays_ex(CapContext* ctx, const CapRayDesc* device_rays, uint64_t n, CapHit* device_hits, const CapTraceOptions* options);
int cap_trace_occlusion_ex(CapContext* ctx, const CapRayDesc* device_rays, uint64_t n, uint32_t* device_occluded,
                           const CapTraceOptions* options);
int cap_trace_rays_multi_ex(CapContext* ctx, const CapRayDesc* device_rays, uint64_t n, uint32_t k, CapHit* device_hits,
                            uint32_t* device_counts, uint32_t multi_flags, const CapTraceOptions* options);

typedef struct CapPointDesc
{
    float point[3];
    float radius;
} CapPointDesc;
typedef struct CapClosest
{
    float    point[3];
    float    dist2;
    float    u, v;
    uint32_t triangle;
    uint32_t feature;
} CapClosest;
enum
{
    CAP_FEATURE_FACE = 0,
    CAP_FEATURE_EDGE_V0V1 = 1,
    CAP_FEATURE_EDGE_V1V2 = 2,
    CAP_FEATURE_EDGE_V2V0 = 3,
    CAP_FEATURE_V0 = 4,
    CAP_FEATURE_V1 = 5,
    CAP_FEATURE_V2 = 6
};
int cap_closest_points(CapContext* ctx, const CapPointDesc* device_points, uint64_t n, CapClosest* device_out,
                       const CapTraceOptions* options );

int cap_closest_points_multi(CapContext* ctx, const CapPointDesc* device_points, uint64_t n, uint32_t k, CapClosest* device_out,
                             uint32_t* device_counts, uint32_t multi_flags, const CapTraceOptions* options );

#define CAP_INSTANCE_MAX_CONDITION 4096.0
#define CAP_INSTANCE_MAX_COUNT (1u << 24)
typedef struct CapInstanceDesc
{
    float    transform[12];
    uint32_t mask;
    uint32_t reserved[3];
} CapInstanceDesc;
enum
{
    CAP_INSTANCES_DEVICE = 1u << 0
};
typedef struct CapInstancesInfo
{
    uint32_t count, inert, tlas_nodes, tlas_depth;
    double   ms;
} CapInstancesInfo;
int cap_instances_set(CapContext* ctx, const CapInstanceDesc* descs, uint32_t count, uint32_t flags, CapInstancesInfo* out );
int cap_instances_set_ex(CapContext* ctx, const CapInstanceDesc* descs, const uint32_t* object_index , uint32_t count,
                         uint32_t flags, CapInstancesInfo* out );
int cap_instances_readback(CapContext* ctx, float* world_to_object, float* world_boxes);
int cap_trace_instances(CapContext* ctx, const CapRayDesc* device_rays, uint64_t n, CapHit* device_hits, uint32_t* device_instances,
                        const CapTraceOptions* options );
int cap_trace_instances_occlusion(CapContext* ctx, const CapRayDesc* device_rays, uint64_t n, uint32_t* device_occluded,
                                  const CapTraceOptions* options );
int cap_trace_instances_multi(CapContext* ctx, const CapRayDesc* device_rays, uint64_t n, uint32_t k, CapHit* device_hits,
                              uint32_t* device_instances, uint32_t* device_counts, uint32_t multi_flags,
                              const CapTraceOptions* options );

int cap_closest_instances(CapContext* ctx, const CapPointDesc* device_points, uint64_t n, CapClosest* device_out,
                          uint32_t* device_instances , const CapTraceOptions* options );

int cap_closest_instances_multi(CapContext* ctx, const CapPointDesc* device_points, uint64_t n, uint32_t k, CapClosest* device_out,
                                uint32_t* device_instances, uint32_t* device_counts, uint32_t multi_flags,
                                const CapTraceOptions* options );

typedef struct CapPseudonormalsInfo
{
    uint32_t vertices;
    uint32_t edges;
    uint32_t boundary_edges;
    uint32_t nonmanifold_edges;
    uint32_t inconsistent_edges;
    uint32_t degenerate_triangles;
    uint32_t closed;
    uint32_t reserved;
    double   ms;
} CapPseudonormalsInfo;
int cap_pseudonormals_build(CapContext* ctx, CapPseudonormalsInfo* out );
int cap_pseudonormals_drop(CapContext* ctx);
int cap_pseudonormals_readback(CapContext* ctx, float* host_normals );
int cap_signed_distance(CapContext* ctx, const CapPointDesc* device_points, uint64_t n, CapClosest* device_out, float* device_signed,
                        const CapTraceOptions* options );

int cap_signed_distance_instances(CapContext* ctx, const CapPointDesc* device_points, uint64_t n, CapClosest* device_out,
                                  uint32_t* device_instances , float* device_signed,
                                  const CapTraceOptions* options );

typedef struct CapWindingInfo
{
    uint32_t inner_nodes;
    uint32_t degenerate_triangles;
    double   total_area;
    float    root_n[3];
    float    root_p[3];
    double   ms;
} CapWindingInfo;
int cap_winding_build(CapContext* ctx, CapWindingInfo* out );
int cap_winding_drop(CapContext* ctx);
int cap_winding_readback(CapContext* ctx, float* host_table );
int cap_winding_numbers(CapContext* ctx, const CapPointDesc* device_points, uint64_t n, float beta, float* device_winding,
                        uint32_t* device_visits );

#define CAP_OBJECT_MAX_COUNT 4096u
typedef struct CapObjectRange
{
    uint32_t first_mesh, mesh_count;
} CapObjectRange;
typedef struct CapObjectInfo
{
    uint32_t first_triangle, triangle_count, node_count, max_depth;
    float    bounds_lo[3], bounds_hi[3];
    uint32_t builder;
    uint32_t reserved;
} CapObjectInfo;
typedef struct CapObjectsInfo
{
    uint32_t count, triangles, nodes, max_depth;
    double   ms;
} CapObjectsInfo;
int cap_objects_set(CapContext* ctx, const CapObjectRange* ranges , uint32_t count, CapObjectsInfo* out );
int cap_objects_info(CapContext* ctx, CapObjectInfo* out, uint32_t capacity, uint32_t* count_out);

int cap_tile_buffer_floats(CapContext* ctx, size_t* out_floats);
int cap_resolve_tiles(CapContext* ctx, float* device_dst);
int cap_assemble_tiles(CapContext* ctx, const float* device_src, uint32_t shard_count, float* device_image);

#define CAP_COMM_ID_BYTES 128
int cap_comm_unique_id(uint8_t* id_128_bytes);
int cap_comm_init_rank(CapContext* ctx, const uint8_t* id_128_bytes, uint32_t rank, uint32_t nranks);
int cap_comm_gather_frame(CapContext* ctx);
int cap_comm_init_all(CapContext* const* ctxs, uint32_t n);
int cap_comm_gather_frame_all(CapContext* const* ctxs, uint32_t n);
int cap_comm_image(CapContext* ctx, float** device_image);
int cap_comm_readback(CapContext* ctx, float* dst);
int cap_comm_info(CapContext* ctx, uint32_t* rank, uint32_t* size, uint32_t* uses_rccl);
int cap_comm_destroy(CapContext* ctx);
int cap_comm_abort(CapContext* ctx);

typedef struct CapPostSettings
{
    int32_t gather;
    int32_t denoise;
    int32_t eaw5;
    float   eaw_normal_sigma;
    float   eaw_depth_sigma;
    float   eaw_luma_sigma;
    float   gather_normal_sigma;
    float   gather_depth_sigma;
    float   gather_luma_sigma;
    float   temporal_upscale_feedback;
    float   taa_feedback;
    int32_t lowres_indirect;
    int32_t disable_variance;
    int32_t fast_weights;
    int32_t output;
} CapPostSettings;
enum
{
    CAP_OUTPUT_COMBINED = 0,
    CAP_OUTPUT_DIRECT   = 1,
    CAP_OUTPUT_INDIRECT = 2,
    CAP_OUTPUT_VARIANCE = 3
};
void cap_post_settings_default(CapPostSettings* out);
int cap_post_frame(CapContext* ctx, const CapPostSettings* settings, uint32_t frame_count, const CapCameraData* prev_camera);
int cap_aov_tile_buffer_floats(CapContext* ctx, size_t* out_floats);
int cap_resolve_aov_tiles(CapContext* ctx, float* device_dst);
int cap_post_frame_gathered(CapContext* ctx, const CapPostSettings* settings, uint32_t frame_count, const CapCameraData* prev_camera,
                            const float* device_gathered, uint32_t shard_count);
int cap_feedback_buffer_floats(CapContext* ctx, size_t* out_floats);
int cap_feedback_export(CapContext* ctx, float* device_dst);
int cap_feedback_import(CapContext* ctx, const float* device_src, uint32_t frame_count);
int cap_post_reset(CapContext* ctx);
int cap_post_readback(CapContext* ctx, float* dst);

#ifdef __cplusplus
}
#endif
#endif
```

Before: 57900 Mrays/s.

## Precompute camera vertices per jitter group and shade bounce zero from a table

Groups frames in a batch by identical Halton jitter on the host and stores each group's index in spare frame-constant fields. A new kernel computes primary hit position, normal and material code once per group into a per-lane table. A new head variant of the lean trace-shade kernel then performs bounce-zero direct lighting, shadow probing and the first extension ray from that table, replacing the fused primary kernel. This aims to avoid redundant primary traversal and shorten the bounce-zero kernel, at the cost of extra table memory, an extra launch and a more complex shading path.

```diff
diff --git a/capsaicin_amd/capi.py b/capsaicin_amd/capi.py
--- a/capsaicin_amd/capi.py
+++ b/capsaicin_amd/capi.py
@@ -593,6 +593,8 @@
     DEBUG_MARK_FORM = 15
     DEBUG_SAMPLE_TABLE = 16
     DEBUG_SELFTEST_SAMPLE_TABLE = 17
+    DEBUG_CAMERA_TABLE = 18
+    DEBUG_SELFTEST_CAMERA_TABLE = 19
 
     def debug_set(self, key, value):
         _check(lib().cap_debug_set(self.ctx, key, value), "cap_debug_set")
diff --git a/capsaicin_amd/csrc/cap_context.h b/capsaicin_amd/csrc/cap_context.h
--- a/capsaicin_amd/csrc/cap_context.h
+++ b/capsaicin_amd/csrc/cap_context.h
@@ -184,6 +184,12 @@
         const FrameConst* frames = nullptr;
         uint32_t          n_slots = 0, num_bounces = 0, lane = 0;
     } last_terms;
+    uint32_t      last_camera_table = 0;
+    struct LastCamera
+    {
+        const FrameConst* frames = nullptr;
+        uint32_t          n_slots = 0, n_groups = 0, lane = 0;
+    } last_camera;
     uint32_t      last_cull_camera_pairs = 0;
     uint32_t      traversal_mode  = CAP_TRAVERSAL_AUTO;
     uint32_t      bvh_build_mode  = CAP_BVH_BUILD_AUTO;
@@ -194,6 +200,7 @@
     {
         hipStream_t      stream = nullptr;
         DevBuf<float4>   hits, q_org[2], q_dir[2], q_thr[2], s_org, s_dir, s_con, pl_color, pl_direct, pl_albedo;
+        DevBuf<float4>   camera;
         DevBuf<float4>   terms;
         DevBuf<uint32_t> counters;
         DevBuf<uint32_t> stack_spill;
diff --git a/capsaicin_amd/csrc/cap_kernels.h b/capsaicin_amd/csrc/cap_kernels.h
--- a/capsaicin_amd/csrc/cap_kernels.h
+++ b/capsaicin_amd/csrc/cap_kernels.h
@@ -37,6 +37,7 @@
     SW_RAYGEN_KERNEL,
     SW_NO_PLANE_CODE,
     SW_SAMPLE_TABLE,
+    SW_NO_CAMERA_TABLE,
     SW_COUNT
 };
 struct SwitchTable
@@ -253,12 +254,15 @@
 constexpr float kCameraCullPad = 2.0f;
 void launch_shade(const LaunchCfg& cfg, const ShadeArgs& args, bool ext, bool feedback = false);
 bool launch_primary_shade(const LaunchCfg& cfg, const BvhDev& bvh, const ShadeArgs& args, float4* hits, bool ext);
-uint32_t launch_trace_shade(const LaunchCfg& cfg, const BvhDev& bvh, const ShadeArgs& args, bool ext, bool feedback = false);
+uint32_t launch_trace_shade(const LaunchCfg& cfg, const BvhDev& bvh, const ShadeArgs& args, bool ext, bool feedback = false, bool camera_head = false);
 bool trace_shade_has_code_form(const BvhDev& bvh, const SceneDev& scene);
 bool trace_shade_has_table_form(const BvhDev& bvh, const SceneDev& scene);
 void launch_sample_terms(hipStream_t stream, const float2* bluenoise, const FrameConst* frames, uint32_t n_slots, uint32_t num_bounces, float4* table);
 void launch_sample_terms_selftest(hipStream_t stream, const float2* bluenoise, const FrameConst* frames, uint32_t n_slots, uint32_t num_bounces,
                                   const float4* table, unsigned long long* out_device);
+
+void launch_camera_vertices(const LaunchCfg& cfg, const BvhDev& bvh, const ShadeArgs& args, uint32_t rows, float4* tab_p, float4* tab_n,
+                            unsigned long long* selftest_out = nullptr);
 
 void launch_resolve(const LaunchCfg& cfg, const Planes& planes, uint32_t n_slots, uint32_t pixels_padded, float4* accum,
                     bool albedo_in_w = false, float kd_untextured = 0.0f, bool code_in_color = false);
diff --git a/capsaicin_amd/csrc/context.hip b/capsaicin_amd/csrc/context.hip
--- a/capsaicin_amd/csrc/context.hip
+++ b/capsaicin_amd/csrc/context.hip
@@ -258,10 +258,10 @@
 
 struct LaneSizes
 {
-    size_t planes, queues, rings, counters, terms;
+    size_t planes, queues, rings, counters, terms, camera;
 };
 
-LaneSizes lane_sizes(const CapContext* c, uint32_t slots, uint32_t bounces, bool sample_table)
+LaneSizes lane_sizes(const CapContext* c, uint32_t slots, uint32_t bounces, bool sample_table, uint32_t camera_groups)
 {
     LaneSizes z;
     z.planes = (size_t)slots * c->screen.pixels_padded;
@@ -269,20 +269,22 @@
     z.rings = std::max(z.queues, (size_t)std::max(c->cu_count, 1) * 8 * (kBlock / 64) * 128);
     z.counters = (3 * (size_t)(bounces + 1) + 1) * kQueueClasses * kCounterStride;
     z.terms = sample_table ? (size_t)slots * bounces * 4096 : 0;
+    z.camera = 2 * (size_t)camera_groups * c->screen.pixels_padded;
     return z;
 }
 
-bool lane_grows(const CapContext::Lane& L, const LaneSizes& z) { return L.pl_color.n < z.planes || L.counters.n < z.counters || L.terms.n < z.terms; }
-
-int ensure_lane(CapContext* c, CapContext::Lane& L, uint32_t slots, uint32_t bounces, bool sample_table)
-{
-    const LaneSizes z = lane_sizes(c, slots, bounces, sample_table);
+bool lane_grows(const CapContext::Lane& L, const LaneSizes& z) { return L.pl_color.n < z.planes || L.counters.n < z.counters || L.terms.n < z.terms || L.camera.n < z.camera; }
+
+int ensure_lane(CapContext* c, CapContext::Lane& L, uint32_t slots, uint32_t bounces, bool sample_table, uint32_t camera_groups)
+{
+    const LaneSizes z = lane_sizes(c, slots, bounces, sample_table, camera_groups);
     for (DevBuf<float4>* b : {&L.hits, &L.q_org[0], &L.q_org[1], &L.q_dir[0], &L.q_dir[1], &L.q_thr[0], &L.q_thr[1], &L.s_dir})
         HIP_TRY(b->ensure(z.queues));
     for (DevBuf<float4>* b : {&L.s_org, &L.s_con}) HIP_TRY(b->ensure(z.rings));
     for (DevBuf<float4>* b : {&L.pl_color, &L.pl_direct, &L.pl_albedo}) HIP_TRY(b->ensure(z.planes));
     HIP_TRY(L.counters.ensure(z.counters));
     if (z.terms) HIP_TRY(L.terms.ensure(z.terms));
+    if (z.camera) HIP_TRY(L.camera.ensure(z.camera));
     if (c->lane[0].stack_spill.n) HIP_TRY(L.stack_spill.ensure(c->lane[0].stack_spill.n));
     return CAP_OK;
 }
@@ -394,7 +396,7 @@
     "CAP_NO_WIDE8", "CAP_LANE1_PRIORITY", "CAP_PLOC_RADIUS", "CAP_SAHDEV_LEAF", "CAP_WIDE_HOST_COLLAPSE", "CAP_TRACE_LAUNCHES", "CAP_NO_TWO_LANES",
     "CAP_LANE_SPLIT_MIN", "CAP_BLOCKS_PER_CU", "CAP_NO_CAMERA_CULL", "CAP_NO_ALBEDO_IN_W", "CAP_NO_INLINE_NEE", "CAP_NO_INLINE_PROBE", "CAP_NO_WAVE_RING",
     "CAP_ANY_REFILL", "CAP_PRIMARY_WIDE", "CAP_NO_PACKET", "CAP_NO_ANY_PROBE", "CAP_ANY_PROBE", "CAP_ANY_BLOCKS", "CAP_NO_PRIMARY_FUSE", "CAP_W8_REFILL",
-    "CAP_W8_GRID", "CAP_AUTO_SAH_TRIANGLES", "CAP_NO_NEE_PAIR_CULL", "CAP_RAYGEN_KERNEL", "CAP_NO_PLANE_CODE", "CAP_SAMPLE_TABLE"};
+    "CAP_W8_GRID", "CAP_AUTO_SAH_TRIANGLES", "CAP_NO_NEE_PAIR_CULL", "CAP_RAYGEN_KERNEL", "CAP_NO_PLANE_CODE", "CAP_SAMPLE_TABLE", "CAP_NO_CAMERA_TABLE"};
 
 static void switches_from_environment(SwitchTable& t)
 {
@@ -726,6 +728,31 @@
         *value = (h[0] << 32) | (expected >> 12);
         return CAP_OK;
     }
+    case CAP_DEBUG_CAMERA_TABLE: *value = c->last_camera_table; return CAP_OK;
+    case CAP_DEBUG_SELFTEST_CAMERA_TABLE:
+    {
+        const CapContext::LastCamera& lc = c->last_camera;
+        if (!c->last_camera_table || !lc.frames) return fail(CAP_ERR_STATE, "cap_debug_get: the last cap_render built no camera table");
+        HIP_TRY(hipSetDevice(c->device));
+        if (sync_and_collect(c) != CAP_OK) return CAP_ERR_HIP;
+        DevBuf<unsigned long long> d;
+        unsigned long long         h[2] = {0, 0};
+        HIP_TRY(d.ensure(2));
+        HIP_TRY(hipMemsetAsync(d.p, 0, sizeof(h), c->stream));
+        ShadeArgs sa{};
+        sa.scene = scene_dev(c), sa.cam = camera_dev(c->camera), sa.screen = c->screen, sa.frames = lc.frames, sa.n_slots = lc.n_slots;
+        sa.cull_camera_pairs = c->last_cull_camera_pairs;
+        LaunchCfg     cfg{c->stream, (uint32_t)c->cu_count * 6u, 0u, (uint32_t)c->cu_count};
+        float4* const tab = c->lane[lc.lane].camera.p;
+        launch_camera_vertices(cfg, bvh_dev(c, c->lane[lc.lane]), sa, lc.n_slots, tab, tab + (size_t)lc.n_groups * c->screen.pixels_padded, d.p);
+        HIP_TRY(hipGetLastError());
+        HIP_TRY(hipMemcpyAsync(h, d.p, sizeof(h), hipMemcpyDeviceToHost, c->stream));
+        HIP_TRY(hipStreamSynchronize(c->stream));
+        const unsigned long long expected = (unsigned long long)lc.n_slots * c->screen.pixels_padded;
+        if (h[1] != expected) return fail(CAP_ERR_HIP, "cap_debug_get: the camera table self-test compared %llu of %llu entries", h[1], expected);
+        *value = (h[0] << 32) | ((uint64_t)lc.n_groups << 16) | lc.n_slots;
+        return CAP_OK;
+    }
     case CAP_DEBUG_NEE_PAIRS:
         if (!c->bvh_ready) return fail(CAP_ERR_STATE, "cap_debug_get: BVH not built");
         *value = ((uint64_t)(c->fan_pairs_nee.p ? c->fan_pair_nee_count : c->fan_pair_count) << 32) | c->fan_pair_count;
@@ -845,9 +872,40 @@
     const bool sample_table = fused && !ext && !feedback && num_bounces >= 1 && c->sw.get(SW_SAMPLE_TABLE, 1) != 0 &&
                               trace_shade_has_table_form(bvh_dev(c, c->lane[0]), scene_dev(c));
     c->last_sample_table = sample_table ? 1u : 0u;
-    const LaneSizes need = lane_sizes(c, slots, num_bounces, sample_table);
+    const bool camera_table = sample_table && !lowres && !(flags & CAP_RENDER_AOV) && !c->sw.on(SW_NO_CAMERA_TABLE) && !c->sw.on(SW_NO_ALBEDO_IN_W) &&
+                              !c->sw.on(SW_NO_PLANE_CODE) && !c->sw.on(SW_NO_INLINE_PROBE) && !c->sw.on(SW_NO_WAVE_RING) && c->debug_capacity_div <= 1 &&
+                              c->texture_host.empty() && trace_shade_has_code_form(bvh_dev(c, c->lane[0]), scene_dev(c));
+    c->last_camera_table = 0;
+    c->last_camera       = CapContext::LastCamera{};
+    std::vector<uint32_t> slot_group, group_first, batch_groups;
+    uint32_t              camera_groups = 0;
+    if (camera_table)
+    {
+        slot_group.resize(n_frames), group_first.assign(n_frames, 0u);
+        for (uint32_t done = 0; done < n_frames; done += slots)
+        {
+            const uint32_t ns = std::min(slots, n_frames - done);
+            uint32_t       ng = 0;
+            for (uint32_t s = 0; s < ns; ++s)
+            {
+                float sx, sy, gx, gy;
+                halton23(frame_begin + done + s, sx, sy);
+                uint32_t g = 0;
+                for (; g < ng; ++g)
+                {
+                    halton23(frame_begin + done + group_first[done + g], gx, gy);
+                    if (memcmp(&gx, &sx, sizeof(float)) == 0 && memcmp(&gy, &sy, sizeof(float)) == 0) break;
+                }
+                if (g == ng) group_first[done + ng++] = s;
+                slot_group[done + s] = g;
+            }
+            batch_groups.push_back(ng);
+            camera_groups = std::max(camera_groups, ng);
+        }
+    }
+    const LaneSizes need = lane_sizes(c, slots, num_bounces, sample_table, camera_groups);
     if (lane_grows(c->lane[0], need) || !c->accum.p || c->accum.n < Ppad) HIP_TRY(hipStreamSynchronize(c->stream));
-    if (ensure_lane(c, c->lane[0], slots, num_bounces, sample_table) != CAP_OK || ensure_frame_buffers(c) != CAP_OK) return CAP_ERR_HIP;
+    if (ensure_lane(c, c->lane[0], slots, num_bounces, sample_table, camera_groups) != CAP_OK || ensure_frame_buffers(c) != CAP_OK) return CAP_ERR_HIP;
     if (policy.lane1_failed_before)
     {
         size_t free_b = 0, total_b = 0;
@@ -865,7 +923,7 @@
             HIP_TRY(hipStreamSynchronize(c->stream));
             if (c->stream2) HIP_TRY(hipStreamSynchronize(c->stream2));
         }
-        if (c->debug_fail_lane || ensure_lane(c, c->lane[1], slots, num_bounces, sample_table) != CAP_OK || ensure_lane_streams(c) != CAP_OK)
+        if (c->debug_fail_lane || ensure_lane(c, c->lane[1], slots, num_bounces, sample_table, camera_groups) != CAP_OK || ensure_lane_streams(c) != CAP_OK)
         {
             (void)hipGetLastError();
             c->lane[1] = CapContext::Lane{};
@@ -890,7 +948,11 @@
         HIP_TRY(hipHostMalloc((void**)&c->frames_pinned[ring], sizeof(FrameConst) * n_frames, hipHostMallocDefault));
         c->frames_pinned_n[ring] = n_frames;
     }
-    for (uint32_t f = 0; f < n_frames; ++f) c->frames_pinned[ring][f] = frame_const(frame_begin + f, lowres);
+    for (uint32_t f = 0; f < n_frames; ++f)
+    {
+        FrameConst& fc = c->frames_pinned[ring][f] = frame_const(frame_begin + f, lowres);
+        if (camera_table) memcpy(&fc.pad1, &slot_group[f], 4), memcpy(&fc.pad2, &group_first[f], 4);
+    }
     HIP_TRY(hipMemcpyAsync(c->frames_ring[ring].p, c->frames_pinned[ring], sizeof(FrameConst) * n_frames, hipMemcpyHostToDevice, c->stream));
     const bool st = (flags & CAP_RENDER_STAGE_TIMERS) != 0;
     if (c->textures_dirty)
@@ -1014,7 +1076,19 @@
             c->last_terms = CapContext::LastTerms{frames, ns, D, lane};
             if (trace_launch(c, "sample_terms batch %u", batch)) return fail(CAP_ERR_HIP, "sample_terms failed");
         }
-        for (uint32_t b = 0; b <= D; ++b)
+        const bool     camera_head = camera_table && sa.code_in_color && sa.wave_ring;
+        const uint32_t n_groups    = camera_head ? batch_groups[batch] : 0u;
+        float4* const  tab_p = L.camera.p, *const tab_n = L.camera.p + (size_t)n_groups * Ppad;
+        if (camera_head)
+        {
+            StageTimer t(c, ST_PRIMARY, st);
+            launch_camera_vertices(cfg, bvh, sa, n_groups, tab_p, tab_n);
+            c->last_camera = CapContext::LastCamera{frames, ns, n_groups, lane};
+            ++c->stats.launches_trace_any;
+            if (trace_launch(c, "camera_vertices batch %u", batch)) return fail(CAP_ERR_HIP, "camera_vertices failed");
+        }
+        c->last_camera_table = camera_head ? 1u : 0u;
+        for (uint32_t b = camera_head ? 1u : 0u; b <= D; ++b)
         {
             const int pi = (int)(b & 1u), po = pi ^ 1;
             sa.bounce    = b;
@@ -1025,10 +1099,12 @@
                                     po ? L.s_dir.p : L.s_org.p};
             sa.shadow    = ShadowQueue{L.s_org.p, L.s_dir.p, L.s_con.p, sh_count + b * per_queue, class_capacity};
             sa.work      = work_shade + b * per_queue;
+            const bool head = camera_head && b == 1;
+            if (head) sa.in = RayQueue{tab_p, tab_n, L.terms.p, ext_count, class_capacity, nullptr};
             if (fused)
             {
                 StageTimer t(c, b == 0 ? ST_PRIMARY : ST_CLOSEST, st);
-                const uint32_t form = launch_trace_shade(cfg, bvh, sa, ext, feedback);
+                const uint32_t form = launch_trace_shade(cfg, bvh, sa, ext, feedback, head);
                 if (b) ++c->stats.launches_trace_closest, c->last_mark_form = form;
                 if (trace_launch(c, "trace_shade bounce %u batch %u", b, batch)) return fail(CAP_ERR_HIP, "trace_shade failed");
             }
diff --git a/capsaicin_amd/csrc/small_scene.hip b/capsaicin_amd/csrc/small_scene.hip
--- a/capsaicin_amd/csrc/small_scene.hip
+++ b/capsaicin_amd/csrc/small_scene.hip
@@ -1,5 +1,6 @@
 #include "cap_shade.h"
 
+#include <algorithm>
 #include <cassert>
 
 namespace cap
@@ -16,13 +17,14 @@
 #ifdef CAP_STAMPS
 __device__ unsigned long long g_wave_times[2 * 16384];
 #endif
-template <bool FIRST_, bool EXT_, bool FB_, bool LDS_, bool TAME_, bool CODE_ = false, bool TAB_ = false>
+template <bool FIRST_, bool EXT_, bool FB_, bool LDS_, bool TAME_, bool CODE_ = false, bool TAB_ = false, bool HEAD_ = false>
 struct TraceShadeCfg
 {
     static_assert(!TAME_ || (!EXT_ && !FB_ && LDS_), "TAME: reference model, scene in LDS");
     static_assert(!CODE_ || (FIRST_ && TAME_), "CODE: bounce 0 of the reference model, scene in LDS, tame records");
     static_assert(!TAB_ || (TAME_ && kChunkLean), "TAB: the lean kernels (reference model, scene in LDS, tame records)");
-    static constexpr bool FIRST = FIRST_, EXT = EXT_, FB = FB_, LDS = LDS_, TAME = TAME_, CODE = CODE_, TAB = TAB_;
+    static_assert(!HEAD_ || (TAB_ && !FIRST_), "HEAD: the lean bounce >= 1 kernel with the sample table");
+    static constexpr bool FIRST = FIRST_, EXT = EXT_, FB = FB_, LDS = LDS_, TAME = TAME_, CODE = CODE_, TAB = TAB_, HEAD = HEAD_;
     static constexpr bool CARRY = !EXT && !TAB, SKY_RMW = false;
     static constexpr bool PROBE = !EXT && !FB && LDS;
     static constexpr bool LEAN = PROBE && TAME && kChunkLean;
@@ -129,6 +131,13 @@
 {
     using C            = TraceShadeCfg<FIRST, false, false, true, true, CODE, kChunkLean>;
     constexpr bool EXT = false, FB = false, LDS = true, TAB = kChunkLean;
+#include "small_scene_body.h"
+}
+
+__global__ __launch_bounds__(kBlock, (TraceShadeCfg<false, false, false, true, true, false, kChunkLean, kChunkLean>::kBlocksPerCu)) void k_trace_shade_head(BvhDev bvh, ShadeArgs a)
+{
+    using C              = TraceShadeCfg<false, false, false, true, true, false, kChunkLean, kChunkLean>;
+    constexpr bool FIRST = false, EXT = false, FB = false, LDS = true, TAB = kChunkLean;
 #include "small_scene_body.h"
 }
 
@@ -257,7 +266,89 @@
     hipLaunchKernelGGL(k_sample_terms_selftest, dim3(rows * (4096u / kBlock)), dim3(kBlock), 0, stream, bluenoise, frames, n_slots, num_bounces, table, out_device);
 }
 
-enum : uint32_t { TS_FIRST = 1, TS_EXT = 2, TS_FB = 4, TS_LDS = 8, TS_TAME = 16, TS_CODE = 32, TS_TAB = 64 };
+__device__ __forceinline__ void camera_vertex(const BvhDev& bvh, const ShadeArgs& a, const FrameConst& fc, uint32_t i, const float4* lds_shade,
+                                              const float4* lds_rec, const float4* lds_org, const float4* lds_bounds, float4& cp, float4& cn)
+{
+    const uint32_t lane = threadIdx.x & 63u;
+    Ray            r    = make_ray(mk3(0.f, 0.f, 0.f), mk3(0.f, 0.f, 1.f), 0.0f, 0.0f);
+    uint32_t       x, y;
+    const bool     valid = local_pixel_to_xy(a.screen, i, x, y);
+    if (valid) r = make_ray(mk3(a.cam.position[0], a.cam.position[1], a.cam.position[2]), primary_dir(a.cam, a.screen, fc, x, y), 0.0f, kPrimaryFar);
+    uint32_t tx = 0, ty = 0;
+    (void)local_pixel_to_xy(a.screen, i & ~63u, tx, ty);
+    const float4   b    = lds_bounds[lane < kExhaustiveMax / 2 ? lane : 0u];
+    const bool     over = lane < bvh.fan_pair_count && b.x < (float)(tx + 8u) && b.z >= (float)tx && b.y < (float)(ty + 8u) && b.w >= (float)ty;
+    const uint32_t pair_mask = (uint32_t)__ballot(over);
+    float          t, u, v;
+    uint32_t       gid;
+    exhaustive_closest<true, false>(bvh, lds_rec, r, t, u, v, gid, lds_org, pair_mask);
+    cp = make_float4(0.f, 0.f, 0.f, kCodePadding), cn = make_float4(0.f, 0.f, 0.f, 0.f);
+    if (valid && gid == kInvalidId)
+        cp.w = kCodeSky;
+    else if (valid)
+    {
+        const float4* tab = lds_shade + kShadeRec * (size_t)gid;
+        const float4  s0 = tab[0], s1 = tab[1], s2 = tab[2], s3 = tab[3], s4 = tab[4], s5 = tab[5];
+        const float   w = (1.0f - u) - v;
+        auto          mix = [&](float c0, float c1, float c2) { return fmaf(c2, v, fmaf(c1, u, c0 * w)); };
+        const v3      nm = mk3(mix(s3.x, s4.x, s5.x), mix(s3.y, s4.y, s5.y), mix(s3.z, s4.z, s5.z));
+        const v3      n  = normalize3_tame(nm);
+        const v3      p  = mk3(mix(s0.x, s1.x, s2.x), mix(s0.y, s1.y, s2.y), mix(s0.z, s1.z, s2.z));
+        const float   kd = a.scene.kd_untextured;
+        cp = make_float4(p.x, p.y, p.z, kd < 1e-5f ? kCodeBlack : kCodeKd);
+        cn = make_float4(n.x, n.y, n.z, 0.0f);
+    }
+}
+template <bool SELFTEST>
+__global__ __launch_bounds__(kBlock) void k_camera_vertices(BvhDev bvh, ShadeArgs a, uint32_t rows, float4* tab_p, float4* tab_n, unsigned long long* out)
+{
+    __shared__ float4 lds_shade[kShadeRec * kExhaustiveMax];
+    __shared__ float4 lds_rec[4 * kExhaustiveMax];
+    __shared__ float4 lds_org[kExhaustiveMax];
+    __shared__ float4 lds_bounds[kExhaustiveMax / 2];
+    stage_scene_records(bvh, a, lds_shade, lds_rec);
+    stage_camera_pairs(bvh, a, lds_org, lds_bounds);
+    __syncthreads();
+    const uint32_t Ppad = a.screen.pixels_padded, cps = Ppad >> 6, chunks = cps * rows, lane = threadIdx.x & 63u;
+    unsigned long long bad = 0, n = 0;
+    for (uint32_t chunk = wave_global_id(); chunk < chunks; chunk += gridDim.x * (kBlock / 64))
+    {
+        const uint32_t   row = chunk / cps, i = (chunk - row * cps) * 64 + lane;
+        const FrameConst fc  = a.frames[SELFTEST ? row : f2u(a.frames[row].pad2)];
+        float4           cp, cn;
+        camera_vertex(bvh, a, fc, i, lds_shade, lds_rec, lds_org, lds_bounds, cp, cn);
+        const size_t at = (size_t)(SELFTEST ? f2u(fc.pad1) : row) * Ppad + i;
+        if (!SELFTEST)
+            tab_p[at] = cp, tab_n[at] = cn;
+        else
+        {
+            const float4 qp = tab_p[at], qn = tab_n[at];
+            const bool   differ = f2u(qp.x) != f2u(cp.x) || f2u(qp.y) != f2u(cp.y) || f2u(qp.z) != f2u(cp.z) || f2u(qp.w) != f2u(cp.w) ||
+                                f2u(qn.x) != f2u(cn.x) || f2u(qn.y) != f2u(cn.y) || f2u(qn.z) != f2u(cn.z) || f2u(qn.w) != f2u(cn.w);
+            bad += (unsigned long long)__popcll(__ballot(differ)), n += 64ull;
+        }
+    }
+    if (SELFTEST && lane == 0u)
+    {
+        if (bad) atomicAdd(&out[0], bad);
+        if (n) atomicAdd(&out[1], n);
+    }
+}
+
+void launch_camera_vertices(const LaunchCfg& cfg, const BvhDev& bvh, const ShadeArgs& args, uint32_t rows, float4* tab_p, float4* tab_n,
+                            unsigned long long* selftest_out)
+{
+    assert(bvh.tri_count <= kExhaustiveMax && args.scene.shade_tame != 0 && args.scene.texture_count == 0);
+    const uint32_t chunks = (args.screen.pixels_padded >> 6) * rows;
+    if (!chunks) return;
+    const uint32_t gx = std::max(1u, std::min(cfg.grid_blocks, (chunks + kBlock / 64 - 1) / (kBlock / 64)));
+    if (selftest_out)
+        hipLaunchKernelGGL(k_camera_vertices<true>, dim3(gx), dim3(kBlock), 0, cfg.stream, bvh, args, rows, tab_p, tab_n, selftest_out);
+    else
+        hipLaunchKernelGGL(k_camera_vertices<false>, dim3(gx), dim3(kBlock), 0, cfg.stream, bvh, args, rows, tab_p, tab_n, selftest_out);
+}
+
+enum : uint32_t { TS_FIRST = 1, TS_EXT = 2, TS_FB = 4, TS_LDS = 8, TS_TAME = 16, TS_CODE = 32, TS_TAB = 64, TS_HEAD = 128 };
 struct TraceShadeKernel
 {
     uint32_t is;
@@ -266,7 +357,12 @@
 template <uint32_t IS>
 constexpr TraceShadeKernel trace_shade_kernel()
 {
-    if constexpr ((IS & TS_TAB) != 0)
+    if constexpr ((IS & TS_HEAD) != 0)
+    {
+        static_assert(IS == (TS_LDS | TS_TAME | TS_TAB | TS_HEAD), "HEAD: the lean bounce >= 1 kernel");
+        return {IS, k_trace_shade_head};
+    }
+    else if constexpr ((IS & TS_TAB) != 0)
     {
         static_assert((IS & ~(TS_FIRST | TS_CODE)) == (TS_LDS | TS_TAME | TS_TAB), "TAB: the lean kernels");
         return {IS, k_trace_shade_tab<(IS & TS_FIRST) != 0, (IS & TS_CODE) != 0>};
@@ -274,7 +370,7 @@
     else
         return {IS, k_trace_shade<(IS & TS_FIRST) != 0, (IS & TS_EXT) != 0, (IS & TS_FB) != 0, (IS & TS_LDS) != 0, (IS & TS_TAME) != 0, (IS & TS_CODE) != 0>};
 }
-constexpr TraceShadeKernel kTraceShadeKernels[16] = {
+constexpr TraceShadeKernel kTraceShadeKernels[17] = {
     trace_shade_kernel<TS_FIRST | TS_LDS | TS_TAME | TS_CODE>(),
     trace_shade_kernel<TS_FIRST | TS_EXT | TS_LDS>(), trace_shade_kernel<TS_FIRST | TS_EXT>(),
     trace_shade_kernel<TS_FIRST | TS_LDS | TS_TAME>(), trace_shade_kernel<TS_FIRST | TS_LDS>(), trace_shade_kernel<TS_FIRST>(),
@@ -282,6 +378,7 @@
     trace_shade_kernel<TS_FB | TS_LDS>(), trace_shade_kernel<TS_FB>(),
     trace_shade_kernel<TS_LDS | TS_TAME>(), trace_shade_kernel<TS_LDS>(), trace_shade_kernel<0>(),
     trace_shade_kernel<TS_FIRST | TS_LDS | TS_TAME | TS_CODE | TS_TAB>(), trace_shade_kernel<TS_FIRST | TS_LDS | TS_TAME | TS_TAB>(), trace_shade_kernel<TS_LDS | TS_TAME | TS_TAB>(),
+    trace_shade_kernel<TS_LDS | TS_TAME | TS_TAB | TS_HEAD>(),
 };
 
 static bool tame_kernels(const BvhDev& bvh, const SceneDev& scene)
@@ -295,7 +392,7 @@
 bool trace_shade_has_code_form(const BvhDev& bvh, const SceneDev& scene) { return tame_kernels(bvh, scene); }
 bool trace_shade_has_table_form(const BvhDev& bvh, const SceneDev& scene) { return kChunkLean && tame_kernels(bvh, scene); }
 
-uint32_t launch_trace_shade(const LaunchCfg& cfg, const BvhDev& bvh, const ShadeArgs& args, bool ext, bool feedback)
+uint32_t launch_trace_shade(const LaunchCfg& cfg, const BvhDev& bvh, const ShadeArgs& args, bool ext, bool feedback, bool camera_head)
 {
     const bool first = args.bounce == 0;
     const bool fb    = feedback && !ext && !first;
@@ -305,10 +402,12 @@
     assert(!code || tame);
     const bool tab = args.sample_terms != nullptr;
     assert(!tab || (tame && kChunkLean));
-    const uint32_t is = (first ? TS_FIRST : 0u) | (ext ? TS_EXT : 0u) | (fb ? TS_FB : 0u) | (lds ? TS_LDS : 0u) | (tame ? TS_TAME : 0u) | (code ? TS_CODE : 0u) | (tab ? TS_TAB : 0u);
-    const uint32_t gx = queue_grid(cfg, first ? args.screen.pixels_padded * args.n_slots : args.max_count);
+    assert(!camera_head || (args.bounce == 1 && tab && args.inline_probe && args.wave_ring && args.in.org_tmin && args.in.dir_tmax && args.in.thr_pid));
+    const uint32_t is = (first ? TS_FIRST : 0u) | (ext ? TS_EXT : 0u) | (fb ? TS_FB : 0u) | (lds ? TS_LDS : 0u) | (tame ? TS_TAME : 0u) | (code ? TS_CODE : 0u) | (tab ? TS_TAB : 0u) |
+                        (camera_head ? TS_HEAD : 0u);
+    const uint32_t gx = queue_grid(cfg, (first || camera_head) ? args.screen.pixels_padded * args.n_slots : args.max_count);
     const TraceShadeKernel* k = kTraceShadeKernels;
-    while (k->is != is && k + 1 < kTraceShadeKernels + 16) ++k;
+    while (k->is != is && k + 1 < kTraceShadeKernels + 17) ++k;
     assert(k->is == is);
     hipLaunchKernelGGL(k->kernel, dim3(gx), dim3(kBlock), 0, cfg.stream, bvh, args);
 #if defined(CAP_CLOSEST_V1)
diff --git a/capsaicin_amd/csrc/small_scene_body.h b/capsaicin_amd/csrc/small_scene_body.h
--- a/capsaicin_amd/csrc/small_scene_body.h
+++ b/capsaicin_amd/csrc/small_scene_body.h
@@ -1,7 +1,8 @@
     const uint32_t Ppad     = a.screen.pixels_padded;
     const uint32_t cps      = Ppad >> 6;
-    const uint32_t chunks   = FIRST ? cps * a.n_slots : (a.in.class_capacity >> 6) * kQueueClasses;
+    const uint32_t chunks   = (FIRST || C::HEAD) ? cps * a.n_slots : (a.in.class_capacity >> 6) * kQueueClasses;
     uint32_t       n_shaded = 0, n_probed = 0;
+    uint32_t       head_ext = 0, head_shadow = 0, head_probed = 0, head_shaded = 0;
     __shared__ FrameConst lds_frames[kMaxFrameSlots];
     __shared__ float4     lds_shade[LDS ? kShadeRec * kExhaustiveMax : 1];
     __shared__ float4     lds_rec[LDS ? 4 * kExhaustiveMax : 1];
@@ -51,7 +52,23 @@
         float4        c = make_float4(0.f, 0.f, 0.f, 0.f), cur = c;
         if (good) c = probe.ring_con[pos], cur = target[idx];
         const bool occluded = exhaustive_any<false>(bvh, sr);
-        if (good && !occluded) target[idx] = make_float4(cur.x + c.x, cur.y + c.y, cur.z + c.z, cur.w);
+        if constexpr (C::HEAD)
+        {
+            if (good && !occluded)
+            {
+                if (f2u(c.w) != 0u)
+                {
+                    a.planes.direct[idx] = make_float4(c.x, c.y, c.z, 0.0f);
+                    reinterpret_cast<float*>(a.planes.color + idx)[3] = c.w + kCodeLit;
+                }
+                else
+                {
+                    float* const t3 = reinterpret_cast<float*>(a.planes.color + idx);
+                    t3[0] = cur.x + c.x, t3[1] = cur.y + c.y, t3[2] = cur.z + c.z;
+                }
+            }
+        }
+        else if (good && !occluded) target[idx] = make_float4(cur.x + c.x, cur.y + c.y, cur.z + c.z, cur.w);
         ring_head = (ring_head + count) & (kWaveRing - 1u);
         ring_n -= count;
     };
@@ -64,7 +81,7 @@
     const uint32_t my_class = wave_global_id() % kQueueClasses;
     const uint32_t lane     = threadIdx.x & 63u;
     uint32_t       n_class  = 0;
-    if (!FIRST)
+    if (!FIRST && !C::HEAD)
     {
         n_class = a.in.count[my_class * kCounterStride];
         n_class = n_class < a.in.class_capacity ? n_class : a.in.class_capacity;
@@ -79,7 +96,66 @@
         v3             thr = mk3(1.0f, 1.0f, 1.0f);
         Ray            r   = make_ray(mk3(0.f, 0.f, 0.f), mk3(0.f, 0.f, 1.f), 0.0f, 0.0f);
         float          carried_r1 = 0.f, carried_r2 = 0.f;
-        if (FIRST)
+        if constexpr (C::HEAD)
+        {
+            const uint32_t chunk = class_chunk(j, my_class);
+            if (chunk >= chunks) break;
+            slot = chunk / cps;
+            i    = (chunk - slot * cps) * 64 + lane;
+            pid  = (slot << kPidShift) | i;
+            const FrameConst& fc = lds_frames[slot];
+            const size_t      at = (size_t)f2u(fc.pad1) * Ppad + i;
+            const float4      cp = a.in.org_tmin[at], cn = a.in.dir_tmax[at];
+            const uint32_t gt   = __umul24(i >> 6, a.screen.shard_count) + a.screen.shard_index;
+            const uint32_t ty   = tile_div(gt, a.screen.tiles_x_mul, a.screen.tiles_x_shift);
+            const uint32_t tx   = gt + (ty & 7u) * ((0u - a.screen.tiles_x) & 7u);
+            const uint32_t base = ((ty & 7u) << 9) | ((i & 0x38u) << 3) | ((tx & 7u) << 3) | (i & 7u);
+            const float4   q0   = a.in.thr_pid[(slot << 12) | base];
+            grab = grab_issue(a.work, my_class);
+            const v3 L = mk3(fc.light_dir[0], fc.light_dir[1], fc.light_dir[2]);
+            const v3 I = mk3(fc.light_intensity[0], fc.light_intensity[1], fc.light_intensity[2]);
+            a.planes.color[(size_t)slot * Ppad + i] = make_float4(0.f, 0.f, 0.f, cp.w);
+            const bool vtx = cp.w == kCodeKd || cp.w == kCodeBlack, lit = cp.w == kCodeKd;
+            const v3   p = mk3(cp.x, cp.y, cp.z), n = mk3(cn.x, cn.y, cn.z);
+            bool       emit_shadow = false, emit_ext = false;
+            v3         dir = unread3(), contrib = unread3();
+            float      f = unread_f();
+            if (lit)
+            {
+                const float kd  = a.scene.kd_untextured;
+                const float ndl = fmaxf(0.0f, dot3(n, L));
+                const v3    c   = mk3(((I.x * kd) * kInvPi) * ndl, ((I.y * kd) * kInvPi) * ndl, ((I.z * kd) * kInvPi) * ndl);
+                if (c.x != 0.0f || c.y != 0.0f || c.z != 0.0f) emit_shadow = true, contrib = c;
+                dir = hemisphere_dir_tame(n, [&] { return HemiTerms{q0.x, q0.y, q0.z}; });
+                const float ndd = dot3(n, dir);
+                const float pdf = div_unscaled(fmaxf(0.0f, ndd), kPi);
+                if (!(pdf < 1e-5f))
+                {
+                    f        = 1.0f * div_unscaled(kInvPi * fmaxf(ndd, 0.0f), pdf);
+                    emit_ext = true;
+                }
+            }
+            const bool occluded0 = pair_occludes_pre(make_ray(p, L, kRayEps, kRayFar), probe.pairs, probe.k, probe.rows[2u * slot], probe.rows[2u * slot + 1u]);
+            const bool probed0   = emit_shadow && occluded0;
+            emit_shadow          = emit_shadow && !occluded0;
+            const unsigned long long ms = __ballot(emit_shadow);
+            head_shaded += (uint32_t)__popcll(__ballot(vtx)), head_probed += (uint32_t)__popcll(__ballot(probed0));
+            head_ext += (uint32_t)__popcll(__ballot(emit_ext)), head_shadow += (uint32_t)__popcll(ms);
+            if (emit_shadow)
+            {
+                const uint32_t pos  = (ring_head + ring_n + (uint32_t)__popcll(ms & ((1ull << lane) - 1ull))) & (kWaveRing - 1u);
+                probe.ring_org[pos] = make_float4(p.x, p.y, p.z, u2f(pid));
+                probe.ring_con[pos] = make_float4(contrib.x, contrib.y, contrib.z, kCodeKd);
+            }
+            ring_n += (uint32_t)__popcll(ms);
+            __builtin_amdgcn_fence(__ATOMIC_RELEASE, "wavefront");
+            if (ring_n >= 64u) trace_ring(64u);
+            active = emit_ext;
+            if (__ballot(active) == 0ull) continue;
+            r   = make_ray(p, dir, kRayEps, kRayFar);
+            thr = mk3(f, f, f);
+        }
+        else if (FIRST)
         {
             const uint32_t chunk = class_chunk(j, my_class);
             if (chunk >= chunks) break;
@@ -190,3 +266,9 @@
 #endif
     if (C::PROBE && ring_n != 0u) trace_ring(ring_n);
     flush_stats(a.out.count + (size_t)my_class * kCounterStride, n_shaded, n_probed);
+    if constexpr (C::HEAD)
+    {
+        unsigned long long* const line0 = reinterpret_cast<unsigned long long*>(a.in.count + (size_t)my_class * kCounterStride);
+        if (lane == 0u && (head_ext | head_shadow)) atomicAdd(line0, ((unsigned long long)head_shadow << 32) | (unsigned long long)head_ext);
+        if (lane == 0u && (head_probed | head_shaded)) atomicAdd(line0 + 1, ((unsigned long long)head_shaded << 32) | (unsigned long long)head_probed);
+    }
diff --git a/include/capsaicin_hip.h b/include/capsaicin_hip.h
--- a/include/capsaicin_hip.h
+++ b/include/capsaicin_hip.h
@@ -182,6 +182,8 @@
     CAP_DEBUG_MARK_FORM            = 15,
     CAP_DEBUG_SAMPLE_TABLE          = 16,
     CAP_DEBUG_SELFTEST_SAMPLE_TABLE = 17,
+    CAP_DEBUG_CAMERA_TABLE          = 18,
+    CAP_DEBUG_SELFTEST_CAMERA_TABLE = 19,
     CAP_DEBUG_SWITCH_BASE         = 64
 };
 int cap_debug_set(CapContext* ctx, uint32_t key, uint64_t value);
```

After: 62960 Mrays/s (median of 6 runs). +8.7%, better.
